# VinAIResearch/DiMSUM

Hardware: AMD Instinct MI355X
Metric: denoiser-fwd latents/sec (higher is better)
Workload: dtype f32; 1 GPU; DiM-L/2 denoiser forward, 256px (4x32x32 latents, 256 tokens), 256 latents per GPU, random-init weights (reference init, zero tensors re-drawn N(0, 0.02^2)); global_batch=256, parallelism=dp1 (replicas, independent latents), launch=eager, matmul_policy=f16s (see notes.matmul_policy)

## Files before the change

### dimsum_amd/_lib.py

```python
import ctypes as C
import os

_HERE = os.path.dirname(os.path.abspath(__file__))
LIB_PATH = os.environ.get("DIMSUM_HIP_LIB") or os.path.join(_HERE, "lib", "libdimsum_hip.so")

F32, F16, BF16 = 0, 1, 2
i32, i64, vp, f32 = C.c_int32, C.c_int64, C.c_void_p, C.c_float


u32 = C.c_uint32


class _Sized(C.Structure):

    def __init__(self, *args, **kw):
        super().__init__(*args, **kw)
        self.struct_size = C.sizeof(type(self))


class SsmExt(_Sized):
    _fields_ = [("struct_size", u32), ("kernel_variant", i32), ("ckpt_ptr", vp), ("timing_start_event", vp), ("timing_stop_event", vp),
                ("out_z_lo_offset", i64), ("dt_w_ptr", vp), ("dt_x_ptr", vp), ("dt_w_row_stride", i64), ("dt_x_row_stride", i64),
                ("dt_rank", i32), ("out_z_f16", i32), ("out_z_scale_ptr", vp), ("out_z_scale_ld", i64)]


class SsmParams(_Sized):
    _fields_ = ([("struct_size", u32)]
                + [(n, i32) for n in ("batch", "dim", "seqlen", "dstate", "n_groups", "n_chunks", "delta_softplus", "dtype", "reserved")]
                + [(n, i64) for n in ("A_d_stride", "A_dstate_stride", "B_batch_stride", "B_group_stride",
                                      "B_dstate_stride", "C_batch_stride", "C_group_stride", "C_dstate_stride",
                                      "u_batch_stride", "u_d_stride", "delta_batch_stride", "delta_d_stride",
                                      "z_batch_stride", "z_d_stride", "out_batch_stride", "out_d_stride",
                                      "out_z_batch_stride", "out_z_d_stride")]
                + [(n, vp) for n in ("A_ptr", "B_ptr", "C_ptr", "D_ptr", "u_ptr", "delta_ptr", "delta_bias_ptr",
                                     "z_ptr", "out_ptr", "x_ptr", "out_z_ptr")]
                + [("ext", C.POINTER(SsmExt))])


def attach_ext(P, ext_type):
    E = ext_type()
    P.ext = C.pointer(E)
    return E


class SsmBwdParams(_Sized):
    _fields_ = ([("struct_size", u32), ("reserved", u32), ("fwd", SsmParams)]
                + [(n, i64) for n in ("dout_batch_stride", "dout_d_stride", "dA_d_stride", "dA_dstate_stride",
                                      "dB_batch_stride", "dB_group_stride", "dB_dstate_stride", "dC_batch_stride",
                                      "dC_group_stride", "dC_dstate_stride", "du_batch_stride", "du_d_stride",
                                      "dz_batch_stride", "dz_d_stride", "ddelta_batch_stride", "ddelta_d_stride")]
                + [(n, vp) for n in ("dout_ptr", "dA_ptr", "dB_ptr", "dC_ptr", "dD_ptr", "du_ptr", "dz_ptr",
                                     "ddelta_ptr", "ddelta_bias_ptr", "workspace_ptr")]
                + [("workspace_bytes", i64)])


class SsmBidirParams(_Sized):
    _fields_ = [("struct_size", u32), ("reserved", u32), ("fwd", SsmParams), ("A_b_ptr", vp), ("A_b_d_stride", i64), ("A_b_dstate_stride", i64),
                ("out_b_ptr", vp), ("out_b_batch_stride", i64), ("out_b_d_stride", i64), ("ckpt_b_ptr", vp)]


class SsmBidirBwdParams(_Sized):
    _fields_ = [("struct_size", u32), ("reserved", u32), ("bwd", SsmBwdParams), ("A_b_ptr", vp), ("A_b_d_stride", i64), ("A_b_dstate_stride", i64),
                ("out_b_ptr", vp), ("out_b_batch_stride", i64), ("out_b_d_stride", i64), ("ckpt_b_ptr", vp),
                ("dA_b_ptr", vp), ("dA_b_d_stride", i64), ("dA_b_dstate_stride", i64)]


class OptimParams(_Sized):
    _fields_ = ([("struct_size", u32), ("n_tensors", i32), ("n_chunks", i32), ("n_partials", i32)]
                + [(n, vp) for n in ("p_ptrs", "g_ptrs", "m_ptrs", "v_ptrs", "ema_ptrs", "step_ptrs", "numel", "chunk_table", "partials", "total_norm")]
                + [(n, C.c_double) for n in ("lr", "beta1", "beta2", "eps", "weight_decay", "max_norm", "ema_decay")]
                + [("reserved", i64 * 4)])


OPTIM_CHUNK, OPTIM_MAX_PARTIALS = 4096, 2048


class ConvParams(_Sized):
    _fields_ = ([("struct_size", u32)] + [(n, i32) for n in ("batch", "dim", "seqlen", "width", "silu_activation", "dtype", "reserved")]
                + [(n, i64) for n in ("x_batch_stride", "x_c_stride", "weight_c_stride", "weight_width_stride",
                                      "out_batch_stride", "out_c_stride")]
                + [(n, vp) for n in ("x_ptr", "weight_ptr", "bias_ptr", "out_ptr")])


class ConvBwdParams(_Sized):
    _fields_ = ([("struct_size", u32), ("reserved", u32), ("fwd", ConvParams)]
                + [(n, i64) for n in ("dout_batch_stride", "dout_c_stride", "dx_batch_stride", "dx_c_stride",
                                      "dweight_c_stride", "dweight_width_stride")]
                + [(n, vp) for n in ("dout_ptr", "dx_ptr", "dweight_ptr", "dbias_ptr")])


class NormParams(_Sized):
    _fields_ = ([("struct_size", u32)] + [(n, i32) for n in ("rows", "cols", "is_rms_norm", "x_dtype", "residual_dtype", "out_dtype")]
                + [("eps", f32)]
                + [(n, i64) for n in ("x_row_stride", "residual_row_stride", "y_row_stride", "residual_out_row_stride")]
                + [(n, vp) for n in ("x_ptr", "residual_ptr", "weight_ptr", "bias_ptr", "y_ptr", "residual_out_ptr",
                                     "mean_ptr", "rstd_ptr", "xbias_ptr", "mod_scale_ptr", "mod_shift_ptr")]
                + [("mod_row_stride", i64), ("rows_per_batch", i32), ("y_split3", i32), ("y_inv_scale_ptr", vp)])


class NormBwdParams(_Sized):
    _fields_ = ([("struct_size", u32)] + [(n, i32) for n in ("rows", "cols", "is_rms_norm")] + [("eps", f32), ("reserved", i32)]
                + [(n, i64) for n in ("r_row_stride", "dy_row_stride", "dres_row_stride", "dx_row_stride")]
                + [(n, vp) for n in ("r_ptr", "weight_ptr", "mean_ptr", "rstd_ptr", "dy_ptr", "dres_ptr", "dx_ptr",
                                     "dweight_ptr", "dbias_ptr")])


class TtParams(_Sized):
    _fields_ = ([("struct_size", u32)] + [(n, i32) for n in ("batch", "tokens", "channels", "grid", "kind", "y_split3")]
                + [(n, i64) for n in ("x_batch_stride", "x_token_stride", "res_batch_stride", "res_token_stride",
                                      "y_batch_stride", "y_token_stride", "mod_batch_stride", "w_batch_stride",
                                      "w_token_stride", "red_batch_stride")]
                + [(n, vp) for n in ("x_ptr", "in_index_ptr", "out_index_ptr", "gate_ptr", "scale_ptr", "shift_ptr",
                                     "residual_ptr", "y_ptr", "w_ptr", "wdot_ptr", "wsum_ptr", "tsum_ptr", "y_inv_scale_ptr")]
                + [("y_f16s_lds_offset", i32), ("reserved", i32)])


class XattnParams(_Sized):
    _fields_ = ([("struct_size", u32)] + [(n, i32) for n in ("batch", "seqlen", "heads", "head_dim")] + [("scale", f32), ("n_dirs", i32)]
                + [(n, i64) for n in ("qkv_batch_stride", "qkv_token_stride", "out_batch_stride", "out_token_stride")]
                + [(n, vp) for n in ("qkv1_ptr", "qkv2_ptr", "out_ptr", "lse_ptr", "bias1_ptr", "bias2_ptr")]
                + [("precision", i32), ("out_split3", i32)]
                + [(n, vp) for n in ("x1_inv_ptr", "x2_inv_ptr", "kv_bound_ptr", "out_inv_ptr")] + [("qkv_f16", i32), ("reserved2", i32)])


class XattnBwdParams(_Sized):
    _fields_ = ([("struct_size", u32), ("reserved", u32), ("fwd", XattnParams)] + [(n, i64) for n in ("dqkv_batch_stride", "dqkv_token_stride")]
                + [(n, vp) for n in ("dout_ptr", "dqkv1_ptr", "dqkv2_ptr", "delta_ptr")])


class GemmExt(_Sized):
    _fields_ = ([("struct_size", u32), ("rows_per_batch", i32), ("timing_start_event", vp), ("timing_stop_event", vp)]
                + [(n, i32) for n in ("tune_variant", "tune_group_m", "tune_reserved", "c_image_pieces")]
                + [(n, vp) for n in ("gate_bound_ptr", "h_inv_scale_ptr", "residual_ptr", "gate_ptr")]
                + [("residual_ld", i64), ("gate_ld", i64), ("x12_ptr", vp), ("x12_ld", i64), ("a_alias_rows", i64), ("b_alias_rows", i64),
                   ("a_alias_weight_order", i32), ("qkv_q_cols", i32), ("conv_weight_ptr", vp), ("conv_bias_ptr", vp),
                   ("conv_rows", i32), ("conv_width", i32), ("conv_seq", i32), ("conv_weight_ld", i32),
                   ("a_block_inv_ptr", vp), ("a_block_inv_ld", i64), ("tn_pair_a_cols", i64), ("tn_pair_b_cols", i64),
                   ("k_scale_ptr", vp), ("c_scale_ptr", vp), ("k_inv_a_ptr", vp), ("k_inv_b_ptr", vp)])


class GemmParams(_Sized):
    _fields_ = ([("struct_size", u32)] + [(n, i32) for n in ("m", "n", "k", "operand_dtype", "epilogue")] + [("out_scale", f32), ("reserved", i32)]
                + [(n, i64) for n in ("lda", "ldb", "ldc")]
                + [(n, vp) for n in ("a_ptr", "b_ptr", "bias_ptr", "c_ptr", "a_inv_scale_ptr", "b_inv_scale_ptr")]
                + [("ext", C.POINTER(GemmExt))])


class F16sJob(C.Structure):
    _fields_ = ([(n, vp) for n in ("src", "dst", "inv_scale_ptr", "l1max_ptr", "absmax_ptr")]
                + [(n, i64) for n in ("rows", "cols", "src_row_stride", "dst_row_stride")] + [("l1_factor", f32), ("reserved", i32)])


GEMM_EPI_F32, GEMM_EPI_GATED_GELU_SPLIT3, GEMM_EPI_GATED_GELU_F16, GEMM_EPI_F32_BIAS, GEMM_EPI_F32_GATE_RESIDUAL, GEMM_EPI_F16_QKV, GEMM_EPI_F32_CONV = 0, 1, 2, 3, 4, 5, 6

EXPORTS = (
    "dimsum_status_string", "dimsum_abi_version", "dimsum_target_arch",
    "dimsum_event_create", "dimsum_event_destroy", "dimsum_event_elapsed_ms",
    "dimsum_ssm_scan_fwd", "dimsum_ssm_scan_bwd", "dimsum_ssm_scan_bwd_workspace_bytes", "dimsum_ssm_scan_fwd_variant",
    "dimsum_ssm_scan_bidir_fwd", "dimsum_ssm_scan_bidir_bwd", "dimsum_ssm_scan_bidir_fwd_variant",
    "dimsum_optim_grad_sumsq", "dimsum_optim_adamw_ema_step", "dimsum_optim_write_ptrs",
    "dimsum_causal_conv1d_fwd", "dimsum_causal_conv1d_bwd",
    "dimsum_norm_fwd", "dimsum_norm_bwd", "dimsum_token_transform", "dimsum_xattn_fusion_fwd", "dimsum_xattn_fusion_bwd",
    "dimsum_gated_gelu_fwd", "dimsum_gated_gelu_bwd", "dimsum_gated_gelu_fwd_split3", "dimsum_gated_gelu_bwd_split3", "dimsum_gated_gelu_bwd_pair", "dimsum_gated_gelu_bwd_f16s", "dimsum_split3", "dimsum_split3_t",
    "dimsum_gemm_nt", "dimsum_gemm_nt_kernel_for", "dimsum_gemm_tn", "dimsum_gemm_nn", "dimsum_row_factors", "dimsum_rows_block_f16s", "dimsum_rows_f16s", "dimsum_rows_f16s_multi",
)

_P = C.POINTER
_SIGNATURES = (
    [("dimsum_status_string", C.c_char_p, [C.c_int]), ("dimsum_target_arch", C.c_char_p, None), ("dimsum_abi_version", C.c_int, None),
     ("dimsum_event_create", vp, []), ("dimsum_event_destroy", None, [vp]), ("dimsum_event_elapsed_ms", C.c_float, [vp, vp])]
    + [(name, C.c_int, [_P(ptype), vp]) for name, ptype in (
        ("dimsum_ssm_scan_fwd", SsmParams), ("dimsum_ssm_scan_bwd", SsmBwdParams), ("dimsum_ssm_scan_bidir_fwd", SsmBidirParams),
        ("dimsum_ssm_scan_bidir_bwd", SsmBidirBwdParams), ("dimsum_optim_grad_sumsq", OptimParams), ("dimsum_optim_adamw_ema_step", OptimParams),
        ("dimsum_causal_conv1d_fwd", ConvParams), ("dimsum_causal_conv1d_bwd", ConvBwdParams), ("dimsum_norm_fwd", NormParams),
        ("dimsum_norm_bwd", NormBwdParams), ("dimsum_token_transform", TtParams), ("dimsum_xattn_fusion_fwd", XattnParams),
        ("dimsum_xattn_fusion_bwd", XattnBwdParams), ("dimsum_gemm_nt", GemmParams))]
    + [(name, C.c_int, [vp] * nptr + [i64, i64, vp]) for name, nptr in (
        ("dimsum_gated_gelu_fwd", 3), ("dimsum_gated_gelu_bwd", 5), ("dimsum_gated_gelu_fwd_split3", 3), ("dimsum_gated_gelu_bwd_split3", 5),
        ("dimsum_gated_gelu_bwd_pair", 5), ("dimsum_gated_gelu_bwd_f16s", 6))]
    + [("dimsum_optim_write_ptrs", C.c_int, [vp, i64, _P(vp), i32, vp]),
       ("dimsum_gemm_nt_kernel_for", C.c_int, [_P(GemmParams)]),
       ("dimsum_gemm_tn", C.c_int, [_P(GemmParams), i32, i64, vp]),
       ("dimsum_gemm_nn", C.c_int, [_P(GemmParams), i32, i64, vp]),
       ("dimsum_rows_block_f16s", C.c_int, [vp, i64, i64, i64, vp, i64, vp, i64, vp]),
       ("dimsum_row_factors", C.c_int, [vp, vp, i64, vp, vp, vp]),
       ("dimsum_split3", C.c_int, [vp, i64, i64, i64, vp, i32, vp]),
       ("dimsum_split3_t", C.c_int, [vp, i64, i64, i64, vp, vp]),
       ("dimsum_rows_f16s", C.c_int, [vp, i64, i64, i64, vp, i64, vp, vp, vp]),
       ("dimsum_rows_f16s_multi", C.c_int, [_P(F16sJob), i32, vp]),
       ("dimsum_ssm_scan_bwd_workspace_bytes", i64, [i32] * 5),
       ("dimsum_ssm_scan_fwd_variant", C.c_int, [_P(SsmParams)]),
       ("dimsum_ssm_scan_bidir_fwd_variant", C.c_int, [_P(SsmBidirParams)])])

_lib = None


def load():
    global _lib
    if _lib is not None:
        return _lib
    if not os.path.exists(LIB_PATH):
        raise RuntimeError(f"dimsum_amd: {LIB_PATH} not found. Build it with `python -c 'import __graft_entry__ as g; "
                           f"g.build()'` or `make -C dimsum_amd/csrc`. There is no CPU fallback.")
    lib = C.CDLL(LIB_PATH)
    for name, restype, argtypes in _SIGNATURES:
        if hasattr(lib, name):
            fn = getattr(lib, name)
            fn.restype, fn.argtypes = restype, argtypes
    if lib.dimsum_abi_version() != 18:
        raise RuntimeError("dimsum_amd: libdimsum_hip.so ABI version mismatch; rebuild")
    _lib = lib
    return lib


GEMM_NT_KERNELS = {0: "gemm_nt_kernel<256 x 256 tiles>", 1: "gemm_nt_m128_kernel<128 x 256 tiles>", 2: "gemm_nt_persist_kernel"}
SCAN_FWD_KERNELS = {1: "ssm_scan_fwd_kernel", 2: "ssm_scan_fwd_split_kernel<2 lanes per channel>",
                    4: "ssm_scan_fwd_split_kernel<4 lanes per channel>",
                    16: "ssm_scan_fwd_lanes_kernel<one lane per state>"}


def check(status, what):
    if status != 0:
        raise RuntimeError(f"{what}: {load().dimsum_status_string(status).decode()} (status {status})")
```

### dimsum_amd/csrc/gemm_nt.hip

```cpp
#include "gemm_nt_kernel.hpp"

namespace dimsum {
namespace gemm_nt {

template <int kOp, int kEpi, int kVar = 0> int launch(const Args &a, hipStream_t s, hipEvent_t e0, hipEvent_t e1, int *probe) {
    if (probe) { *probe = 0; return DIMSUM_OK; }
    const dim3 grid((unsigned)(a.tiles_m * a.tiles_n)), block(512);
    if (e0 || e1) hipExtLaunchKernelGGL((gemm_nt_kernel<kOp, kEpi, kVar>), grid, block, 0, s, e0, e1, 0, a);
    else hipLaunchKernelGGL((gemm_nt_kernel<kOp, kEpi, kVar>), grid, block, 0, s, a);
    return launch_status();
}

template <int kOp, int kEpi, int kVar = 0> int launch_m128(const Args &a0, hipStream_t s, hipEvent_t e0, hipEvent_t e1, int *probe) {
    if (probe) { *probe = 1; return DIMSUM_OK; }
    Args a = a0;
    a.tiles_m = a.M / 128;
    a.group_m = a.tiles_m <= 32 ? a.tiles_m : 2 * a0.group_m;
    const dim3 grid((unsigned)(a.tiles_m * a.tiles_n)), block(256);
    if (e0 || e1) hipExtLaunchKernelGGL((gemm_nt_m128_kernel<kOp, kEpi, kVar>), grid, block, 0, s, e0, e1, 0, a);
    else hipLaunchKernelGGL((gemm_nt_m128_kernel<kOp, kEpi, kVar>), grid, block, 0, s, a);
    return launch_status();
}

inline int persist_grid() {
    int dev = 0, cus = 256;
    if (hipGetDevice(&dev) == hipSuccess) (void)hipDeviceGetAttribute(&cus, hipDeviceAttributeMultiprocessorCount, dev);
    return cus >= 8 ? cus / 8 * 8 : 8;
}
inline bool persist_ok(const Args &a, int tune_variant) {
    const int nk = a.K / kBK;
    return tune_variant != 513 && tune_variant != 512 && nk >= 4 && nk % 2 == 0 && a.tiles_m * a.tiles_n > persist_grid() && a.a_alias_tiles == 0 && a.b_alias_tiles == 0;
}
template <int kOp, int kEpi, int kVar = 0> int launch_persist(const Args &a, hipStream_t s, hipEvent_t e0, hipEvent_t e1, int *probe) {
    if (probe) { *probe = 2; return DIMSUM_OK; }
    const dim3 grid((unsigned)persist_grid()), block(512);
    if (e0 || e1) hipExtLaunchKernelGGL((gemm_nt_persist_kernel<kOp, kEpi, kVar>), grid, block, 0, s, e0, e1, 0, a);
    else hipLaunchKernelGGL((gemm_nt_persist_kernel<kOp, kEpi, kVar>), grid, block, 0, s, a);
    return launch_status();
}

template <int kEpi, int kVar = 0> int launch_f16(const Args &a, hipStream_t s, hipEvent_t e0, hipEvent_t e1, bool m128, int *probe) {
    return m128 ? launch_m128<kOpF16, kEpi, kVar>(a, s, e0, e1, probe) : launch<kOpF16, kEpi, kVar>(a, s, e0, e1, probe);
}

struct gemm_flat_t : dimsum_gemm_ext_t {
    int32_t m, n, k, operand_dtype, epilogue;
    float out_scale;
    int64_t lda, ldb, ldc;
    const void *a_ptr, *b_ptr, *bias_ptr;
    void *c_ptr;
    const void *a_inv_scale_ptr, *b_inv_scale_ptr;
};
static int gemm_flat_from(const dimsum_gemm_params_t *p, gemm_flat_t &f) {
    if (!p) return DIMSUM_ERR_NULL;
    if (p->struct_size != sizeof(dimsum_gemm_params_t)) return DIMSUM_ERR_ABI;
    const int rc = ext_from<dimsum_gemm_ext_t>(p->ext, f);
    if (rc != DIMSUM_OK) return rc;
    f.m = p->m; f.n = p->n; f.k = p->k; f.operand_dtype = p->operand_dtype; f.epilogue = p->epilogue; f.out_scale = p->out_scale;
    f.lda = p->lda; f.ldb = p->ldb; f.ldc = p->ldc;
    f.a_ptr = p->a_ptr; f.b_ptr = p->b_ptr; f.bias_ptr = p->bias_ptr; f.c_ptr = p->c_ptr;
    f.a_inv_scale_ptr = p->a_inv_scale_ptr; f.b_inv_scale_ptr = p->b_inv_scale_ptr;
    return DIMSUM_OK;
}

}
}

static int gemm_nt_run(const dimsum_gemm_params_t *pub, void *stream, int *probe) {
    using namespace dimsum;
    using namespace dimsum::gemm_nt;
    gemm_flat_t flat;
    {
        const int frc = gemm_flat_from(pub, flat);
        if (frc != DIMSUM_OK) return frc;
    }
    const gemm_flat_t *p = &flat;
    if (!p->a_ptr || !p->b_ptr || !p->c_ptr) return DIMSUM_ERR_NULL;
    if (p->operand_dtype != DIMSUM_F16 && p->operand_dtype != DIMSUM_BF16) return DIMSUM_ERR_DTYPE;
    if (p->m <= 0 || p->n <= 0 || p->k < 2 * kBK || p->m % kBM != 0 || p->k % kBK != 0 || p->n % 4 != 0) return DIMSUM_ERR_SHAPE;
    if (p->a_alias_rows != 0 && (p->a_alias_rows < 0 || p->a_alias_rows % kBK != 0 || p->k != 3 * p->a_alias_rows)) return DIMSUM_ERR_SHAPE;
    if (p->b_alias_rows != 0 && (p->b_alias_rows < 0 || p->b_alias_rows % kBK != 0 || p->k != 3 * p->b_alias_rows || (p->epilogue != DIMSUM_GEMM_EPI_F32 && p->epilogue != DIMSUM_GEMM_EPI_F32_CONV))) return DIMSUM_ERR_SHAPE;
    if (p->lda % 8 != 0 || p->ldb % 8 != 0 || p->lda < (p->a_alias_rows ? 2 * p->a_alias_rows : p->k) || p->ldb < (p->b_alias_rows ? 2 * p->b_alias_rows : p->k) ||
        !aligned_to<char>(p->a_ptr, 16) ||
        !aligned_to<char>(p->b_ptr, 16))
        return DIMSUM_ERR_STRIDE;
    if ((int64_t)256 * p->lda * 2 >= ((int64_t)1 << 31) || (int64_t)256 * p->ldb * 2 >= ((int64_t)1 << 31) || (int64_t)257 * p->ldc * 4 >= ((int64_t)1 << 31))
        return DIMSUM_ERR_STRIDE;
    Args a{};
    a.A = reinterpret_cast<const char *>(p->a_ptr);
    a.C = p->c_ptr;
    a.lda = p->lda; a.ldb = p->ldb; a.ldc = p->ldc;
    a.M = p->m; a.K = p->k;
    a.tiles_m = p->m / kBM;
    a.out_scale = p->out_scale;
    a.a_alias_tiles = (int)(p->a_alias_rows / kBK);
    a.a_alias_from = a.a_alias_tiles;
    if (p->a_alias_weight_order) {
        if (!p->a_alias_rows) return DIMSUM_ERR_SHAPE;
        a.a_alias_tiles *= 2;
        a.a_alias_from = a.a_alias_tiles;
    }
    a.b_alias_tiles = (int)(p->b_alias_rows / kBK);
    a.group_m = p->tune_group_m > 0 ? p->tune_group_m : (a.tiles_m <= 16 ? a.tiles_m : 4);
    a.stagger = p->tune_reserved > 0 ? p->tune_reserved : 0;
    if ((p->a_inv_scale_ptr == nullptr) != (p->b_inv_scale_ptr == nullptr)) return DIMSUM_ERR_NULL;
    a.sa = reinterpret_cast<const float *>(p->a_inv_scale_ptr);
    a.sb = reinterpret_cast<const float *>(p->b_inv_scale_ptr);
    if (a.sb && !aligned_to<char>(a.sb, 16)) return DIMSUM_ERR_STRIDE;
    hipStream_t s = reinterpret_cast<hipStream_t>(stream);
    hipEvent_t e0 = reinterpret_cast<hipEvent_t>(p->timing_start_event), e1 = reinterpret_cast<hipEvent_t>(p->timing_stop_event);
    const bool bf = p->operand_dtype == DIMSUM_BF16;
    const bool m128 = p->tune_variant == 512 || (p->tune_variant == 0 && !bf && p->k <= 576 && (p->epilogue == DIMSUM_GEMM_EPI_F32 || p->epilogue == DIMSUM_GEMM_EPI_F32_BIAS));
#ifndef DIMSUM_GEMM_TUNE
    if (p->tune_variant != 0 && p->tune_variant != 512 && p->tune_variant != 513 && p->tune_variant != 514) return DIMSUM_ERR_UNSUPPORTED;
#endif
    if (p->tune_variant == 512 && bf) return DIMSUM_ERR_UNSUPPORTED;
    if (p->epilogue == DIMSUM_GEMM_EPI_F32_GATE_RESIDUAL) {
        if (!p->residual_ptr) return DIMSUM_ERR_NULL;
        if (p->ldc % 4 != 0 || p->ldc < p->n || !aligned_to<char>(p->c_ptr, 16) || p->residual_ld % 4 != 0 || p->residual_ld < p->n ||
            !aligned_to<char>(p->residual_ptr, 16) || (p->bias_ptr && !aligned_to<char>(p->bias_ptr, 16)) ||
            (p->gate_ptr && (p->gate_ld % 4 != 0 || !aligned_to<char>(p->gate_ptr, 16))))
            return DIMSUM_ERR_STRIDE;
        if (p->gate_ptr && (p->rows_per_batch <= 0 || p->rows_per_batch % kBM != 0 || p->m % p->rows_per_batch != 0)) return DIMSUM_ERR_SHAPE;
        a.B0 = a.B1 = reinterpret_cast<const char *>(p->b_ptr);
        a.bias0 = reinterpret_cast<const float *>(p->bias_ptr);
        a.res = reinterpret_cast<const float *>(p->residual_ptr);
        a.gate = reinterpret_cast<const float *>(p->gate_ptr);
        a.ldr = p->residual_ld; a.ldg = p->gate_ld;
        a.rows_per_batch = p->gate_ptr ? p->rows_per_batch : p->m;
        a.N = p->n;
        a.tiles_n = (p->n + kBN - 1) / kBN;
        constexpr int kShipR = kVarFullLineStores | kVarNtStores;
        if (!bf && !m128 && p->tune_variant == 514 && p->n % kBN == 0 && persist_ok(a, p->tune_variant)) return launch_persist<kOpF16, kEpiF32GateRes, kShipR>(a, s, e0, e1, probe);
        return bf ? launch<kOpBf16, kEpiF32GateRes, kShipR>(a, s, e0, e1, probe) : launch_f16<kEpiF32GateRes, kShipR>(a, s, e0, e1, m128, probe);
    }
    if (p->epilogue == DIMSUM_GEMM_EPI_F16_QKV) {
        if (bf || !a.sa || !p->gate_bound_ptr) return DIMSUM_ERR_NULL;
        if (p->rows_per_batch <= 0 || p->rows_per_batch % kBM != 0 || p->m % p->rows_per_batch != 0 || p->qkv_q_cols <= 0 || p->qkv_q_cols % 16 != 0 ||
            p->qkv_q_cols > p->n || p->n % 8 != 0)
            return DIMSUM_ERR_SHAPE;
        if (p->ldc % 8 != 0 || p->ldc < p->n || !aligned_to<char>(p->c_ptr, 16) || (p->bias_ptr && !aligned_to<char>(p->bias_ptr, 16)) ||
            (int64_t)257 * p->ldc * 2 >= ((int64_t)1 << 31))
            return DIMSUM_ERR_STRIDE;
        a.B0 = a.B1 = reinterpret_cast<const char *>(p->b_ptr);
        a.bias0 = reinterpret_cast<const float *>(p->bias_ptr);
        a.gate_bound = reinterpret_cast<const float *>(p->gate_bound_ptr);
        a.rows_per_batch = p->rows_per_batch;
        a.q_cols = p->qkv_q_cols;
        a.N = p->n;
        a.tiles_n = (p->n + kBN - 1) / kBN;
        return launch_f16<kEpiF16Qkv>(a, s, e0, e1, p->tune_variant == 512 || (p->tune_variant == 0 && p->k <= 576), probe);
    }
    if (p->epilogue == DIMSUM_GEMM_EPI_F32_CONV) {
        if (!p->conv_weight_ptr) return DIMSUM_ERR_NULL;
        if (p->conv_rows <= 0 || p->conv_rows % kBM != 0 || p->conv_rows > p->m || p->conv_width < 2 || p->conv_width > 4 || p->conv_seq <= 0 || 256 % p->conv_seq != 0 ||
            p->conv_seq % 4 != 0 || p->n % p->conv_seq != 0 || p->conv_weight_ld < p->conv_width)
            return DIMSUM_ERR_SHAPE;
        if (p->ldc % 4 != 0 || p->ldc < p->n || !aligned_to<char>(p->c_ptr, 16)) return DIMSUM_ERR_STRIDE;
        a.B0 = a.B1 = reinterpret_cast<const char *>(p->b_ptr);
        a.conv_w = reinterpret_cast<const float *>(p->conv_weight_ptr);
        a.conv_b = reinterpret_cast<const float *>(p->conv_bias_ptr);
        a.conv_rows = p->conv_rows; a.conv_width = p->conv_width; a.conv_seq = p->conv_seq; a.conv_w_ld = p->conv_weight_ld;
        a.N = p->n;
        a.tiles_n = (p->n + kBN - 1) / kBN;
        constexpr int kShipC = kVarFullLineStores | kVarNtStores;
        return bf ? launch<kOpBf16, kEpiF32Conv, kShipC>(a, s, e0, e1, probe) : launch_f16<kEpiF32Conv, kShipC>(a, s, e0, e1, p->tune_variant == 512 || (p->tune_variant == 0 && p->k <= 576), probe);
    }
    if (p->epilogue == DIMSUM_GEMM_EPI_F32 || p->epilogue == DIMSUM_GEMM_EPI_F32_BIAS) {
        if (p->ldc % 4 != 0 || p->ldc < p->n || !aligned_to<char>(p->c_ptr, 16)) return DIMSUM_ERR_STRIDE;
        const bool bias = p->epilogue == DIMSUM_GEMM_EPI_F32_BIAS;
        if (bias && (!p->bias_ptr || !aligned_to<char>(p->bias_ptr, 16))) return DIMSUM_ERR_NULL;
        a.B0 = a.B1 = reinterpret_cast<const char *>(p->b_ptr);
        a.bias0 = reinterpret_cast<const float *>(p->bias_ptr);
        a.N = p->n;
        a.tiles_n = (p->n + kBN - 1) / kBN;
        constexpr int kShip = kVarFullLineStores | kVarNtStores;
        if (bias) return bf ? launch<kOpBf16, kEpiF32Bias, kShip>(a, s, e0, e1, probe) : launch_f16<kEpiF32Bias, kShip>(a, s, e0, e1, m128, probe);
#ifdef DIMSUM_GEMM_TUNE
        if (bf) switch (p->tune_variant) {
            case 0: case 512: case 513: break;
            case 100: return launch<kOpBf16, kEpiF32, 0>(a, s, e0, e1, probe);
            case 1: return launch<kOpBf16, kEpiF32, 1>(a, s, e0, e1, probe);
            case 2: return launch<kOpBf16, kEpiF32, 2>(a, s, e0, e1, probe);
            case 4: return launch<kOpBf16, kEpiF32, 4>(a, s, e0, e1, probe);
            case 8: return launch<kOpBf16, kEpiF32, 8>(a, s, e0, e1, probe);
            case 12: return launch<kOpBf16, kEpiF32, 12>(a, s, e0, e1, probe);
            case 16: return launch<kOpBf16, kEpiF32, 16>(a, s, e0, e1, probe);
            case 3: return launch<kOpBf16, kEpiF32, 3>(a, s, e0, e1, probe);
            case 40: return launch<kOpBf16, kEpiF32, 40>(a, s, e0, e1, probe);
            case 44: return launch<kOpBf16, kEpiF32, 44>(a, s, e0, e1, probe);
            case 72: return launch<kOpBf16, kEpiF32, 72>(a, s, e0, e1, probe);
            case 104: return launch<kOpBf16, kEpiF32, 104>(a, s, e0, e1, probe);
            default: return DIMSUM_ERR_UNSUPPORTED;
        }
#endif
        return bf ? launch<kOpBf16, kEpiF32, kShip>(a, s, e0, e1, probe) : launch_f16<kEpiF32, kShip>(a, s, e0, e1, m128, probe);
    }
    if (p->epilogue == DIMSUM_GEMM_EPI_GATED_GELU_SPLIT3 || p->epilogue == DIMSUM_GEMM_EPI_GATED_GELU_F16) {
        if (p->n % 16 != 0) return DIMSUM_ERR_SHAPE;
        const int F = p->n / 2;
        const bool img = p->epilogue == DIMSUM_GEMM_EPI_GATED_GELU_SPLIT3;
        if (p->c_image_pieces != 0 && p->c_image_pieces != 3 && !(img && p->c_image_pieces == 2)) return DIMSUM_ERR_UNSUPPORTED;
        a.c_pieces2 = p->c_image_pieces == 2;
        if (p->ldc % 8 != 0 || p->ldc < (img ? (a.c_pieces2 ? 2 : 3) : 1) * (int64_t)F || !aligned_to<char>(p->c_ptr, 16) || (int64_t)257 * p->ldc * 2 + 6 * (int64_t)F >= ((int64_t)1 << 31))
            return DIMSUM_ERR_STRIDE;
        if (p->bias_ptr && !aligned_to<char>(p->bias_ptr, 16)) return DIMSUM_ERR_STRIDE;
        a.B0 = reinterpret_cast<const char *>(p->b_ptr);
        a.B1 = a.B0 + (int64_t)F * p->ldb * 2;
        a.bias0 = reinterpret_cast<const float *>(p->bias_ptr);
        a.bias1 = a.bias0 ? a.bias0 + F : nullptr;
        a.N = F;
        a.tiles_n = (F + 127) / 128;
        if (p->gate_bound_ptr) {
            if (img || !a.sa || !p->h_inv_scale_ptr) return DIMSUM_ERR_NULL;
            a.gate_bound = reinterpret_cast<const float *>(p->gate_bound_ptr);
            a.inv_out = reinterpret_cast<float *>(p->h_inv_scale_ptr);
        }
        if (p->x12_ptr) {
            const bool f16_train = !img && !bf && a.sa && p->gate_bound_ptr;
            if (!f16_train && (!img || !bf || a.sa)) return DIMSUM_ERR_UNSUPPORTED;
            if (p->x12_ld % 4 != 0 || p->x12_ld < p->n || !aligned_to<char>(p->x12_ptr, 16) || (int64_t)257 * p->x12_ld * 4 + (int64_t)p->n * 4 >= ((int64_t)1 << 31))
                return DIMSUM_ERR_STRIDE;
            a.x12 = reinterpret_cast<float *>(p->x12_ptr);
            a.ldx = p->x12_ld;
            if (f16_train) return launch<kOpF16, kEpiGatedF16, kVarKeepX12>(a, s, e0, e1, probe);
            return launch<kOpBf16, kEpiGatedSplit3, kVarKeepX12>(a, s, e0, e1, probe);
        }
        if (img) return bf ? launch<kOpBf16, kEpiGatedSplit3>(a, s, e0, e1, probe) : launch<kOpF16, kEpiGatedSplit3>(a, s, e0, e1, probe);
        if (!bf && !m128 && F % 128 == 0 && persist_ok(a, p->tune_variant)) return launch_persist<kOpF16, kEpiGatedF16>(a, s, e0, e1, probe);
        return bf ? launch<kOpBf16, kEpiGatedF16>(a, s, e0, e1, probe) : launch_f16<kEpiGatedF16>(a, s, e0, e1, m128, probe);
    }
    return DIMSUM_ERR_UNSUPPORTED;
}

extern "C" int dimsum_gemm_nt(const dimsum_gemm_params_t *p, void *stream) { return gemm_nt_run(p, stream, nullptr); }

extern "C" int dimsum_gemm_nt_kernel_for(const dimsum_gemm_params_t *p) {
    int which = -1;
    const int rc = gemm_nt_run(p, nullptr, &which);
    return rc == DIMSUM_OK ? which : -rc;
}

extern "C" int dimsum_gemm_tn(const dimsum_gemm_params_t *pub, int32_t splits, int64_t c_split_stride, void *stream) {
    using namespace dimsum;
    using namespace dimsum::gemm_nt;
    gemm_flat_t flat;
    {
        const int frc = gemm_flat_from(pub, flat);
        if (frc != DIMSUM_OK) return frc;
    }
    const gemm_flat_t *p = &flat;
    if (!p->a_ptr || !p->b_ptr || !p->c_ptr) return DIMSUM_ERR_NULL;
    if (p->operand_dtype != DIMSUM_F16 && p->operand_dtype != DIMSUM_BF16) return DIMSUM_ERR_DTYPE;
    if (p->epilogue != DIMSUM_GEMM_EPI_F32 || p->bias_ptr) return DIMSUM_ERR_UNSUPPORTED;
    if (((p->a_inv_scale_ptr || p->a_block_inv_ptr) == 0) != (p->b_inv_scale_ptr == nullptr)) return DIMSUM_ERR_NULL;
    if ((p->a_inv_scale_ptr || p->a_block_inv_ptr) && (p->operand_dtype != DIMSUM_F16 || splits != 1 || p->tn_pair_a_cols != 0 || p->a_alias_rows != 0)) return DIMSUM_ERR_UNSUPPORTED;
    if (p->k_inv_b_ptr && !p->k_inv_a_ptr) return DIMSUM_ERR_NULL;
    if (p->k_scale_ptr || p->k_inv_a_ptr) {
        if (p->k_inv_a_ptr ? (p->k_scale_ptr || p->c_scale_ptr) : !p->c_scale_ptr) return DIMSUM_ERR_NULL;
        if (p->operand_dtype != DIMSUM_F16 || p->a_inv_scale_ptr || p->a_block_inv_ptr || p->tn_pair_a_cols != 0 || p->a_alias_rows != 0) return DIMSUM_ERR_UNSUPPORTED;
        if (splits < 1 || p->k / splits > 16384) return DIMSUM_ERR_SHAPE;
        if ((p->k_scale_ptr && (!aligned_to<char>(p->k_scale_ptr, 16) || !aligned_to<char>(p->c_scale_ptr, 4))) ||
            (p->k_inv_a_ptr && (!aligned_to<char>(p->k_inv_a_ptr, 16) || (p->k_inv_b_ptr && !aligned_to<char>(p->k_inv_b_ptr, 16)) || p->k / splits % 8 != 0)))
            return DIMSUM_ERR_STRIDE;
    }
    if (p->a_block_inv_ptr && (p->a_inv_scale_ptr || p->a_block_inv_ld < p->k / kBK || p->k > 64 * kBK)) return DIMSUM_ERR_SHAPE;
    if (p->b_inv_scale_ptr && !aligned_to<char>(p->b_inv_scale_ptr, 16)) return DIMSUM_ERR_STRIDE;
    const int row_splits = (p->tn_pair_a_cols != 0) ? splits / 3 : splits;
    const int64_t n_pad = (p->n + kBN - 1) / kBN * kBN;
    if (splits < 1 || row_splits < 1 || p->m <= 0 || p->n <= 0 || p->m % kBM != 0 || p->n % 4 != 0 || (p->n % kBN != 0 && (p->ldb < n_pad || p->tn_pair_a_cols != 0)) ||
        p->k % ((int64_t)row_splits * kBK) != 0 || p->k / row_splits < 2 * kBK)
        return DIMSUM_ERR_SHAPE;
    if (p->lda % 8 != 0 || p->ldb % 8 != 0 || p->lda < p->m || p->ldb < p->n || !aligned_to<char>(p->a_ptr, 16) || !aligned_to<char>(p->b_ptr, 16) ||
        p->ldc % 4 != 0 || p->ldc < p->n || !aligned_to<char>(p->c_ptr, 16) || (splits > 1 && (c_split_stride % 4 != 0 || c_split_stride < (int64_t)p->m * p->ldc)))
        return DIMSUM_ERR_STRIDE;
    if ((int64_t)64 * p->lda * 2 + 512 >= ((int64_t)1 << 31) || (int64_t)64 * p->ldb * 2 + 512 >= ((int64_t)1 << 31) || (int64_t)257 * p->ldc * 4 >= ((int64_t)1 << 31))
        return DIMSUM_ERR_STRIDE;
    Args a{};
    a.A = reinterpret_cast<const char *>(p->a_ptr);
    a.B0 = a.B1 = reinterpret_cast<const char *>(p->b_ptr);
    a.C = p->c_ptr;
    a.lda = p->lda; a.ldb = p->ldb; a.ldc = p->ldc;
    a.M = p->m; a.N = p->n; a.K = p->k / row_splits;
    a.tiles_m = p->m / kBM;
    a.tiles_n = (int)(n_pad / kBN);
// ... 97 lines not shown
```

### dimsum_amd/csrc/gemm_nt_kernel.hpp

```cpp
#pragma once
#include "common.hpp"

namespace dimsum {
namespace gemm_nt {

typedef float f4 __attribute__((ext_vector_type(4)));
typedef __bf16 bf16x8_t __attribute__((ext_vector_type(8)));
typedef _Float16 f16x8_t __attribute__((ext_vector_type(8)));
typedef unsigned u32x4 __attribute__((ext_vector_type(4)));
typedef unsigned u32x2 __attribute__((ext_vector_type(2)));
typedef __attribute__((address_space(3))) void lds_void_t;
typedef __attribute__((address_space(1))) const void glb_void_t;

constexpr int kBM = 256, kBN = 256, kBK = 64;
constexpr int kHalf = 16384;
constexpr int kParity = 4 * kHalf;
constexpr int kSlotA0 = 0, kSlotA1 = kHalf, kSlotB0 = 2 * kHalf, kSlotB1 = 3 * kHalf;

enum { kOpBf16 = 0, kOpF16 = 1 };
enum { kEpiF32 = 0, kEpiGatedSplit3 = 1, kEpiGatedF16 = 2, kEpiF32Bias = 3, kEpiF32GateRes = 4, kEpiF16Qkv = 5, kEpiF32Conv = 6 };

struct Args {
    const char *A, *B0, *B1;
    void *C;
    const float *bias0, *bias1;
    const float *sa, *sb;
    const float *gate_bound;
    float *inv_out;
    const float *res, *gate;
    int64_t ldr, ldg;
    int rows_per_batch;
    int64_t lda, ldb, ldc;
    int M, N, K;
    int tiles_m, tiles_n;
    float out_scale;
    int group_m;
    int stagger;
    float *x12;
    int64_t ldx;
    int splits;
    int64_t c_split_stride;
    int a_alias_tiles;
    int a_alias_from;
    int tn_pieces;
    int64_t a_pair_cols, b_pair_cols;
    int b_alias_tiles;
    const float *conv_w, *conv_b;
    int conv_rows, conv_width, conv_seq, conv_w_ld;
    const float *a_block_inv;
    int a_block_inv_ld;
    const _Float16 *k_fac;
    const float *c_scale;
    const float *k_inv_a, *k_inv_b;
    int q_cols;
    int c_pieces2;
};
enum { kVarLgkmAfterBarrier = 1, kVarNoEpilogue = 2, kVarNtStores = 4, kVarFullLineStores = 8, kVarNoSetprio = 16, kVarSc1Stores = 32, kVarSc0Stores = 64, kVarKeepX12 = 128, kVarTN = 256, kVarM128 = 512, kVarRebase = 1024, kVarPersist = 2048, kVarRowFac = 4096, kVarNN = 8192 };

__device__ __forceinline__ float dpp_row_ror8(float x) {
    const int v = __builtin_bit_cast(int, x);
    return __builtin_bit_cast(float, __builtin_amdgcn_update_dpp(v, v, 0x128, 0xf, 0xf, false));
}
template <int kAux> __device__ __forceinline__ void store_f4(__amdgpu_buffer_rsrc_t rsrc, unsigned voff, const f4 &v) {
    __builtin_amdgcn_raw_buffer_store_b128(__builtin_bit_cast(u32x4, v), rsrc, voff, 0, kAux);
}

template <int kOp> __device__ __forceinline__ f4 mma(const u32x4 &a, const u32x4 &b, f4 c) {
    if constexpr (kOp == kOpBf16) return __builtin_amdgcn_mfma_f32_16x16x32_bf16(__builtin_bit_cast(bf16x8_t, a), __builtin_bit_cast(bf16x8_t, b), c, 0, 0, 0);
    else return __builtin_amdgcn_mfma_f32_16x16x32_f16(__builtin_bit_cast(f16x8_t, a), __builtin_bit_cast(f16x8_t, b), c, 0, 0, 0);
}

__device__ __forceinline__ const char *uniform_ptr(const char *q) {
    const uint64_t v = reinterpret_cast<uint64_t>(q);
    const unsigned lo = __builtin_amdgcn_readfirstlane((unsigned)v), hi = __builtin_amdgcn_readfirstlane((unsigned)(v >> 32));
    return reinterpret_cast<const char *>(((uint64_t)hi << 32) | lo);
}

__device__ __forceinline__ unsigned pick_mask(bool c) {
    unsigned m = c ? 0xffffffffu : 0u;
    asm volatile("" : "+v"(m));
    return m;
}
__device__ __forceinline__ unsigned pick_mask_lanes(bool c) {
    unsigned m = c ? 0xffffffffu : 0u;
    asm volatile("" : "+v"(m));
    return m;
}
__device__ __forceinline__ float pick(unsigned m, float a, float b) {
    return __uint_as_float((__float_as_uint(a) & m) | (__float_as_uint(b) & ~m));
}
__device__ __forceinline__ f4 pick(unsigned m, const f4 &a, const f4 &b) {
    return f4{pick(m, a[0], b[0]), pick(m, a[1], b[1]), pick(m, a[2], b[2]), pick(m, a[3], b[3])};
}

#define DIMSUM_DS_READ_B128(dst, addr, off) asm volatile("ds_read_b128 %0, %1 offset:%2" : "=v"(dst) : "v"(addr), "i"(off))
#define DIMSUM_DS_READ_TR(dst, addr, off) asm volatile("ds_read_b64_tr_b16 %0, %1 offset:%2" : "=v"(dst) : "v"(addr), "i"(off))
#define DIMSUM_WAIT_VM(n) asm volatile("s_waitcnt vmcnt(" #n ")" ::: "memory")
#ifndef DIMSUM_PERSIST_GS
#define DIMSUM_PERSIST_GS 2
#endif
#ifndef DIMSUM_EPI_PACE
#define DIMSUM_EPI_PACE 0
#endif
#define DIMSUM_STR2(x) #x
#define DIMSUM_STR(x) DIMSUM_STR2(x)
#define DIMSUM_PACE_STORES() do { if constexpr (kM1 && DIMSUM_EPI_PACE >= 0) asm volatile("s_waitcnt vmcnt(" DIMSUM_STR(DIMSUM_EPI_PACE) ")" ::: "memory"); } while (0)
#define DIMSUM_WAIT_LGKM0() asm volatile("s_waitcnt lgkmcnt(0)" ::: "memory")

__device__ __forceinline__ float gelu_tanh_f(float x) {
    const float u = 0.7978845608028654f * (x + 0.044715f * x * x * x);
    return x * fast_rcp(1.0f + fast_exp2(-2.0f * kLog2e * u));
}

template <int kOp, int kEpi, int kVar>
__device__ __forceinline__ void gemm_body(const Args &p, char *lds) {
    const unsigned lds0 = (unsigned)(uintptr_t)(__attribute__((address_space(3))) char *)lds;
    const int lane = threadIdx.x & 63;
    const int w = __builtin_amdgcn_readfirstlane(threadIdx.x >> 6);
    constexpr bool kM1 = (kVar & kVarM128) != 0;
    constexpr int kTileM = kM1 ? 128 : kBM;
    constexpr int kMiRows = kM1 ? 64 : 128;
    const int wr = kM1 ? 0 : (w >> 2), wc = w & 3;

    constexpr bool kTN = (kVar & kVarTN) != 0;
    constexpr bool kNN = (kVar & kVarNN) != 0;
    constexpr bool kBT = kTN || kNN;
    static_assert(!kBT || kEpi == kEpiF32, "the TN / NN variants have the plain fp32 epilogue");
    static_assert(!(kBT && kM1) && !(kTN && kNN), "the TN / NN variants have 256 x 256 tiles only");
    constexpr bool kPersist = (kVar & kVarPersist) != 0;
    static_assert(!kPersist || (!kTN && !kM1 && (kEpi == kEpiF32 || kEpi == kEpiF32Bias || kEpi == kEpiF32GateRes || kEpi == kEpiGatedF16)), "persistent: the 256-row NT kernel");
    int tile_m, tile_n, split = 0;
    auto map_tile = [&](int bid, int &tile_m, int &tile_n) {
        const int nwg = kPersist ? p.tiles_m * p.tiles_n : (int)gridDim.x;
        const int q = nwg >> 3, r = nwg & 7, xcd = bid & 7;
        int t = (xcd < r ? xcd * (q + 1) : r * (q + 1) + (xcd - r) * q) + (bid >> 3);
        if constexpr (kBT) {
            const int tiles = p.tiles_m * p.tiles_n;
            split = t / tiles;
            t -= split * tiles;
        }
        const int GM = p.group_m;
        const int per_group = GM * p.tiles_n;
        const int g = t / per_group, within = t - g * per_group;
        const int first_m = g * GM;
        const int gsz = min(p.tiles_m - first_m, GM);
        tile_n = within / gsz;
        tile_m = first_m + (within - tile_n * gsz);
    };
    int bid = blockIdx.x;
    map_tile(bid, tile_m, tile_n);
    constexpr int kTileN = (kEpi == kEpiGatedSplit3 || kEpi == kEpiGatedF16) ? 128 : kBN;
    int m0 = tile_m * kTileM, n0 = tile_n * kTileN;

    const int st_row = w * 16 + (lane >> 2);
    const int st_kc = (lane & 3) ^ ((lane >> 5) << 1);
    const unsigned a_voff = (unsigned)((st_row * p.lda + st_kc * 8) * 2);
    struct Src { const char *a_base, *b_base[2]; unsigned b_voff[2]; };
    auto make_src = [&](int m0_, int n0_) {
        Src s_;
        if constexpr (kEpi == kEpiGatedSplit3 || kEpi == kEpiGatedF16) {
            s_.b_base[0] = p.B0 + (int64_t)n0_ * p.ldb * 2;
            s_.b_base[1] = p.B1 + (int64_t)n0_ * p.ldb * 2;
            const int row = min(st_row, p.N - 1 - n0_);
            s_.b_voff[0] = s_.b_voff[1] = (unsigned)((row * p.ldb + st_kc * 8) * 2);
        } else {
            s_.b_base[0] = s_.b_base[1] = p.B0 + (int64_t)n0_ * p.ldb * 2;
#pragma unroll
            for (int ni = 0; ni < 2; ++ni) {
                const int row = min(ni * 128 + st_row, p.N - 1 - n0_);
                s_.b_voff[ni] = (unsigned)((row * p.ldb + st_kc * 8) * 2);
            }
        }
        s_.a_base = p.A + (int64_t)m0_ * p.lda * 2;
        return s_;
    };
    Src cur = make_src(m0, n0);
    const char *(&b_base)[2] = cur.b_base;
    unsigned (&b_voff)[2] = cur.b_voff;
    const char *&a_base = cur.a_base;
    const int64_t a_half = (int64_t)kMiRows * p.lda * 2;
    unsigned b_voff2[2][2];
    if constexpr (kM1) {
#pragma unroll
        for (int ni = 0; ni < 2; ++ni)
#pragma unroll
            for (int h = 0; h < 2; ++h) {
                const int first = (kEpi == kEpiGatedSplit3 || kEpi == kEpiGatedF16) ? 0 : ni * 128;
                const int row = min(first + h * 64 + st_row, p.N - 1 - n0);
                b_voff2[ni][h] = (unsigned)((row * p.ldb + st_kc * 8) * 2);
            }
    }

    unsigned tn_voff_a[2], tn_voff_b[2];
    const char *tn_a = nullptr, *tn_b = nullptr;
    int64_t tn_a_tile = 0, tn_b_tile = 0;
    int tn_row_split = 0;
    if constexpr (kBT) {
#pragma unroll
        for (int pc = 0; pc < 2; ++pc) {
            const int row = w * 8 + pc * 4 + (lane >> 4), key = pc * 4 + (lane >> 4);
            const int chunk = ((((lane & 15) >> 1) ^ key) << 1) | (lane & 1);
            const int rl = row & 31, srow = kNN ? ((row & ~31) | (((rl & 15) >> 2) << 3) | ((rl >> 4) << 2) | (rl & 3)) : row;
            tn_voff_a[pc] = (unsigned)(srow * p.lda * 2 + chunk * 16);
            tn_voff_b[pc] = (unsigned)(srow * p.ldb * 2 + chunk * 16);
        }
        int row_split = split;
        int64_t a_col = 0, b_col = 0;
        if (p.tn_pieces) {
            const int spp = p.splits / 3, piece = split / spp;
            row_split = split - piece * spp;
// ... 264 lines not shown
            adv(spos, 2 * kU);
        };
#define DIMSUM_M1_SYNC()                                                                   \
    do {                                                                                   \
        DIMSUM_WAIT_LGKM0();                                                               \
        __builtin_amdgcn_s_barrier();                                                      \
        __builtin_amdgcn_sched_barrier(0);                                                 \
    } while (0)
#define DIMSUM_M1_PHASE(READ, SIZE, STAGE, VM, MI, NI, AF, BF)                              \
    do {                                                                                   \
        READ;                                                                              \
        adv(rpos, SIZE);                                                                   \
        STAGE;                                                                             \
        DIMSUM_WAIT_VM(VM);                                                                \
        DIMSUM_M1_SYNC();                                                                  \
        DIMSUM_QUADRANT(MI, NI, AF, BF);                                                   \
        __builtin_amdgcn_sched_barrier(0);                                                 \
    } while (0)
        st_a(0, 0); st_b(0, 0); st_b(1, 0); st_a(1, 0); st_a(0, 1); st_b(0, 1);
        DIMSUM_WAIT_VM(12);
        __builtin_amdgcn_s_barrier();
        __builtin_amdgcn_sched_barrier(0);
        DIMSUM_READ_A(a0, 0, rpos);
        adv(rpos, kU);
        DIMSUM_M1_SYNC();
        int kt = 0;
        for (; kt < nk - 2; ++kt) {
            DIMSUM_M1_PHASE(DIMSUM_READ_B(b0, 0, rpos), 2 * kU, st_b(1, kt + 1), 12, 0, 0, a0, b0);
            DIMSUM_M1_PHASE(DIMSUM_READ_B(b1, 0, rpos), 2 * kU, st_a(1, kt + 1), 12, 0, 1, a0, b1);
            DIMSUM_M1_PHASE(DIMSUM_READ_A(a1, 0, rpos), kU, st_a(0, kt + 2), 12, 1, 1, a1, b1);
            DIMSUM_M1_PHASE(DIMSUM_READ_A(a0, 0, rpos), kU, st_b(0, kt + 2), 12, 1, 0, a1, b0);
        }
        DIMSUM_M1_PHASE(DIMSUM_READ_B(b0, 0, rpos), 2 * kU, st_b(1, kt + 1), 12, 0, 0, a0, b0);
        DIMSUM_M1_PHASE(DIMSUM_READ_B(b1, 0, rpos), 2 * kU, st_a(1, kt + 1), 12, 0, 1, a0, b1);
        DIMSUM_M1_PHASE(DIMSUM_READ_A(a1, 0, rpos), kU, (void)0, 10, 1, 1, a1, b1);
        DIMSUM_M1_PHASE(DIMSUM_READ_A(a0, 0, rpos), kU, (void)0, 6, 1, 0, a1, b0);
        DIMSUM_M1_PHASE(DIMSUM_READ_B(b0, 0, rpos), 2 * kU, (void)0, 2, 0, 0, a0, b0);
        DIMSUM_M1_PHASE(DIMSUM_READ_B(b1, 0, rpos), 2 * kU, (void)0, 0, 0, 1, a0, b1);
        DIMSUM_M1_PHASE(DIMSUM_READ_A(a1, 0, rpos), kU, (void)0, 0, 1, 1, a1, b1);
        DIMSUM_QUADRANT(1, 0, a1, b0);
#undef DIMSUM_M1_PHASE
#undef DIMSUM_M1_SYNC
    } else {
    stage_a0(0); stage_b0(0); stage_b1(0); stage_a1(0);
    stage_a0(1); stage_b0(1); stage_b1(1); stage_a1(1);
    DIMSUM_WAIT_VM(12);
    __builtin_amdgcn_s_barrier();
    if (wr == 1) __builtin_amdgcn_s_barrier();
    __builtin_amdgcn_sched_barrier(0);
    DIMSUM_READ_A(a0, kSlotA0, 0);
    read_fac(0);
    DIMSUM_PHASE_SYNC();
    rebase(a0, 0, 0);
    DIMSUM_PHASE_END();

    }
#define DIMSUM_KTILE(KT, ST_A0, ST_B0, ST_B1, ST_A1, W12, W34)                                                                  \
    do {                                                                                                                        \
        const unsigned par = ((KT) & 1) * kParity, par_next = kParity - par;                                                    \
        DIMSUM_READ_B(b0, kSlotB0, par); ST_A0; if (W12) DIMSUM_WAIT_VM(12); DIMSUM_PHASE_SYNC();                               \
        DIMSUM_QUADRANT(0, 0, a0, b0); DIMSUM_PHASE_END();                                                                      \
        DIMSUM_READ_B(b1, kSlotB1, par); ST_B0; if (W12) DIMSUM_WAIT_VM(12); DIMSUM_PHASE_SYNC();                               \
        DIMSUM_QUADRANT(0, 1, a0, b1); DIMSUM_PHASE_END();                                                                      \
        DIMSUM_READ_A(a1, kSlotA1, par); read_fac(KT); ST_B1; if (W34) DIMSUM_WAIT_VM(12); DIMSUM_PHASE_SYNC();                 \
        rebase(a1, 1, KT); DIMSUM_QUADRANT(1, 1, a1, b1); DIMSUM_PHASE_END();                                                   \
        DIMSUM_READ_A(a0, kSlotA0, par_next); read_fac((KT) + 1);                                                               \
        ST_A1; if (W34) DIMSUM_WAIT_VM(12); DIMSUM_PHASE_SYNC();                                                                \
        DIMSUM_QUADRANT(1, 0, a1, b0);                                                                                          \
        rebase(a0, 0, (KT) + 1);                     \
        DIMSUM_PHASE_END();                                                                                                     \
    } while (0)
    bool resumed = false;
    for (;;) {
    bool has_next = false;
    int nbid = 0, ntile_m = 0, ntile_n = 0;
    Src nxt = cur;
    if constexpr (kPersist) {
        nbid = bid + (int)gridDim.x;
        has_next = nbid < p.tiles_m * p.tiles_n;
        if (has_next) {
            map_tile(nbid, ntile_m, ntile_n);
            nxt = make_src(ntile_m * kTileM, ntile_n * kTileN);
        }
    }
    if constexpr (kPersist) {
        for (int kt = 0; kt < nk; ++kt) {
            const bool own = kt + 2 < nk;
            const int skt = own ? kt + 2 : kt + 2 - nk;
            Src ss;
            ss.a_base = uniform_ptr(own ? cur.a_base : nxt.a_base);
            ss.b_base[0] = uniform_ptr(own ? cur.b_base[0] : nxt.b_base[0]);
            ss.b_base[1] = uniform_ptr(own ? cur.b_base[1] : nxt.b_base[1]);
            ss.b_voff[0] = cur.b_voff[0];
            ss.b_voff[1] = cur.b_voff[1];
            const bool w12 = !(resumed && kt < 2), w34 = !(resumed && kt < 1);
            DIMSUM_KTILE(kt, stage_of(ss, 0, skt), stage_of(ss, 1, skt), stage_of(ss, 2, skt), stage_of(ss, 3, skt), w12, w34);
        }
        if (wr == 0) __builtin_amdgcn_s_barrier();
    } else if constexpr (!kM1) {
    int kt = 0;
    for (; kt < nk - 2; ++kt) DIMSUM_KTILE(kt, stage_a0(kt + 2), stage_b0(kt + 2), stage_b1(kt + 2), stage_a1(kt + 2), true, true);
    {
        const unsigned par = (kt & 1) * kParity, par_next = kParity - par;
        DIMSUM_READ_B(b0, kSlotB0, par);
        DIMSUM_WAIT_VM(10);
        DIMSUM_PHASE_SYNC();
        DIMSUM_QUADRANT(0, 0, a0, b0);
        DIMSUM_PHASE_END();
        DIMSUM_READ_B(b1, kSlotB1, par);
        DIMSUM_WAIT_VM(8);
        DIMSUM_PHASE_SYNC();
        DIMSUM_QUADRANT(0, 1, a0, b1);
        DIMSUM_PHASE_END();
        DIMSUM_READ_A(a1, kSlotA1, par);
        read_fac(kt);
        DIMSUM_WAIT_VM(6);
        DIMSUM_PHASE_SYNC();
        rebase(a1, 1, kt);
        DIMSUM_QUADRANT(1, 1, a1, b1);
        DIMSUM_PHASE_END();
        DIMSUM_READ_A(a0, kSlotA0, par_next);
        read_fac(kt + 1);
        DIMSUM_WAIT_VM(4);
        DIMSUM_PHASE_SYNC();
        DIMSUM_QUADRANT(1, 0, a1, b0);
        rebase(a0, 0, kt + 1);
        DIMSUM_PHASE_END();
        DIMSUM_READ_B(b0, kSlotB0, par_next);
        DIMSUM_WAIT_VM(2);
        DIMSUM_PHASE_SYNC();
        DIMSUM_QUADRANT(0, 0, a0, b0);
        DIMSUM_PHASE_END();
        DIMSUM_READ_B(b1, kSlotB1, par_next);
        DIMSUM_WAIT_VM(0);
        DIMSUM_PHASE_SYNC();
        DIMSUM_QUADRANT(0, 1, a0, b1);
        DIMSUM_PHASE_END();
        DIMSUM_READ_A(a1, kSlotA1, par_next);
        read_fac(kt + 1);
        DIMSUM_PHASE_SYNC();
        rebase(a1, 1, kt + 1);
        DIMSUM_QUADRANT(1, 1, a1, b1);
        DIMSUM_PHASE_END();
        DIMSUM_QUADRANT(1, 0, a1, b0);
    }
    if (wr == 0) __builtin_amdgcn_s_barrier();
    }

    int lane_e = lane;
    if constexpr (kPersist) asm volatile("" : "+v"(lane_e));
    {
    const int lane = lane_e;
    const int ecol = wc * 32 + (lane >> 4) * 4;
    if constexpr (kVar & kVarNoEpilogue) {
#pragma unroll
        for (int mi = 0; mi < 2; ++mi)
#pragma unroll
            for (int ni = 0; ni < 2; ++ni)
#pragma unroll
                for (int i = 0; i < 4; ++i)
#pragma unroll
                    for (int j = 0; j < 2; ++j) asm volatile("" ::"v"(acc[mi][ni][i][j]));
    } else if constexpr (kEpi == kEpiF32 || kEpi == kEpiF32Bias || kEpi == kEpiF32GateRes || kEpi == kEpiF32Conv) {
        if constexpr (kEpi == kEpiF32Conv) {
            if (m0 < p.conv_rows) {
                constexpr int kNW = kM1 ? 4 : 8;
                constexpr int kHalfRows = kM1 ? 64 : 128;
                float *Ct = reinterpret_cast<float *>(p.C) + (int64_t)m0 * p.ldc + n0;
                const __amdgpu_buffer_rsrc_t crsrc = __builtin_amdgcn_make_buffer_rsrc(Ct, 0, 0x7fffffff, 0x00020000);
                const int W = p.conv_width;
                const bool has_s = p.sa != nullptr;
                const unsigned ms = pick_mask(has_s);
                const float *sap = has_s ? p.sa + m0 : reinterpret_cast<const float *>(p.A), *sbp = has_s ? p.sb : reinterpret_cast<const float *>(p.B0);
                float csa[2][4];
                f4 csb[2][2];
#pragma unroll
                for (int mi = 0; mi < 2; ++mi)
#pragma unroll
                    for (int i = 0; i < 4; ++i) {
                        csa[mi][i] = pick(ms, sap[mi * kMiRows + wr * 64 + i * 16 + (lane & 15)], 1.0f);
                    }
#pragma unroll
                for (int ni = 0; ni < 2; ++ni)
#pragma unroll
                    for (int j = 0; j < 2; ++j) {
                        const int col = n0 + ni * 128 + ecol + j * 16;
                        csb[ni][j] = pick(ms, *reinterpret_cast<const f4 *>(sbp + (col < p.N ? col : 0)), f4{1.f, 1.f, 1.f, 1.f});
                    }
                float ctap[2], cbia[2];
#pragma unroll
                for (int mi = 0; mi < 2; ++mi) {
                    const int row = m0 + mi * kMiRows + w * (kHalfRows / kNW) + (lane & 15);
                    ctap[mi] = pick(pick_mask_lanes((lane >> 4) < W), p.conv_w[(int64_t)row * p.conv_w_ld + ((lane >> 4) < W ? (lane >> 4) : 0)], 0.f);
                    cbia[mi] = pick(pick_mask(p.conv_b != nullptr), (p.conv_b ? p.conv_b : reinterpret_cast<const float *>(p.B0))[row], 0.f);
                }
#pragma unroll
                for (int mi = 0; mi < 2; ++mi) {
                    if (mi) __syncthreads();
#pragma unroll
                    for (int ni = 0; ni < 2; ++ni)
#pragma unroll
                        for (int j = 0; j < 2; ++j) {
                            const int tcol = ni * 128 + ecol + j * 16;
#pragma unroll
                            for (int i = 0; i < 4; ++i) {
                                const int rl = wr * 64 + i * 16 + (lane & 15);
                                const f4 x = acc[mi][ni][i][j] * (csb[ni][j] * csa[mi][i]);
                                *reinterpret_cast<f4 *>(lds + rl * 1024 + (((tcol >> 2) ^ (rl & 7)) << 4)) = x;
                            }
                        }
                    __syncthreads();
#pragma unroll 4
                    for (int it = 0; it < kHalfRows / kNW; ++it) {
                        const int rl = w * (kHalfRows / kNW) + it, row = m0 + mi * kMiRows + rl;
                        const f4 v = *reinterpret_cast<const f4 *>(lds + rl * 1024 + ((lane ^ (rl & 7)) << 4));
                        float w4[4];
#pragma unroll
                        for (int k = 0; k < 4; ++k)
                            w4[k] = (k >= 4 - W) ? __builtin_bit_cast(float, __builtin_amdgcn_readlane(__builtin_bit_cast(int, ctap[mi]), it + 16 * (k - (4 - W)))) : 0.f;
                        const float cbias = __builtin_bit_cast(float, __builtin_amdgcn_readlane(__builtin_bit_cast(int, cbia[mi]), it));
                        const bool start = ((4 * lane) % p.conv_seq) == 0;
                        float p1 = __shfl_up(v[3], 1, 64), p2 = __shfl_up(v[2], 1, 64), p3 = __shfl_up(v[1], 1, 64);
                        p1 = start ? 0.f : p1; p2 = start ? 0.f : p2; p3 = start ? 0.f : p3;
                        f4 y;
                        y[0] = fmaf(w4[0], p3, fmaf(w4[1], p2, fmaf(w4[2], p1, fmaf(w4[3], v[0], cbias))));
                        y[1] = fmaf(w4[0], p2, fmaf(w4[1], p1, fmaf(w4[2], v[0], fmaf(w4[3], v[1], cbias))));
                        y[2] = fmaf(w4[0], p1, fmaf(w4[1], v[0], fmaf(w4[2], v[1], fmaf(w4[3], v[2], cbias))));
                        y[3] = fmaf(w4[0], v[0], fmaf(w4[1], v[1], fmaf(w4[2], v[2], fmaf(w4[3], v[3], cbias))));
#pragma unroll
                        for (int e = 0; e < 4; ++e) y[e] = y[e] * fast_rcp(1.0f + fast_exp(-y[e]));
                        if (n0 + 4 * lane < p.N) store_f4<2>(crsrc, (unsigned)(((mi * kMiRows + rl) * p.ldc + 4 * lane) * 4), y);
                        DIMSUM_PACE_STORES();
                    }
                }
                return;
            }
        }
        constexpr int kAux = ((kVar & kVarNtStores) ? 2 : 0) | ((kVar & kVarSc1Stores) ? 16 : 0) | ((kVar & kVarSc0Stores) ? 1 : 0);
        float *Ct = reinterpret_cast<float *>(p.C) + (int64_t)m0 * p.ldc + n0 + (kBT ? (int64_t)split * p.c_split_stride : (int64_t)0);
        const __amdgpu_buffer_rsrc_t rsrc = __builtin_amdgcn_make_buffer_rsrc(Ct, 0, 0x7fffffff, 0x00020000);
        if constexpr (kVar & kVarFullLineStores) {
            const bool up = (lane & 8) != 0;
            const int frow = wr * 64 + (lane & 7);
            const int fcol = wc * 32 + (lane >> 4) * 4 + (up ? 16 : 0);
            const bool has_s = kRebase || p.sa != nullptr;
            const unsigned ms = pick_mask(has_s);
            const bool has_sb = has_s && !kRowFac;
            const unsigned msb = pick_mask(has_sb);
            const float *sap = p.sa ? p.sa + m0 : reinterpret_cast<const float *>(p.A), *sbp = has_sb ? p.sb : reinterpret_cast<const float *>(p.B0);
            float c_scale = 1.0f;
            if constexpr (kRowFac) c_scale = p.k_inv_a ? c_scale_own : *p.c_scale;
            bool live[2];
            f4 bv[2], sbv[2], gv[2];
            auto load_cols = [&](int ni) {
                const int col = ni * 128 + fcol;
                live[ni] = n0 + col < p.N;
                const int lc = live[ni] ? n0 + col : 0;
                bv[ni] = f4{0.f, 0.f, 0.f, 0.f}; sbv[ni] = gv[ni] = f4{1.f, 1.f, 1.f, 1.f};
                if constexpr (kEpi == kEpiF32Bias) bv[ni] = *reinterpret_cast<const f4 *>(p.bias0 + lc);
                if constexpr (kEpi == kEpiF32GateRes) {
                    bv[ni] = pick(pick_mask(p.bias0 != nullptr), *reinterpret_cast<const f4 *>((p.bias0 ? p.bias0 : reinterpret_cast<const float *>(p.B0)) + lc), bv[ni]);
                    gv[ni] = pick(pick_mask(p.gate != nullptr),
                                  *reinterpret_cast<const f4 *>((p.gate ? p.gate + (int64_t)(m0 / p.rows_per_batch) * p.ldg : reinterpret_cast<const float *>(p.B0)) + lc), gv[ni]);
                }
                sbv[ni] = pick(msb, *reinterpret_cast<const f4 *>(sbp + lc), sbv[ni]);
            };
            load_cols(0);
            live[1] = n0 + 128 + fcol < p.N;
            float rs[2][4][2];
            if constexpr (!kPersist || kRebase || kEpi != kEpiF32GateRes)
#pragma unroll
            for (int mi = 0; mi < 2; ++mi)
#pragma unroll
                for (int i = 0; i < 4; ++i) {
                    const int lrow = frow + mi * kMiRows + i * 16;
                    if constexpr (kRebase) rs[mi][i][0] = rs[mi][i][1] = top[mi * 2 + (i >> 1)];
                    else if constexpr (kRowFac) {
                        rs[mi][i][0] = c_scale * pick(ms, sap[lrow], 1.0f); rs[mi][i][1] = c_scale * pick(ms, sap[lrow + 8], 1.0f);
                    }
                    else {
                        rs[mi][i][0] = pick(ms, sap[lrow], 1.0f); rs[mi][i][1] = pick(ms, sap[lrow + 8], 1.0f);
                    }
                }
            constexpr int kGS = kPersist ? DIMSUM_PERSIST_GS : 4, kNG = 16 / kGS;
            f4 rr[2][kGS][2];
            float rg[2][kGS][2];
            auto load_res = [&](int g) {
                if constexpr (kEpi == kEpiF32GateRes) {
                    const int t0 = g * kGS, ni = t0 >> 3, mi = (t0 >> 2) & 1;
                    if constexpr (kPersist) {
#pragma unroll
                        for (int k = 0; k < kGS; ++k) {
                            const int lrow = frow + mi * kMiRows + ((t0 + k) & 3) * 16;
                            rg[g & 1][k][0] = pick(ms, sap[lrow], 1.0f); rg[g & 1][k][1] = pick(ms, sap[lrow + 8], 1.0f);
                        }
                    }
                    const float *rp = p.res + (int64_t)(m0 + frow + mi * kMiRows) * p.ldr + (live[ni] ? n0 + ni * 128 + fcol : 0);
#pragma unroll
                    for (int k = 0; k < kGS; ++k) {
                        const int i = (t0 + k) & 3;
                        rr[g & 1][k][0] = *reinterpret_cast<const f4 *>(rp + (int64_t)(i * 16) * p.ldr);
                        rr[g & 1][k][1] = *reinterpret_cast<const f4 *>(rp + (int64_t)(i * 16 + 8) * p.ldr);
                    }
                }
            };
            load_res(0);
#pragma unroll
            for (int g = 0; g < kNG; ++g) {
                if (g + 1 < kNG) load_res(g + 1);
                if (g * kGS == 4) load_cols(1);
#pragma unroll
                for (int k = 0; k < kGS; ++k) {
                    const int t = g * kGS + k, ni = t >> 3, mi = (t >> 2) & 1, i = t & 3;
                    const int col = ni * 128 + fcol;
                    const f4 x0 = acc[mi][ni][i][0], x1 = acc[mi][ni][i][1];
                    f4 s0, s1;
#pragma unroll
                    for (int e = 0; e < 4; ++e) {
                        const float r0 = dpp_row_ror8(x0[e]), r1 = dpp_row_ror8(x1[e]);
                        s0[e] = up ? r1 : x0[e];
                        s1[e] = up ? x1[e] : r0;
                    }
                    const int lrow = frow + mi * kMiRows + i * 16;
                    const unsigned voff = (unsigned)((lrow * p.ldc + col) * 4);
                    constexpr bool kRowsInGroup = kPersist && kEpi == kEpiF32GateRes;
                    s0 = s0 * (sbv[ni] * (kRowsInGroup ? rg[g & 1][k][0] : rs[mi][i][0]));
                    s1 = s1 * (sbv[ni] * (kRowsInGroup ? rg[g & 1][k][1] : rs[mi][i][1]));
                    if constexpr (kEpi == kEpiF32GateRes) {
                        s0 = rr[g & 1][k][0] + gv[ni] * (s0 + bv[ni]);
                        s1 = rr[g & 1][k][1] + gv[ni] * (s1 + bv[ni]);
                    } else {
                        s0 = s0 + bv[ni];
                        s1 = s1 + bv[ni];
                    }
                    if (live[ni]) {
                        store_f4<kAux>(rsrc, voff, s0);
                        store_f4<kAux>(rsrc, voff + (unsigned)(8 * p.ldc * 4), s1);
                    }
                    if constexpr (kEpi != kEpiF32GateRes) DIMSUM_PACE_STORES();
                }
            }
        } else {
            const int frow = wr * 64 + (lane & 15);
#pragma unroll
            for (int ni = 0; ni < 2; ++ni)
#pragma unroll
                for (int j = 0; j < 2; ++j) {
                    const int col = ni * 128 + ecol + j * 16;
                    if (n0 + col < p.N) {
                        f4 bv = f4{0.f, 0.f, 0.f, 0.f};
                        if constexpr (kEpi == kEpiF32Bias) bv = *reinterpret_cast<const f4 *>(p.bias0 + n0 + col);
#pragma unroll
                        for (int mi = 0; mi < 2; ++mi)
#pragma unroll
                            for (int i = 0; i < 4; ++i)
                                store_f4<kAux>(rsrc, (unsigned)(((frow + mi * kMiRows + i * 16) * p.ldc + col) * 4), acc[mi][ni][i][j] + bv);
                    }
                }
        }
    } else if constexpr (kEpi == kEpiF16Qkv) {
        constexpr int kNW = kM1 ? 4 : 8;
        float *red = reinterpret_cast<float *>(lds);
        const float wl1 = p.gate_bound[0], bmax = p.gate_bound[1];
        float row_sa[2][4], row_qs[2][4];
        f4 cbv[2][2], csb[2][2];
#pragma unroll
        for (int mi = 0; mi < 2; ++mi)
#pragma unroll
            for (int i = 0; i < 4; ++i) row_sa[mi][i] = p.sa[m0 + mi * kMiRows + wr * 64 + i * 16 + (lane & 15)];
        {
            const unsigned mbias = pick_mask(p.bias0 != nullptr);
            const float *b0p = p.bias0 ? p.bias0 : p.sb;
#pragma unroll
            for (int ni = 0; ni < 2; ++ni)
#pragma unroll
                for (int j = 0; j < 2; ++j) {
                    const int col = n0 + ni * 128 + ecol + j * 16, lc = col < p.N ? col : 0;
                    cbv[ni][j] = pick(mbias, *reinterpret_cast<const f4 *>(b0p + lc), f4{0.f, 0.f, 0.f, 0.f});
                    csb[ni][j] = *reinterpret_cast<const f4 *>(p.sb + lc);
                }
        }
        {
            const float *sab = p.sa + (int64_t)(m0 / p.rows_per_batch) * p.rows_per_batch;
            float mloc = 0.f;
            for (int t = threadIdx.x; t < p.rows_per_batch; t += kNW * 64) mloc = fmaxf(mloc, sab[t]);
            mloc = wave_allmax(mloc);
            if (lane == 0) red[w] = mloc;
        }
        __syncthreads();
        float mb = red[0];
#pragma unroll
        for (int i = 1; i < kNW; ++i) mb = fmaxf(mb, red[i]);
        __syncthreads();
        float kv_scale, kv_inv;
        f16s_scales(2.0f * (32768.0f * mb * wl1 + bmax), kv_scale, kv_inv);
#pragma unroll
        for (int mi = 0; mi < 2; ++mi)
#pragma unroll
            for (int i = 0; i < 4; ++i) {
                float qinv;
                f16s_scales(2.0f * (32768.0f * row_sa[mi][i] * wl1 + bmax), row_qs[mi][i], qinv);
            }
#pragma unroll
        for (int ni = 0; ni < 2; ++ni)
#pragma unroll
            for (int j = 0; j < 2; ++j) {
                const int tcol = ni * 128 + ecol + j * 16, col = n0 + tcol;
                const f4 bv = cbv[ni][j], sbv = csb[ni][j];
                const bool is_q = col < p.q_cols;
                const int unit = tcol >> 2;
#pragma unroll
                for (int mi = 0; mi < 2; ++mi)
#pragma unroll
                    for (int i = 0; i < 4; ++i) {
                        const int r = mi * kMiRows + wr * 64 + i * 16 + (lane & 15);
                        const f4 x = acc[mi][ni][i][j] * (sbv * row_sa[mi][i]) + bv;
                        const float sc = is_q ? row_qs[mi][i] : kv_scale;
                        const __half2 a = __floats2half2_rn(x[0] * sc, x[1] * sc), b = __floats2half2_rn(x[2] * sc, x[3] * sc);
                        *reinterpret_cast<uint2 *>(lds + r * 512 + ((unit ^ (lane & 15)) << 3)) = make_uint2(__builtin_bit_cast(unsigned, a), __builtin_bit_cast(unsigned, b));
                    }
            }
        __syncthreads();
        char *Ct = reinterpret_cast<char *>(p.C) + ((int64_t)m0 * p.ldc + n0) * 2;
        const __amdgpu_buffer_rsrc_t rsrc = __builtin_amdgcn_make_buffer_rsrc(Ct, 0, 0x7fffffff, 0x00020000);
        const int piece = lane & 31;
        const bool live = n0 + piece * 8 < p.N;
#pragma unroll
        for (int it = 0; it < 16; ++it) {
            const int r = w * 32 + it * 2 + (lane >> 5);
            const char *src = lds + r * 512 + ((piece ^ ((r & 15) >> 1)) << 4);
            u32x4 v = *reinterpret_cast<const u32x4 *>(src);
            v = (r & 1) ? u32x4{v[2], v[3], v[0], v[1]} : v;
            if (live) __builtin_amdgcn_raw_buffer_store_b128(v, rsrc, (unsigned)((r * p.ldc + piece * 8) * 2), 0, 2);
        }
    } else {
        constexpr bool kImg = kEpi == kEpiGatedSplit3;
        const bool has_s = p.sa != nullptr, has_b = p.bias0 != nullptr;
        const unsigned ms = pick_mask(has_s), mb = pick_mask(has_b);
        const float *sap = has_s ? p.sa + m0 : reinterpret_cast<const float *>(p.A);
        const float *sbp = has_s ? p.sb : reinterpret_cast<const float *>(p.B0), *b0p = has_b ? p.bias0 : reinterpret_cast<const float *>(p.B0), *b1p = has_b ? p.bias1 : b0p;
        const int sb2_off = has_s ? p.N : 0;
        float row_sa[2][4], row_hs[2][4];
        f4 cbv1[2], cbv2[2], csb1[2], csb2[2];
#pragma unroll
        for (int mi = 0; mi < 2; ++mi)
#pragma unroll
            for (int i = 0; i < 4; ++i) row_sa[mi][i] = pick(ms, sap[mi * kMiRows + wr * 64 + i * 16 + (lane & 15)], 1.0f);
#pragma unroll
        for (int j = 0; j < 2; ++j) {
            const int col = n0 + ecol + j * 16, lc = col < p.N ? col : 0;
            const f4 zero = f4{0.f, 0.f, 0.f, 0.f}, one = f4{1.f, 1.f, 1.f, 1.f};
            cbv1[j] = pick(mb, *reinterpret_cast<const f4 *>(b0p + lc), zero);
            cbv2[j] = pick(mb, *reinterpret_cast<const f4 *>(b1p + lc), zero);
            csb1[j] = pick(ms, *reinterpret_cast<const f4 *>(sbp + lc), one);
            csb2[j] = pick(ms, *reinterpret_cast<const f4 *>(sbp + sb2_off + lc), one);
        }
        const bool bound = !kImg && has_s && p.gate_bound != nullptr;
        const float gb0 = bound ? p.gate_bound[0] : 0.f, gb1 = bound ? p.gate_bound[1] : 0.f;
#pragma unroll
        for (int mi = 0; mi < 2; ++mi)
#pragma unroll
            for (int i = 0; i < 4; ++i) {
                const int r = mi * kMiRows + wr * 64 + i * 16 + (lane & 15);
                row_hs[mi][i] = p.out_scale;
                if constexpr (!kImg) {
                    if (bound) {
                        const float xb = 32768.0f * row_sa[mi][i] * gb0 + gb1;
                        float inv;
                        f16s_scales(4.0f * xb * xb, row_hs[mi][i], inv);
                        if (tile_n == 0 && wc == 0 && lane < 16) p.inv_out[m0 + r] = inv;
                    }
                }
            }
        if constexpr ((kVar & kVarKeepX12) != 0) {
            float *Xt = p.x12 + (int64_t)m0 * p.ldx + n0;
            const __amdgpu_buffer_rsrc_t xrsrc = __builtin_amdgcn_make_buffer_rsrc(Xt, 0, 0x7fffffff, 0x00020000);
            const bool up = (lane & 8) != 0;
            const int frow = wr * 64 + (lane & 7);
            const int fcol = wc * 32 + (lane >> 4) * 4 + (up ? 16 : 0);
            const bool xlive = n0 + fcol < p.N;
#pragma unroll
            for (int ni = 0; ni < 2; ++ni)
#pragma unroll
                for (int mi = 0; mi < 2; ++mi)
#pragma unroll
                    for (int i = 0; i < 4; ++i) {
                        const f4 x0 = acc[mi][ni][i][0] * ((ni ? csb2[0] : csb1[0]) * row_sa[mi][i]), x1 = acc[mi][ni][i][1] * ((ni ? csb2[1] : csb1[1]) * row_sa[mi][i]);
                        f4 s0, s1;
// ... 171 lines not shown
```

### dimsum_amd/gemm.py

```python
import contextlib

import threading

import os

import torch
import torch.nn.functional as F

_policy = "default"


class _Local(threading.local):
    frozen = None


_tls = _Local()


@contextlib.contextmanager
def frozen_weights():
    outer = _tls.frozen
    if outer is None:
        _tls.frozen = {}
    try:
# ... 293 lines not shown
def qkv_f16s(x, weight, bias, rows_per_batch, bound2):
    from . import native
    w16 = weight_f16s(weight)
    N = weight.shape[0]
    if not (os.environ.get("DIMSUM_QKV_F16", "1") != "0" and own_gemm_enabled() and native.gemm_nt_supported(x.data, w16.data) and rows_per_batch % 256 == 0
            and x.data.shape[0] % rows_per_batch == 0 and N % 3 == 0 and (N // 3) % 16 == 0):
        return None
    b = None if bias is None else bias.detach().float().contiguous()
    return native.gemm_nt(x.data, w16.data, bias=b, epilogue="f16_qkv", scales=(x.inv, w16.inv), gate_bound=bound2, rows_per_batch=rows_per_batch,
                          q_cols=N // 3)


def f16s_plan(model):
    from .attention_fusion import CrossAttentionFusion
    from .mlp import GatedMLP
    plan = []
    for m in model.modules():
        if hasattr(m, "in_proj") and hasattr(m, "x_proj") and hasattr(m, "dt_proj"):
            plan.append((m.in_proj.weight, "plain", None, None))
            if getattr(m, "out_proj", None) is not None and getattr(m.out_proj, "bias", None) is None:
                plan.append((m.out_proj.weight, "plain_t", None, None))
        elif isinstance(m, CrossAttentionFusion):
            plan += [(m.qkv1.weight, "kv", m.qkv1.bias, m.qkv2), (m.proj.weight, "plain", None, None)]
        elif isinstance(m, GatedMLP):
            plan += [(m.w12.weight, "gated", m.w12.bias, None), (m.w3.weight, "plain", None, None)]
        elif type(m).__name__ == "Attention" and hasattr(m, "qkv") and hasattr(m, "proj"):
            plan += [(m.qkv.weight, "kv", m.qkv.bias, None), (m.proj.weight, "plain", None, None)]
    return plan


@contextlib.contextmanager
def forward_scope(model, rows):
    import os
    from . import native
    first = next(model.parameters(), None)
    training = torch.is_grad_enabled()
    if (_policy != "f16s" or _tls.frozen is not None or not torch.backends.cuda.matmul.allow_tf32 or first is None
            or (training and (os.environ.get("DIMSUM_F16S_TRAIN", "1") == "0" or os.environ.get("DIMSUM_SPLIT3_TRAIN", "1") == "0"
                              or os.environ.get("DIMSUM_FORWARD_SCOPE_TRAIN", "1") == "0" or first.dtype != torch.float32 or torch.is_autocast_enabled("cuda")))
            or not first.is_cuda or torch.cuda.is_current_stream_capturing() or not own_gemm_enabled() or os.environ.get("DIMSUM_SPLIT3", "1") == "0"
            or rows < int(os.environ.get("DIMSUM_SPLIT3_MIN_ROWS", "8192")) or os.environ.get("DIMSUM_FORWARD_SCOPE", "1") == "0"):
        yield
        return
    ident = tuple(id(p_) for p_ in model.parameters())
    cached = model.__dict__.get("_f16s_plan")
    if cached is None or cached[0] != ident:
        cached = model.__dict__["_f16s_plan"] = (ident, f16s_plan(model))
    plan = cached[1]

    def src_ok(t):
        if t is None:
            return True
        t2 = t if t.dim() == 2 else t.reshape(1, -1)
        return (t.is_cuda and t.dtype == torch.float32 and t2.stride(1) == 1 and t2.shape[1] % 4 == 0 and (t2.shape[0] == 1 or t2.stride(0) % 4 == 0)
                and t.data_ptr() % 16 == 0)
    jobs, slot = [], 0
    tbufs = {}
    layout = []
    for w, kind, bias, partner in plan:
        ok = src_ok(w) and src_ok(bias) and (partner is None or (src_ok(partner.weight) and src_ok(partner.bias)))
        if not ok:
            layout.append(None)
            continue
        layout.append((len(jobs), slot))
        if kind == "plain":
            jobs.append((w.detach(), True, slot, None, 1.0))
            slot += 1
        elif kind == "plain_t" and (training or os.environ.get("DIMSUM_OUT_PROJ_F16", "1") == "0"):
            layout[-1] = None
        elif kind == "plain_t":
            buf = tbufs.setdefault(tuple(w.shape), [])
            buf.append(len(jobs))
            jobs.append((w.detach(), True, slot, None, 1.0, None))
            slot += 1
        elif kind == "gated":
            jobs.append((w.detach(), True, slot, None, _K10))
            if bias is not None:
                jobs.append((bias.detach().float(), False, None, slot + 1, 1.0))
            slot += 2
        else:
            ws = [(w, bias)] + ([(partner.weight, partner.bias)] if partner is not None else [])
            for i, (wi, bi) in enumerate(ws):
                jobs.append((wi.detach(), True, slot + 2 * i, None, _K10))
                if bi is not None:
                    jobs.append((bi.detach().float(), False, None, slot + 2 * i + 1, 1.0))
            slot += 4
    tdata = {}
    for shape, idx in tbufs.items():
        data = torch.empty((len(idx),) + shape, device=first.device, dtype=torch.float16)
        inv = torch.empty((len(idx), shape[0]), device=first.device, dtype=torch.float32)
        for n, j in enumerate(idx):
            jobs[j] = jobs[j][:5] + ((data[n], inv[n]),)
            tdata[j] = (shape, n)
        tbufs[shape] = (data, inv)
    images, scal = native.rows_f16s_multi(jobs, n_slots=slot)
    tbufs = {shape: (_pad_cols_256(data.transpose(1, 2)), inv) for shape, (data, inv) in tbufs.items()}
    cache = {}
    key = lambda kind, w: (kind, w.data_ptr(), tuple(w.shape), tuple(w.stride()), w.dtype)
    for (w, kind, bias, partner), lay in zip(plan, layout):
        if lay is None:
            continue
        j, sl = lay
        if kind == "plain":
            cache[key("w16s", w)] = ((images[j], scal[sl:sl + 1]), w)
        elif kind == "plain_t":
            shape, n = tdata[j]
            cache[key("w16t", w)] = ((tbufs[shape][0][n], tbufs[shape][1][n]), w)
        elif kind == "gated":
            cache[key("w16s", w)] = ((images[j], lambda i=sl: scal[i:i + 1] / _K10), w)
            cache[key("w16s_bound", w)] = (scal[sl:sl + 2], w)
        else:
            cache[key("w16s", w)] = ((images[j], lambda i=sl: scal[i:i + 1] / _K10), w)
            if partner is not None:
                j2 = j + (2 if bias is not None else 1)
                cache[key("w16s", partner.weight)] = ((images[j2], lambda i=sl + 2: scal[i:i + 1] / _K10), partner.weight)
                cache[key("kvbound", w)] = (scal[sl:sl + 4], w)
            else:
                cache[key("kvbound", w)] = (torch.cat([scal[sl:sl + 2], scal[sl:sl + 2]]), w)
    if not training and os.environ.get("DIMSUM_FORWARD_MEMO", "1") != "0":
        alogs = [a for m in model.modules() for a in (getattr(m, "A_log", None), getattr(m, "A_b_log", None)) if isinstance(a, torch.nn.Parameter) and a.is_cuda]
        if alogs:
            vals = torch._foreach_neg(torch._foreach_exp([a.detach().float() for a in alogs]))
            for a, v in zip(alogs, vals):
                cache[key("negexpA", a)] = (v, a)
    _tls.frozen = cache
    try:
        yield
    finally:
        _tls.frozen = None


def neg_exp(a_log):
    frozen = _tls.frozen
    if frozen is not None and not torch.is_grad_enabled() and not torch.cuda.is_current_stream_capturing():
        hit = frozen.get(("negexpA", a_log.data_ptr(), tuple(a_log.shape), tuple(a_log.stride()), a_log.dtype))
        if hit is not None:
            return hit[0]
    return -torch.exp(a_log.float())


def own_gemm_enabled():
    import os
    return os.environ.get("DIMSUM_GEMM_NT", "1") != "0"


def _nt(a, b, **kw):
    from . import native
    if own_gemm_enabled() and native.gemm_nt_supported(a, b):
        return native.gemm_nt(a, b, **kw)
    y = torch.mm(a, b.t(), out_dtype=torch.float32)
    return y if kw.get("bias") is None else y + kw["bias"]


def _tail(y, bias, residual, gate, rows_per_batch):
    if bias is not None:
        y = y + bias
    if residual is None:
        return y
    if gate is not None:
        y = (y.view(-1, rows_per_batch, y.shape[-1]) * gate.unsqueeze(1)).view(y.shape)
    return residual + y


def _nt_f16s(a, b, bias=None, residual=None, gate=None, rows_per_batch=None):
    from . import native
    if own_gemm_enabled() and native.gemm_nt_supported(a.data, b.data) and (gate is None or rows_per_batch % 256 == 0):
        return native.gemm_nt(a.data, b.data, bias=bias, scales=(a.inv, b.inv), residual=residual, gate=gate, rows_per_batch=rows_per_batch)
    return _tail(torch.mm(a.data, b.data.t(), out_dtype=torch.float32) * a.inv[:, None] * b.inv[None, :], bias, residual, gate, rows_per_batch)


def linear_split3(x3, weight, bias=None, residual=None, gate=None, rows_per_batch=None):
    from . import native
    if isinstance(x3, native.F16Image):
        return _nt_f16s(x3, weight_f16s(weight), bias, residual, gate, rows_per_batch)
    w3i = weight_image(weight)
    if isinstance(x3, native.PairImage) and not (own_gemm_enabled() and native.gemm_nt_supported(x3, w3i) and (gate is None or rows_per_batch % 256 == 0)):
        x3 = x3.image3()
    if residual is None and bias is None:
        return _nt(x3, w3i)
    if own_gemm_enabled() and native.gemm_nt_supported(x3, w3i) and (gate is None or rows_per_batch % 256 == 0):
        return native.gemm_nt(x3, w3i, bias=bias, residual=residual, gate=gate, rows_per_batch=rows_per_batch)
    return _tail(torch.mm(x3, w3i.t(), out_dtype=torch.float32), bias, residual, gate, rows_per_batch)


def matmul_wx_split3(weight, x3, conv=None):
    from . import native
    if conv is not None:
        cw, cb, seq = conv
        a = weight_f16s(weight) if isinstance(x3, native.F16Image) else weight_image(weight)
        ad, bd = (a.data, x3.data) if isinstance(x3, native.F16Image) else (a, x3)
        ok = (os.environ.get("DIMSUM_INPROJ_CONV", "1") != "0" and own_gemm_enabled() and native.gemm_nt_supported(ad, bd)
              and cw.dtype == torch.float32 and cw.dim() == 2 and cw.stride(1) == 1 and cw.shape[0] % 256 == 0 and 2 <= cw.shape[1] <= 4
              and seq % 4 == 0 and 256 % seq == 0 and x3.shape[0] % seq == 0)
        if ok:
            cbf = None if cb is None else cb.detach().float().contiguous()
            if isinstance(x3, native.F16Image):
                return native.gemm_nt(ad, bd, scales=(a.inv, x3.inv), conv=(cw.detach(), cbf, seq)), True
            return native.gemm_nt(a, x3, conv=(cw.detach(), cbf, seq)), True
        return matmul_wx_split3(weight, x3), False
    if isinstance(x3, native.F16Image):
        return _nt_f16s(weight_f16s(weight), x3)
    w3i = weight_image(weight)
    if isinstance(x3, native.PairImage) and not (own_gemm_enabled() and native.gemm_nt_supported(w3i, x3)):
        x3 = x3.image3()
    return _nt(w3i, x3)


def gated_mlp_hidden_split3(x3, w12, b12):
    from . import native
    if isinstance(x3, native.F16Image):
        w16 = weight_f16s(w12)
        if own_gemm_enabled() and native.gemm_nt_supported(x3.data, w16.data, gated=True):
            return native.gemm_nt(x3.data, w16.data, bias=b12, epilogue="gated_f16", scales=(x3.inv, w16.inv), gate_bound=gated_bound(w12, b12))
        x12 = _nt_f16s(x3, w16)
        return native.rows_f16s(native.gated_gelu_fwd(x12, b12))
    w3i = weight_image(w12)
    if own_gemm_enabled() and native.gemm_nt_supported(x3, w3i, gated=True):
        pair = (w12.shape[0] // 2) % 64 == 0 and os.environ.get("DIMSUM_PAIR_IMAGES", "1") != "0"
        return native.gemm_nt(x3, w3i, bias=b12, epilogue="gated_split3", pair_out=pair)
    if isinstance(x3, native.PairImage):
        x3 = x3.image3()
    return native.gated_gelu_fwd(torch.mm(x3, w3i.t(), out_dtype=torch.float32), b12, split3=True)


def train_pairs_enabled(M, *widths):
    return (own_gemm_enabled() and os.environ.get("DIMSUM_PAIR_IMAGES", "1") != "0" and M % 256 == 0 and M >= 2048
            and all(w % 256 == 0 for w in widths))


def gated_mlp_hidden_split3_train(x3, w12, b12):
    from . import native
    w3i = weight_image(w12)
    if own_gemm_enabled() and native.gemm_nt_supported(x3, w3i, gated=True):
        return native.gemm_nt(x3, w3i, bias=b12, epilogue="gated_split3", keep_x12=True, pair_out=isinstance(x3, native.PairImage))
    if isinstance(x3, native.PairImage):
        x3 = x3.image3()
    x12 = _nt(x3, w3i)
    return native.gated_gelu_fwd(x12, b12, split3=True), x12


def split3_train_enabled(x, weight):
    import os
    if not (_policy in ("default", "f16s") and torch.backends.cuda.matmul.allow_tf32 and os.environ.get("DIMSUM_SPLIT3", "1") != "0"
            and os.environ.get("DIMSUM_SPLIT3_TRAIN", "1") != "0" and x.is_cuda and x.dtype == torch.float32
            and weight.dtype == torch.float32 and x.shape[-1] % 4 == 0 and torch.is_grad_enabled()
            and not torch.is_autocast_enabled("cuda")):
        return False
    if x.numel() // x.shape[-1] < int(os.environ.get("DIMSUM_SPLIT3_MIN_ROWS", "8192")):
        return False
    if _policy == "f16s" and os.environ.get("DIMSUM_F16S_TRAIN", "1") != "0" and own_gemm_enabled():
        return "f16s"
    return True


def attn_bwd_f16_enabled(qkv):
    import os
    return bool(_policy == "f16s" and torch.backends.cuda.matmul.allow_tf32 and os.environ.get("DIMSUM_F16S_TRAIN", "1") != "0"
                and os.environ.get("DIMSUM_SPLIT3_TRAIN", "1") != "0" and os.environ.get("DIMSUM_SPLIT3", "1") != "0"
                and qkv.is_cuda and qkv.dtype == torch.float32 and not torch.is_autocast_enabled("cuda"))


def weight_f16s_train(weight, want_l1=False):
    from . import native
    if _tls.frozen is not None and not torch.cuda.is_current_stream_capturing():
        return weight_f16s(weight, want_l1=want_l1)
    return native.rows_f16s(weight.detach(), want_l1=want_l1)


def train_scope_active():
    return _tls.frozen is not None and not torch.cuda.is_current_stream_capturing()


def weight_t_f16s_train(weight):
    from . import native
    return native.rows_f16s(weight.detach().t().contiguous())


def nt_f16s_any(a, b):
    from . import native
    if own_gemm_enabled() and native.gemm_nt_supported(a.data, b.data):
        return native.gemm_nt(a.data, b.data, scales=(a.inv.reshape(-1), b.inv))
    return torch.mm(a.data, b.data.t(), out_dtype=torch.float32) * a.inv.reshape(-1)[:, None] * b.inv[None, :]


def dx_f16s(dy16, w16):
    from . import native
    a = dy16.data.reshape(-1, dy16.data.shape[-1])
    if own_gemm_enabled() and native.gemm_nn_supported(a, w16.data) and w16.data.shape[0] <= 16384:
        return native.gemm_nn(a, dy16.inv.reshape(-1).contiguous(), w16.data, w16.inv)
    return torch.mm(a.float() * dy16.inv.reshape(-1)[:, None], w16.data.float() * w16.inv[:, None])


def dw_f16s(dy16, x16):
    from . import native
    a, b = dy16.data.reshape(-1, dy16.data.shape[-1]), x16.data.reshape(-1, x16.data.shape[-1])
    ai, bi = dy16.inv.reshape(-1), x16.inv.reshape(-1)
    if own_gemm_enabled() and native.gemm_tn_supported(a, b):
        return native.gemm_tn(a, b, row_invs=(ai.contiguous(), bi.contiguous()))
    return mm_tn(a.float() * ai[:, None], b.float() * bi[:, None])


class _LinearF16sFn(torch.autograd.Function):

    @staticmethod
    def forward(ctx, x, weight):
        from . import native
        K = x.shape[-1]
        x16 = native.rows_f16s(x.reshape(-1, K))
        w16 = weight_f16s_train(weight)
        ctx.save_for_backward(x16.data, x16.inv, w16.data, w16.inv)
        ctx.x_shape = x.shape
        return nt_f16s_any(x16, w16).view(*x.shape[:-1], weight.shape[0])

    @staticmethod
    def backward(ctx, dy):
        from . import native
        xd, xi, wd, wi = ctx.saved_tensors
        N = wd.shape[0]
        M = xd.shape[0]
        dy16 = native.rows_f16s(dy.reshape(M, N).contiguous())
        dx = dw = None
        if ctx.needs_input_grad[0]:
            dx = dx_f16s(dy16, native.F16Image(wd, wi)).view(ctx.x_shape)
        if ctx.needs_input_grad[1]:
            dw = dw_f16s(dy16, native.F16Image(xd, xi))
        return dx, dw
```

### dimsum_amd/mlp.py

```python
import torch
import torch.nn as nn
import torch.nn.functional as F

from . import gemm, native


class _GatedGeluFn(torch.autograd.Function):
    @staticmethod
    def forward(ctx, x12, bias):
        x12 = x12.contiguous()
        ctx.save_for_backward(x12, bias)
        return native.gated_gelu_fwd(x12, bias)

    @staticmethod
    def backward(ctx, dh):
        x12, bias = ctx.saved_tensors
        dx12, dbias = native.gated_gelu_bwd(x12, bias, dh, need_dbias=bias is not None and ctx.needs_input_grad[1])
        return dx12, dbias


def gated_gelu(x12, bias=None):
    return _GatedGeluFn.apply(x12, bias)


class _ModGatedMlpImagesFn(torch.autograd.Function):

    @staticmethod
    def forward(ctx, normed, shift, scale, w12, b12, w3):
        B, L, H = normed.shape
        M = B * L
        normed = normed if normed.stride(-1) == 1 else normed.contiguous()
        pairs = gemm.train_pairs_enabled(M, H, w12.shape[0] // 2, w3.shape[0])
        h3 = native.token_transform(normed, "none", True, scale=scale, shift=shift, split3="pair" if pairs else True)
        b12f = None if b12 is None else b12.float()
        g3, x12 = gemm.gated_mlp_hidden_split3_train(h3.reshape(M, -1), w12, b12f)
        m = gemm.linear_split3(g3, w3)
        ctx.pairs = pairs and isinstance(g3, native.PairImage)
        ctx.save_for_backward(normed, scale, h3.data if pairs else h3, x12, g3.data if ctx.pairs else g3, w12, b12f, w3)
        if pairs and not ctx.pairs:
            raise RuntimeError("mlp: the pair images need the hand-written GEMM for every product of the MLP")
        return m.view(B, L, w3.shape[0])

    @staticmethod
    def backward(ctx, dm):
        normed, scale, h3, x12, g3, w12, b12f, w3 = ctx.saved_tensors
        B, L, H = normed.shape
        M, F2 = x12.shape
        Fh = F2 // 2
        Ho = w3.shape[0]
        if ctx.pairs:
            P = native.PairImage
            dm_w = native.split3_rows(dm.reshape(M, Ho).contiguous(), left="pair")
            dg = native.gemm_nt(dm_w, native.split3_rows(w3.detach().t().contiguous(), left=True), weight_order=True)
            dw3 = gemm.mm_tn(dm_w, P(g3)) if ctx.needs_input_grad[5] else None
            dx12_w, db12 = native.gated_gelu_bwd(x12, b12f, dg, need_dbias=b12f is not None and ctx.needs_input_grad[4], split3="pair")
            dh = native.gemm_nt(dx12_w, native.split3_rows(w12.detach().t().contiguous(), left=True), weight_order=True)
            dw12 = gemm.mm_tn(dx12_w, P(h3.view(M, 2 * H))) if ctx.needs_input_grad[3] else None
        else:
            dm_w = native.split3_rows(dm.reshape(M, Ho).contiguous(), left=False)
            dg = gemm._nt(dm_w, native.split3_rows(w3.detach().t().contiguous(), left=True))
            dw3 = gemm.mm_tn(dm_w.view(3 * M, Ho), g3.view(3 * M, Fh), out_dtype=torch.float32) if ctx.needs_input_grad[5] else None
            dx12_w, db12 = native.gated_gelu_bwd(x12, b12f, dg, need_dbias=b12f is not None and ctx.needs_input_grad[4], split3=True)
            dh = gemm._nt(dx12_w, native.split3_rows(w12.detach().t().contiguous(), left=True))
            dw12 = gemm.mm_tn(dx12_w.view(3 * M, F2), h3.view(3 * M, H), out_dtype=torch.float32) if ctx.needs_input_grad[3] else None
        dh = dh.view(B, L, H)
        dnormed = dshift = dscale = None
        if ctx.needs_input_grad[0] and (ctx.needs_input_grad[1] or ctx.needs_input_grad[2]):
            dnormed, dscale, _, dshift = native.token_transform(dh, "none", True, scale=scale, w=normed, want_y=True, want_tsum=True)
        elif ctx.needs_input_grad[0]:
            dnormed = native.token_transform(dh, "none", False, gate=1.0 + scale)
        elif ctx.needs_input_grad[1] or ctx.needs_input_grad[2]:
            _, dscale, dshift = native.token_transform(normed, "none", True, w=dh, want_y=False, want_wsum=True)
        if db12 is not None and b12f is not None:
            db12 = db12.to(b12f.dtype)
        return dnormed, dshift, dscale, dw12, db12, dw3


class _ModGatedMlpF16sFn(torch.autograd.Function):

    @staticmethod
    def forward(ctx, normed, shift, scale, w12, b12, w3):
        B, L, H = normed.shape
        M = B * L
        normed = normed if normed.stride(-1) == 1 else normed.contiguous()
        h16 = native.token_transform(normed, "none", True, scale=scale, shift=shift, split3="f16s")
        b12f = None if b12 is None else b12.float()
        if gemm.train_scope_active():
            w12_16, bound = gemm.weight_f16s_train(w12), gemm.gated_bound(w12, b12)
        else:
            w12_16, l1 = gemm.weight_f16s_train(w12, want_l1=True)
            bound = torch.cat([l1 * gemm._K10, gemm._absmax(b12f, w12)]).contiguous()
        g16, x12 = native.gemm_nt(h16.data.view(M, H), w12_16.data, bias=b12f, epilogue="gated_f16", scales=(h16.inv.view(M), w12_16.inv), gate_bound=bound, keep_x12=True)
        w3_16 = gemm.weight_f16s_train(w3)
        m = gemm.nt_f16s_any(g16, w3_16)
        ctx.save_for_backward(normed, scale, h16.data, h16.inv, x12, g16.data, g16.inv, w12_16.data, w12_16.inv, b12f, w3_16.data, w3_16.inv)
        return m.view(B, L, w3.shape[0])

    @staticmethod
    def backward(ctx, dm):
        normed, scale, hd, hi, x12, gd, gi, w12d, w12i, b12f, w3d, w3i = ctx.saved_tensors
        B, L, H = normed.shape
        M = B * L
        Ho = w3d.shape[0]
        F16 = native.F16Image
        dm16 = native.rows_f16s(dm.reshape(M, Ho).contiguous())
        dg = gemm.dx_f16s(dm16, F16(w3d, w3i))
        dw3 = gemm.dw_f16s(dm16, F16(gd, gi)) if ctx.needs_input_grad[5] else None
        dx12_16, db12 = native.gated_gelu_bwd(x12, b12f, dg, need_dbias=b12f is not None and ctx.needs_input_grad[4], split3="f16s")
        dh = gemm.dx_f16s(dx12_16, F16(w12d, w12i)).view(B, L, H)
        dw12 = gemm.dw_f16s(dx12_16, F16(hd, hi)) if ctx.needs_input_grad[3] else None
        dnormed = dshift = dscale = None
        if ctx.needs_input_grad[0] and (ctx.needs_input_grad[1] or ctx.needs_input_grad[2]):
            dnormed, dscale, _, dshift = native.token_transform(dh, "none", True, scale=scale, w=normed, want_y=True, want_tsum=True)
        elif ctx.needs_input_grad[0]:
            dnormed = native.token_transform(dh, "none", False, gate=1.0 + scale)
        elif ctx.needs_input_grad[1] or ctx.needs_input_grad[2]:
            _, dscale, dshift = native.token_transform(normed, "none", True, w=dh, want_y=False, want_wsum=True)
        if db12 is not None and b12f is not None:
            db12 = db12.to(b12f.dtype)
        return dnormed, dshift, dscale, dw12, db12, dw3


def f16s_mlp_train_ok(mlp, normed):
    H, F2 = mlp.w12.weight.shape[1], mlp.w12.weight.shape[0]
    M = normed.numel() // normed.shape[-1]
    return M % 256 == 0 and H % 64 == 0 and H >= 128 and H <= 2048 and (F2 // 2) % 128 == 0 and F2 // 2 <= 5120 and mlp.w3.weight.shape[0] % 4 == 0


def mod_gated_mlp_images(mlp, normed, shift, scale):
    if gemm.split3_train_enabled(normed, mlp.w12.weight) == "f16s" and f16s_mlp_train_ok(mlp, normed):
        return _ModGatedMlpF16sFn.apply(normed, shift, scale, mlp.w12.weight, mlp.w12.bias, mlp.w3.weight), mlp.w3.bias
    return _ModGatedMlpImagesFn.apply(normed, shift, scale, mlp.w12.weight, mlp.w12.bias, mlp.w3.weight), mlp.w3.bias


class GatedMLP(nn.Module):
    def __init__(self, in_features, hidden_features=None, out_features=None, act_layer=F.gelu, drop=0.0, bias=True):
        super().__init__()
        out_features = out_features or in_features
        hidden_features = hidden_features or in_features
        self.w12 = nn.Linear(in_features, 2 * hidden_features, bias=bias)
        self.w3 = nn.Linear(hidden_features, out_features, bias=bias)
        self.act_layer = act_layer()
        self._fused = isinstance(self.act_layer, nn.GELU) and self.act_layer.approximate == "tanh"

    def forward_deferred(self, x, x3=None, residual=None, gate=None):
        if x3 is not None:
            b12 = self.w12.bias
            h3 = gemm.gated_mlp_hidden_split3(x3, self.w12.weight, None if b12 is None else b12.float())
            if residual is not None:
                H = self.w3.weight.shape[0]
                b3 = None if self.w3.bias is None else self.w3.bias.float()
                y = gemm.linear_split3(h3, self.w3.weight, bias=b3, residual=residual.reshape(-1, H), gate=gate, rows_per_batch=residual.shape[-2])
                return y.view(residual.shape), None
            return gemm.linear_split3(h3, self.w3.weight).view(*x.shape[:-1], self.w3.weight.shape[0]), self.w3.bias
        if self._fused and x.dtype == torch.float32:
            b12 = self.w12.bias
            h = gated_gelu(gemm.linear(x, self.w12.weight), None if b12 is None else b12.float())
        else:
            x1, x2 = self.w12(x).chunk(2, dim=-1)
            h = self.act_layer(x1) * x2
        return gemm.linear(h, self.w3.weight), self.w3.bias

    def forward(self, x):
        y, b = self.forward_deferred(x)
        return y if b is None else y + b
```

### dimsum_amd/models_dim.py

```python
import math
import os
from functools import partial

import numpy as np
import torch
import torch.nn as nn
import torch.nn.functional as F

from . import scanning_orders as so
from . import gemm
from .attention_fusion import CrossAttentionFusion
from .dct_layer import init_dct_kernel, init_idct_kernel
from .mlp import GatedMLP
from .modules.mamba_simple import CondMamba, Mamba
from .ops import token_ops
from .ops.layernorm import RMSNorm, layer_norm_fn, rms_norm_fn
from .wavelet_layer import DWT_2D, IDWT_2D


def modulate(x, shift, scale):
    return x * (1 + scale.unsqueeze(1)) + shift.unsqueeze(1)


def get_1d_sincos_pos_embed_from_grid(embed_dim, pos):
# ... 108 lines not shown

def _ln_modulate(norm, x, shift, scale, split3=False):
    if torch.is_grad_enabled() or not x.is_cuda or x.dtype != torch.float32 or norm.weight is not None:
        return None
    from . import native
    B, L, H = x.shape
    ones = norm.__dict__.get("_dimsum_ones")
    if ones is None or ones.device != x.device:
        ones = norm.__dict__["_dimsum_ones"] = torch.ones(H, device=x.device, dtype=torch.float32)
    y = native.layer_norm_fwd(x.reshape(B * L, H), ones, None, norm.eps, is_rms_norm=False, mod_scale=scale, mod_shift=shift, rows_per_batch=L,
                              **({"split3": split3} if split3 else {}))[0]
    return y if split3 else y.view(B, L, H)


class FinalLayer(nn.Module):
    def __init__(self, hidden_size, patch_size, out_channels):
        super().__init__()
        self.norm_final = nn.LayerNorm(hidden_size, elementwise_affine=False, eps=1e-6)
        self.linear = nn.Linear(hidden_size, patch_size * patch_size * out_channels, bias=True)
        self.adaLN_modulation = nn.Sequential(nn.SiLU(), nn.Linear(hidden_size, 2 * hidden_size, bias=True))

    def forward(self, x, c):
        shift, scale = _modulation(self.adaLN_modulation, c).chunk(2, dim=1)
        h = _ln_modulate(self.norm_final, x, shift, scale)
        return self.linear(modulate(self.norm_final(x), shift, scale) if h is None else h)


class Attention(nn.Module):

    def __init__(self, dim, num_heads=8, qkv_bias=False, **_):
        super().__init__()
        self.num_heads, self.head_dim = num_heads, dim // num_heads
        self.qkv = nn.Linear(dim, dim * 3, bias=qkv_bias)
        self.proj = nn.Linear(dim, dim)

    def forward_deferred(self, x, x3=None, residual=None, gate=None):
        from . import native
        from .attention_fusion import _XattnCoreFn
        B, N, C = x.shape
        if x3 is not None:
            qb = None if self.qkv.bias is None else self.qkv.bias.float().contiguous()
            in_gemm = qb is not None and native.xattn_supported(x, self.head_dim)
            f16 = isinstance(x3, native.F16Image) and C % 8 == 0 and native.xattn_supported(x, self.head_dim)
            qkv = None
            if f16:
                kvb = gemm.attn_kv_bound(self.qkv.weight, self.qkv.bias)
                qkv = gemm.qkv_f16s(x3.reshape(B * N, -1), self.qkv.weight, self.qkv.bias, N, kvb[0:2])
                if qkv is not None:
                    qkv, in_gemm = qkv.view(B, N, 3 * C), True
            if qkv is None:
                qkv = gemm.linear_split3(x3, self.qkv.weight, **({"bias": qb} if in_gemm else {})).view(B, N, 3 * C)
            if native.xattn_supported(x, self.head_dim):
                if in_gemm:
                    qb = None
                if f16:
                    o3 = native.xattn_fusion_fwd(qkv, None, self.num_heads, bias1=qb, split3="f16s", f16s=(x3.inv.reshape(B, N), None, kvb))
                else:
                    o3 = native.xattn_fusion_fwd(qkv, None, self.num_heads, bias1=qb, split_bf16=True, split3="pair" if isinstance(x3, native.PairImage) else True)
                if residual is not None:
                    pb = None if self.proj.bias is None else self.proj.bias.float()
                    y = gemm.linear_split3(o3.reshape(B * N, -1), self.proj.weight, bias=pb, residual=residual.reshape(B * N, C), gate=gate, rows_per_batch=N)
                    return y.view(B, N, C), None
                return gemm.linear_split3(o3.reshape(B * N, -1), self.proj.weight).view(B, N, C), self.proj.bias
        else:
            qkv = gemm.linear(x, self.qkv.weight)
        if native.xattn_supported(qkv, self.head_dim):
            o = _XattnCoreFn.apply(qkv, None, self.qkv.bias, None, self.num_heads)
        else:
            from .utils import note_torch_path
            note_torch_path(f"Attention (shared DiTBlock) core for head_dim {self.head_dim} / {qkv.dtype}", required_opt_in=True)
            if self.qkv.bias is not None:
                qkv = qkv + self.qkv.bias
            q, k, v = qkv.reshape(B, N, 3, self.num_heads, self.head_dim).permute(2, 0, 3, 1, 4).unbind(0)
            o = torch.nn.functional.scaled_dot_product_attention(q, k, v).transpose(1, 2).reshape(B, N, C)
        return gemm.linear(o, self.proj.weight), self.proj.bias

    def forward(self, x):
        y, b = self.forward_deferred(x)
        return y if b is None else y + b


class Mlp(nn.Module):
    def __init__(self, in_features, hidden_features=None, out_features=None, act_layer=nn.GELU, drop=0.0):
        super().__init__()
        self.fc1 = nn.Linear(in_features, hidden_features or in_features)
        self.act = act_layer()
        self.fc2 = nn.Linear(hidden_features or in_features, out_features or in_features)

    def forward(self, x):
        return self.fc2(self.act(self.fc1(x)))


def drop_path(x, drop_prob=0.0, training=False, scale_by_keep=True):
    if drop_prob == 0.0 or not training:
        return x
    keep = 1 - drop_prob
    mask = x.new_empty((x.shape[0],) + (1,) * (x.ndim - 1)).bernoulli_(keep)
    if keep > 0.0 and scale_by_keep:
        mask.div_(keep)
    return x * mask


class DropPath(nn.Module):
    def __init__(self, drop_prob=0.0, scale_by_keep=True):
        super().__init__()
        self.drop_prob, self.scale_by_keep = drop_prob, scale_by_keep

    def forward(self, x):
        return drop_path(x, self.drop_prob, self.training, self.scale_by_keep)


_approx_gelu = lambda: nn.GELU(approximate="tanh")


def _make_mlp(dim, use_gated_mlp=True):
    cls = GatedMLP if use_gated_mlp else Mlp
    return cls(in_features=dim, hidden_features=int(dim * 4), act_layer=_approx_gelu, drop=0)


def _modulation(seq, c):
    hit = getattr(gemm._tls, "cond", None)
    if hit is not None and hit[0] is c and len(seq) == 2 and isinstance(seq[0], nn.SiLU):
        return seq[1](hit[1])
    return seq(c)


def _mlp_tail(mlp, x, normed, shift, scale, gate):
    if getattr(mlp, "_fused", False) and gemm.split3_train_enabled(normed, mlp.w12.weight):
        from .mlp import mod_gated_mlp_images
        m, mb = mod_gated_mlp_images(mlp, normed, shift, scale)
        return token_ops.gate_residual(x, m, gate, mb)
    h = token_ops.pre_mixer(normed, "none", None, shift, scale)
    if hasattr(mlp, "forward_deferred"):
        m, mb = mlp.forward_deferred(h)
        return token_ops.gate_residual(x, m, gate, mb)
    return token_ops.gate_residual(x, mlp(h), gate, None)


def _mix_through_images(mixer, hidden_states, kind, table, shift, scale, c, fork=False):
    if getattr(mixer, "takes_image", lambda: False)() and gemm.split3_enabled(hidden_states, mixer.in_proj.weight, left=False):
        m = mixer(None, c, x3=token_ops.pre_mixer(hidden_states, kind, table, shift, scale,
                                                  split3=gemm.split3_enabled(hidden_states, mixer.in_proj.weight, left=False)))
        return (m, hidden_states) if fork else m
    if fork and hidden_states.is_cuda and torch.is_grad_enabled() and hidden_states.requires_grad:
        t, hidden_states = token_ops.pre_mixer_fork(hidden_states, kind, table, shift, scale)
        return mixer(t, c), hidden_states
    m = mixer(token_ops.pre_mixer(hidden_states, kind, table, shift, scale), c)
    return (m, hidden_states) if fork else m


class _BlockBase(nn.Module):

    def _prenorm(self, hidden_states, residual):
        if not self.fused_add_norm:
            residual = hidden_states if residual is None else residual + self.drop_path(hidden_states)
            hidden_states = (self.norm(residual) if isinstance(self.norm, nn.Identity)
                             else self.norm(residual.to(dtype=self.norm.weight.dtype)))
            if self.residual_in_fp32:
                residual = residual.to(torch.float32)
            return hidden_states, residual
        fn = rms_norm_fn if isinstance(self.norm, RMSNorm) else layer_norm_fn
        x = hidden_states if residual is None else self.drop_path(hidden_states)
        return fn(x, self.norm.weight, self.norm.bias, residual=residual, prenorm=True,
                  residual_in_fp32=self.residual_in_fp32, eps=self.norm.eps)

    def _table(self, L, device, build):
        cache = self.__dict__.setdefault("_tables", {})
        key = (L, str(device))
        if key not in cache:
            fwd = build(math.isqrt(L))
            mixer = getattr(self, "mixer", None)
            if mixer is not None and getattr(mixer, "_is_zigzag", lambda: False)() and getattr(mixer, "zigzag_paths", None) is not None \
                    and os.environ.get("DIMSUM_FOLD_ZIGZAG", "1") != "0":
                perm = mixer.zigzag_paths[mixer.layer_idx].detach().cpu().numpy().astype(np.int64)
                assert perm.shape[0] == L, "zigzag path length != sequence length"
                fwd = perm if fwd is None else so.compose(fwd, perm)
                mixer._zigzag_folded = True
            if fwd is None:
                cache[key] = None
            else:
                inv = so.reverse_permut_np(fwd)
                cache[key] = {"fwd": so.as_index(fwd, device), "inv": so.as_index(inv, device),
                              "inv32": torch.as_tensor(inv.astype(np.int32), device=device)}
        return cache[key]

    def allocate_inference_cache(self, *a, **k):
        raise NotImplementedError("autoregressive decode caches are outside the denoiser hot path")


class DiMBlockRaw(_BlockBase):

    def __init__(self, dim, mixer_cls, norm_cls=nn.LayerNorm, fused_add_norm=False, residual_in_fp32=False, drop_path=0.0,
                 reverse=False, transpose=False, scanning_continuity=False, c_dim=None):
        super().__init__()
        self.residual_in_fp32, self.fused_add_norm = residual_in_fp32, fused_add_norm
        self.reverse, self.transpose, self.scanning_continuity = reverse, transpose, scanning_continuity
        c_dim = dim if c_dim is None else c_dim
        self.mixer = mixer_cls(dim)
        self.norm = norm_cls(dim)
        self.drop_path = DropPath(drop_path) if drop_path > 0.0 else nn.Identity()
        self.adaLN_modulation = nn.Sequential(nn.SiLU(), nn.Linear(c_dim, 3 * dim, bias=True))

    def _order(self, H):
        if not (self.reverse or self.transpose or self.scanning_continuity):
            return None
        return so.block_order_table(H, self.reverse, self.transpose, self.scanning_continuity)

    def forward(self, hidden_states, residual=None, c=None, inference_params=None, out_split3=False):
        hidden_states, residual = self._prenorm(hidden_states, residual)
        table = self._table(hidden_states.shape[1], hidden_states.device, self._order)
        shift, scale, gate = _modulation(self.adaLN_modulation, c).chunk(3, dim=1)
        m, hidden_states = _mix_through_images(self.mixer, hidden_states, "none", table, shift, scale, c, fork=True)
        return token_ops.post_mixer(hidden_states, m, gate, "none", table, **({"split3": out_split3} if out_split3 else {})), residual


class _FreqBlock(_BlockBase):
    kind = "none"

    def _init_common(self, dim, mixer_cls, norm_cls, fused_add_norm, residual_in_fp32, drop_path, reverse, transpose,
                     scanning_continuity, no_ffn, c_dim):
        self.residual_in_fp32, self.fused_add_norm = residual_in_fp32, fused_add_norm
        self.reverse, self.transpose, self.scanning_continuity, self.no_ffn = reverse, transpose, scanning_continuity, no_ffn
        self._c_dim = dim if c_dim is None else c_dim

    def _finish_common(self, dim, norm_cls, drop_path):
        self.drop_path = DropPath(drop_path) if drop_path > 0.0 else nn.Identity()
        self.adaLN_modulation = nn.Sequential(nn.SiLU(), nn.Linear(self._c_dim, 6 * dim if not self.no_ffn else 3 * dim, bias=True))
        if not self.no_ffn:
            self.norm_2 = norm_cls(dim)
            self.mlp = _make_mlp(dim)

    def forward(self, hidden_states, residual=None, c=None, inference_params=None, out_split3=False):
        hidden_states, residual = self._prenorm(hidden_states, residual)
        table = self._table(hidden_states.shape[1], hidden_states.device, self._order)
        mods = _modulation(self.adaLN_modulation, c).chunk(3 if self.no_ffn else 6, dim=1)
        shift, scale, gate = mods[:3]
        if self.no_ffn:
            m, hidden_states = _mix_through_images(self.mixer, hidden_states, self.kind, table, shift, scale, c, fork=True)
            return token_ops.post_mixer(hidden_states, m, gate, self.kind, table, **({"split3": out_split3} if out_split3 else {})), residual
        assert not out_split3
        t = token_ops.pre_mixer(hidden_states, self.kind, table, torch.zeros_like(shift), torch.zeros_like(scale))
        t = t + gate.unsqueeze(1) * self.mixer(modulate(t, shift, scale), c)
        t = t + mods[5].unsqueeze(1) * self.mlp(modulate(self.norm_2(t), mods[3], mods[4]))
        zero = torch.zeros_like(hidden_states)
        return token_ops.post_mixer(zero, t, torch.ones_like(gate), self.kind, table), residual


class WaveDiMBlock(_FreqBlock):
    kind = "haar"

    def __init__(self, dim, mixer_cls, norm_cls=nn.LayerNorm, fused_add_norm=False, residual_in_fp32=False, drop_path=0.0,
                 reverse=False, transpose=False, scanning_continuity=False, skip=False, no_ffn=False, c_dim=None,
                 window_scan=True, num_wavelet_lv=2):
        super().__init__()
        assert num_wavelet_lv == 2, "only the two-level transform of the published configs is implemented"
        self._init_common(dim, mixer_cls, norm_cls, fused_add_norm, residual_in_fp32, drop_path, reverse, transpose,
                          scanning_continuity, no_ffn, c_dim)
        self.window_scan, self.num_wavelet_lv = window_scan, num_wavelet_lv
        self.mixer = mixer_cls(dim)
        self.norm = norm_cls(dim)
        self.dwt, self.idwt = DWT_2D(wave="haar"), IDWT_2D(wave="haar")
        self._finish_common(dim, norm_cls, drop_path)

    def _order(self, H):
        if self.window_scan:
            tab = so.local_scan_table(H, H // 4, column_first=bool(self.transpose))
        else:
            tab = so.block_order_table(H, False, self.transpose, False)
        return so.compose(tab, so.block_order_table(H, self.reverse, False, self.scanning_continuity))


class DCTBlock(_FreqBlock):
    kind = "dct"

    def __init__(self, dim, mixer_cls, fused_add_norm=False, residual_in_fp32=False, drop_path=0.0, norm_cls=nn.LayerNorm,
                 dct_size=2, reverse=False, transpose=False, scanning_continuity=False, no_ffn=False, c_dim=None):
        super().__init__()
        assert dct_size == 4, "only the 4x4 DCT of DiMBlockCombinedFourier is implemented"
        self._init_common(dim, mixer_cls, norm_cls, fused_add_norm, residual_in_fp32, drop_path, reverse, transpose,
                          scanning_continuity, no_ffn, c_dim)
        self.dim, self.dct_size, self.reserve_kernel = dim, dct_size, dct_size
        self.norm = norm_cls(dim)
        self.mixer = mixer_cls(dim)
        self._finish_common(dim, norm_cls, drop_path)
        self.dct_conv = init_dct_kernel(dim, dct_size, dct_size)
        self.idct_conv = nn.Sequential(init_idct_kernel(dim, dct_size, dct_size), nn.PixelShuffle(dct_size))

    def _order(self, H):
        if not (self.reverse or self.transpose or self.scanning_continuity):
            return None
        return so.block_order_table(H, self.reverse, self.transpose, self.scanning_continuity)


class _ForkHalves(torch.autograd.Function):

    @staticmethod
    def forward(ctx, h):
        C = h.shape[-1] // 2
        return h[..., :C], h[..., C:], h.view_as(h)

    @staticmethod
    def backward(ctx, d1, d2, dres):
        if dres is None:
            return torch.cat((d1, d2), dim=-1)
        C = dres.shape[-1] // 2
        out = torch.empty(dres.shape, device=dres.device, dtype=dres.dtype)
        for d, sl in ((d1, slice(0, C)), (d2, slice(C, 2 * C))):
            if d is None:
                out[..., sl] = dres[..., sl]
            else:
                torch.add(d, dres[..., sl], out=out[..., sl])
        return out


class _CombinedBase(_BlockBase):
    def _init_tail(self, dim, norm_cls, drop_path, use_gated_mlp, swap_k_kw):
        self.proj = CrossAttentionFusion(dim, num_heads=8, qkv_bias=True, **swap_k_kw)
        self.drop_path = DropPath(drop_path) if drop_path > 0.0 else nn.Identity()
        self.norm_2 = norm_cls(dim)
        self.adaLN_modulation = nn.Sequential(nn.SiLU(), nn.Linear(dim, 3 * dim, bias=True))
        self.mlp = _make_mlp(dim, use_gated_mlp)

    def forward(self, hidden_states, residual=None, c=None, inference_params=None):
        hidden_states, residual = self._prenorm(hidden_states, residual)
        if hidden_states.is_cuda and torch.is_grad_enabled() and hidden_states.requires_grad:
            x1, x2, hidden_states = _ForkHalves.apply(hidden_states)
        else:
            x1, x2 = hidden_states.chunk(2, dim=2)
        img = self.proj.takes_images(hidden_states) and gemm.split3_enabled(x1, self.proj.qkv1.weight)
        kw = {"out_split3": img} if img else {}
        if ((not torch.is_grad_enabled()) and hidden_states.is_cuda and branch_streams_enabled()
                and not torch.cuda.is_current_stream_capturing()):
            cur = torch.cuda.current_stream(hidden_states.device)
            side = self.__dict__.get("_side_stream")
            if side is None or side.device != hidden_states.device:
                side = self.__dict__["_side_stream"] = torch.cuda.Stream(device=hidden_states.device)
            side.wait_stream(cur)
            with torch.cuda.stream(side):
                x2, _ = self.freq_mamba(x2, None, c, inference_params, **kw)
            x1, _ = self.spatial_mamba(x1, None, c, inference_params, **kw)
            cur.wait_stream(side)
            x2.record_stream(cur)
        else:
            x1, _ = self.spatial_mamba(x1, None, c, inference_params, **kw)
            x2, _ = self.freq_mamba(x2, None, c, inference_params, **kw)
        fast_tail = (not torch.is_grad_enabled() and isinstance(self.norm_2, RMSNorm) and hasattr(self.mlp, "forward_deferred")
                     and hidden_states.dtype == torch.float32)
        in_epilogue = bool(img) and fast_tail and hidden_states.is_contiguous()
        fused, pb = self.proj.forward_deferred(x1, x2, **({"images": True} if img else {}), **({"residual": hidden_states} if in_epilogue else {}))
        shift, scale, gate = _modulation(self.adaLN_modulation, c).chunk(3, dim=1)
        if fast_tail:
            from . import native
            B, L, H = hidden_states.shape
            s3 = getattr(self.mlp, "_fused", False) and gemm.split3_enabled(hidden_states, self.mlp.w12.weight, producer="norm")
            y, _, _, hnew = native.layer_norm_fwd(fused.reshape(B * L, H), self.norm_2.weight, self.norm_2.bias, self.norm_2.eps,
                                                  residual=None if in_epilogue else hidden_states.reshape(B * L, H), is_rms_norm=True, x_bias=pb,
                                                  mod_scale=scale, mod_shift=shift, rows_per_batch=L, **({"split3": s3} if s3 else {}))
            if s3 and hnew.is_contiguous():
                return self.mlp.forward_deferred(hidden_states, x3=y, residual=hnew.view(B, L, H), gate=gate)[0], residual
            m, mb = self.mlp.forward_deferred(hidden_states, x3=y) if s3 else self.mlp.forward_deferred(y.view(B, L, H))
            return token_ops.gate_residual(hnew.view(B, L, H), m, gate, mb), residual
        hidden_states = token_ops.gate_residual(hidden_states, fused, None, pb)
        if isinstance(self.norm_2, RMSNorm) and hidden_states.is_cuda and torch.is_grad_enabled():
            normed, hidden_states = self.norm_2(hidden_states, prenorm=True)
            return _mlp_tail(self.mlp, hidden_states, normed, shift, scale, gate), residual
        return _mlp_tail(self.mlp, hidden_states, self.norm_2(hidden_states), shift, scale, gate), residual


class DiMBlockCombined(_CombinedBase):

    def __init__(self, dim, mixer_cls, norm_cls=nn.LayerNorm, fused_add_norm=False, residual_in_fp32=False, drop_path=0.0,
                 reverse=False, transpose=False, scanning_continuity=False, use_gated_mlp=True):
        super().__init__()
        self.residual_in_fp32, self.fused_add_norm = residual_in_fp32, fused_add_norm
        self.reverse, self.transpose, self.scanning_continuity = reverse, transpose, scanning_continuity
        self.norm = norm_cls(dim)
        kw = dict(norm_cls=nn.Identity, drop_path=0.0, fused_add_norm=False, residual_in_fp32=residual_in_fp32,
                  scanning_continuity=scanning_continuity, c_dim=dim)
        self.spatial_mamba = DiMBlockRaw(dim // 2, mixer_cls, reverse=reverse, transpose=transpose, **kw)
        self.freq_mamba = WaveDiMBlock(dim // 2, mixer_cls, reverse=False, transpose=reverse, no_ffn=True, num_wavelet_lv=2, **kw)
        self._init_tail(dim, norm_cls, drop_path, use_gated_mlp, dict(swap_k=False))


class DiMBlockCombinedFourier(_CombinedBase):

    def __init__(self, dim, mixer_cls, mixer_cls_2, norm_cls=nn.LayerNorm, fused_add_norm=False, residual_in_fp32=False,
                 drop_path=0.0, reverse=False, transpose=False, scanning_continuity=False, use_gated_mlp=True):
        super().__init__()
        self.residual_in_fp32, self.fused_add_norm = residual_in_fp32, fused_add_norm
        self.reverse, self.transpose, self.scanning_continuity = reverse, transpose, scanning_continuity
        self.norm = norm_cls(dim)
        kw = dict(norm_cls=nn.Identity, drop_path=0.0, fused_add_norm=False, residual_in_fp32=residual_in_fp32,
                  scanning_continuity=scanning_continuity, c_dim=dim)
        self.spatial_mamba = DiMBlockRaw(dim // 2, mixer_cls, reverse=reverse, transpose=transpose, **kw)
        self.freq_mamba = DCTBlock(dim // 2, mixer_cls_2, reverse=False, transpose=False, no_ffn=True, dct_size=4, **kw)
        self._init_tail(dim, norm_cls, drop_path, use_gated_mlp, {})


class DiTBlock(nn.Module):

    def __init__(self, hidden_size, num_heads, mlp_ratio=4.0, use_gated_mlp=True, **block_kwargs):
        super().__init__()
        self.norm1 = nn.LayerNorm(hidden_size, elementwise_affine=False, eps=1e-6)
        self.attn = Attention(hidden_size, num_heads=num_heads, qkv_bias=True, **block_kwargs)
        self.norm2 = nn.LayerNorm(hidden_size, elementwise_affine=False, eps=1e-6)
        cls = GatedMLP if use_gated_mlp else Mlp
        self.mlp = cls(in_features=hidden_size, hidden_features=int(hidden_size * mlp_ratio), act_layer=_approx_gelu, drop=0)
        self.adaLN_modulation = nn.Sequential(nn.SiLU(), nn.Linear(hidden_size, 6 * hidden_size, bias=True))

    def forward(self, x, c=None, **kwargs):
        sa, ca, ga, sm, cm, gm = _modulation(self.adaLN_modulation, c).chunk(6, dim=1)
        s3 = gemm.split3_enabled(x, self.attn.qkv.weight, producer="norm")
        h = _ln_modulate(self.norm1, x, sa, ca, split3=s3)
        from . import native
        if h is not None and s3 and x.is_contiguous() and native.xattn_supported(x, self.attn.head_dim):
            x = self.attn.forward_deferred(x, x3=h, residual=x, gate=ga)[0]
        else:
            if h is not None and s3:
                a, ab = self.attn.forward_deferred(x, x3=h)
            else:
                a, ab = self.attn.forward_deferred(token_ops.pre_mixer(self.norm1(x), "none", None, sa, ca) if h is None else h)
            x = token_ops.gate_residual(x, a, ga, ab)
        s3 = getattr(self.mlp, "_fused", False) and s3
        h = _ln_modulate(self.norm2, x, sm, cm, split3=s3)
        if h is None:
            return _mlp_tail(self.mlp, x, self.norm2(x), sm, cm, gm)
        if hasattr(self.mlp, "forward_deferred"):
            if s3 and x.is_contiguous():
                return self.mlp.forward_deferred(x, x3=h, residual=x, gate=gm)[0]
            m, mb = self.mlp.forward_deferred(x, x3=h) if s3 else self.mlp.forward_deferred(h)
            return token_ops.gate_residual(x, m, gm, mb)
        return token_ops.gate_residual(x, self.mlp(h), gm, None)


def _init_weights(module, n_layer, initializer_range=0.02, rescale_prenorm_residual=True, n_residuals_per_layer=1):
    if isinstance(module, nn.Linear):
        if module.bias is not None and not getattr(module.bias, "_no_reinit", False):
            nn.init.zeros_(module.bias)
    elif isinstance(module, nn.Embedding):
        nn.init.normal_(module.weight, std=initializer_range)
    if rescale_prenorm_residual:
        for name, p in module.named_parameters():
            if name in ("out_proj.weight", "fc2.weight"):
                nn.init.kaiming_uniform_(p, a=math.sqrt(5))
                with torch.no_grad():
                    p /= math.sqrt(n_residuals_per_layer * n_layer)


def create_block(d_model, ssm_cfg=None, norm_epsilon=1e-5, drop_path=0.0, rms_norm=False, residual_in_fp32=True,
                 fused_add_norm=False, layer_idx=None, device=None, dtype=None, scan_type="none", add_bias_linear=False,
                 gated_linear_unit=True, routing_mode="sinkhorn", num_moe_experts=8, mamba_moe_layers=None, is_moe=False,
                 block_type="linear", reverse=False, transpose=False, cond_mamba=False, scanning_continuity=False,
                 skip=False, use_gated_mlp=True, block_kwargs={}, block_kwargs2={}):
    if is_moe:
        raise NotImplementedError("MoE blocks are outside the denoiser hot path (never enabled by a published config)")
    ssm_cfg = ssm_cfg or {}
    fk = {"device": device, "dtype": dtype}
    norm_cls = partial(nn.LayerNorm if not rms_norm else RMSNorm, eps=norm_epsilon, **fk)
    if cond_mamba:
        kw = dict(layer_idx=layer_idx, scan_type=scan_type, d_cond=d_model, **ssm_cfg, **fk)
        kw.update(block_kwargs)
        mixer_cls = partial(CondMamba, **kw)
    else:
        mixer_cls = partial(Mamba, layer_idx=layer_idx, scan_type=scan_type, **ssm_cfg, **fk)
    common = dict(norm_cls=norm_cls, drop_path=drop_path, fused_add_norm=fused_add_norm, residual_in_fp32=residual_in_fp32,
                  scanning_continuity=scanning_continuity)
    if block_type == "raw":
        block = DiMBlockRaw(d_model, mixer_cls, reverse=reverse, transpose=transpose, **common)
    elif block_type == "wave":
        block = WaveDiMBlock(d_model, mixer_cls, reverse=reverse, transpose=transpose, skip=skip, window_scan=False, **common)
    elif block_type == "combined":
        block = DiMBlockCombined(d_model, mixer_cls, reverse=reverse, transpose=transpose, use_gated_mlp=use_gated_mlp, **common)
    elif block_type == "combined_fourier":
        mixer_cls_2 = partial(CondMamba, layer_idx=layer_idx, d_cond=d_model, **ssm_cfg, **block_kwargs2, **fk)
        block = DiMBlockCombinedFourier(d_model, mixer_cls, mixer_cls_2, reverse=reverse, transpose=transpose,
                                        use_gated_mlp=use_gated_mlp, **common)
    else:
        raise NotImplementedError(f"block_type={block_type!r} is outside the denoiser hot path "
                                  "(published configs use 'combined'; also available: raw, wave, combined_fourier)")
    block.layer_idx = layer_idx
    return block


class DiM(nn.Module):
    def __init__(self, img_resolution=32, patch_size=2, in_channels=4, hidden_size=1024, depth=16, label_dropout=0.1,
                 num_classes=1000, learn_sigma=False, ssm_cfg=None, rms_norm=False, residual_in_fp32=True,
                 fused_add_norm=False, scan_type="none", initializer_cfg=None, num_moe_experts=8, mamba_moe_layers=None,
                 add_bias_linear=False, gated_linear_unit=True, routing_mode="top1", is_moe=False, pe_type="ape",
                 block_type="linear", cond_mamba=False, scanning_continuity=False, enable_fourier_layers=False,
                 learnable_pe=False, skip=False, drop_path=0.0, use_final_norm=False, use_attn_every_k_layers=-1,
                 use_gated_mlp=True, use_independent_attn=False):
        super().__init__()
        if pe_type != "ape":
            raise NotImplementedError("only the absolute positional embedding of the published configs is implemented")
        if enable_fourier_layers:
            raise NotImplementedError("enable_fourier_layers is broken in the reference (models_dim.py:1702) and unused")
        self.depth = int(depth * 3) if block_type == "raw" else depth
        self.learn_sigma, self.in_channels = learn_sigma, in_channels
        self.out_channels = in_channels * 2 if learn_sigma else in_channels
        self.patch_size, self.num_classes, self.initializer_cfg = patch_size, num_classes, initializer_cfg
        self.enable_fourier_layers, self.fused_add_norm, self.residual_in_fp32 = False, fused_add_norm, residual_in_fp32
        self.use_attn_every_k_layers, self.use_independent_attn = use_attn_every_k_layers, use_independent_attn
        self.pe_type, self.block_type = pe_type, block_type
        if use_independent_attn:
            n_tb = self.depth // use_attn_every_k_layers - 1
            self.depth = self.depth - self.depth // use_attn_every_k_layers

        self.x_embedder = PatchEmbed(img_resolution, patch_size, in_channels, hidden_size)
        self.t_embedder = TimestepEmbedder(hidden_size)
        self.y_embedder = LabelEmbedder(num_classes, hidden_size, label_dropout)
        num_patches = self.x_embedder.num_patches
        self.pos_embed = nn.Parameter(torch.zeros(1, num_patches, hidden_size), requires_grad=learnable_pe)
        dpr = [x.item() for x in torch.linspace(0, drop_path, self.depth, device="cpu")]
        inter_dpr = [0.0] + dpr
        self.drop_path = DropPath(drop_path) if drop_path > 0.0 else nn.Identity()
        grid = int(math.sqrt(num_patches))

        def gen_paths(N, st):
            kind, n = st.split("_")[0], int(st.split("_")[1])
            zz = so.SCAN_ZOO[kind](N)[:n]
            rev = [so.reverse_permut_np(p) for p in zz]
            return dict(zigzag_paths=torch.cat([torch.from_numpy(p)[None] for p in zz] * self.depth, dim=0),
                        zigzag_paths_reverse=torch.cat([torch.from_numpy(p)[None] for p in rev] * self.depth, dim=0),
                        scan_type=st)

        block_kwargs = gen_paths(grid, scan_type) if scan_type.startswith(("zigma", "sweep", "jpeg")) else {}
        block_kwargs2 = gen_paths(grid, "jpeg_2")
        self.blocks = nn.ModuleList([
            create_block(hidden_size, ssm_cfg=ssm_cfg, norm_epsilon=1e-5, rms_norm=rms_norm, residual_in_fp32=residual_in_fp32,
                         fused_add_norm=fused_add_norm, layer_idx=i, scan_type=scan_type, drop_path=inter_dpr[i],
                         num_moe_experts=num_moe_experts, mamba_moe_layers=mamba_moe_layers, add_bias_linear=add_bias_linear,
                         gated_linear_unit=gated_linear_unit, routing_mode=routing_mode, is_moe=is_moe, block_type=block_type,
                         reverse=(scan_type == "none") and (i % 2 > 0), transpose=(scan_type == "none") and (i % 4 >= 2),
                         cond_mamba=cond_mamba, scanning_continuity=scanning_continuity, use_gated_mlp=use_gated_mlp,
                         block_kwargs=block_kwargs, block_kwargs2=block_kwargs2)
            for i in range(self.depth)])
        if use_attn_every_k_layers > 0:
            if use_independent_attn:
                self.attn_block = nn.ModuleList([DiTBlock(hidden_size, 16, use_gated_mlp=use_gated_mlp) for _ in range(n_tb)])
            else:
                self.attn_block = DiTBlock(hidden_size, 16, use_gated_mlp=use_gated_mlp)
        self.norm_f = (nn.LayerNorm if not rms_norm else RMSNorm)(hidden_size, eps=1e-5) if use_final_norm else None
        self.final_layer = FinalLayer(hidden_size, patch_size, self.out_channels)
        self.initialize_weights()

    def initialize_weights(self):
        pe = get_2d_sincos_pos_embed(self.pos_embed.shape[-1], int(self.x_embedder.num_patches ** 0.5))
        self.pos_embed.data.copy_(torch.from_numpy(pe).float().unsqueeze(0))
        w = self.x_embedder.proj.weight.data
        nn.init.xavier_uniform_(w.view([w.shape[0], -1]))
        nn.init.constant_(self.x_embedder.proj.bias, 0)
        nn.init.normal_(self.y_embedder.embedding_table.weight, std=0.02)
        nn.init.normal_(self.t_embedder.mlp[0].weight, std=0.02)
        nn.init.normal_(self.t_embedder.mlp[2].weight, std=0.02)
        for block in self.blocks:
            nn.init.constant_(block.adaLN_modulation[-1].weight, 0)
            nn.init.constant_(block.adaLN_modulation[-1].bias, 0)
        nn.init.constant_(self.final_layer.adaLN_modulation[-1].weight, 0)
        nn.init.constant_(self.final_layer.adaLN_modulation[-1].bias, 0)
        nn.init.constant_(self.final_layer.linear.weight, 0)
        nn.init.constant_(self.final_layer.linear.bias, 0)
        self.apply(partial(_init_weights, n_layer=self.depth, **(self.initializer_cfg or {})))

    def unpatchify(self, x):
        c, p = self.out_channels, self.x_embedder.patch_size[0]
        h = w = int(x.shape[1] ** 0.5)
        assert h * w == x.shape[1]
        x = x.reshape(x.shape[0], h, w, p, p, c)
        return torch.einsum("nhwpqc->nchpwq", x).reshape(x.shape[0], c, h * p, h * p)

    def forward(self, x, t, y=None, inference_params=None, **kwargs):
        if t is None:
            t = torch.randint(0, 1000, (x.shape[0],), device=x.device)
        if y is None:
            y = torch.ones(x.size(0), dtype=torch.long, device=x.device) * (self.y_embedder.get_in_channels() - 1)
        with gemm.forward_scope(self, x.shape[0] * self.x_embedder.num_patches):
            return self._forward(x, t, y, inference_params)

    def _forward(self, x, t, y, inference_params):
        c = self.t_embedder(t) + self.y_embedder(y, self.training)
        gemm._tls.cond = (c, F.silu(c)) if os.environ.get("DIMSUM_FORWARD_MEMO", "1") != "0" else None
        try:
            return self._forward_blocks(x, c, inference_params)
        finally:
            gemm._tls.cond = None

    def _forward_blocks(self, x, c, inference_params):
        x = self.x_embedder(x) + self.pos_embed
        residual = None
        for idx, block in enumerate(self.blocks):
            x, residual = block(x, residual, c, inference_params=inference_params)
            if self.use_attn_every_k_layers > 0 and (idx + 1) % self.use_attn_every_k_layers == 0:
                if self.use_independent_attn:
                    x = self.attn_block[(idx + 1) // self.use_attn_every_k_layers - 1](x, c)
                else:
                    x = self.attn_block(x, c)
        if self.norm_f is not None:
            if not self.fused_add_norm:
                residual = x if residual is None else residual + self.drop_path(x)
                x = self.norm_f(residual.to(dtype=self.norm_f.weight.dtype))
            else:
                fn = rms_norm_fn if isinstance(self.norm_f, RMSNorm) else layer_norm_fn
                x = fn(self.drop_path(x), self.norm_f.weight, self.norm_f.bias, eps=self.norm_f.eps, residual=residual,
                       prenorm=False, residual_in_fp32=self.residual_in_fp32)
        return self.unpatchify(self.final_layer(x, c))

    def forward_with_cfg(self, x, t, y=None, inference_params=None, cfg_scale=1.0, **kwargs):
        half = x[: len(x) // 2]
        out = self.forward(torch.cat([half, half], dim=0), t, y, inference_params)
        eps, rest = out[:, : self.in_channels], out[:, self.in_channels:]
        cond, uncond = torch.split(eps, len(eps) // 2, dim=0)
        g = uncond + cfg_scale * (cond - uncond)
        return torch.cat([torch.cat([g, g], dim=0), rest], dim=1)

    def forward_with_adacfg(self, x, t, y=None, inference_params=None, cfg_scale=3.8, scale_pow=4.0, **kwargs):
        if cfg_scale is None:
            return self.forward(x, t, y, inference_params)
        half = x[: len(x) // 2]
        out = self.forward(torch.cat([half, half], dim=0), t, y, inference_params)
        eps, rest = out[:, : self.in_channels], out[:, self.in_channels:]
        cond, uncond = torch.split(eps, len(eps) // 2, dim=0)
        step = (1 - torch.cos(((1 - t) ** scale_pow) * math.pi)) / 2
        s = ((cfg_scale - 1) * step + 1)[: len(x) // 2].view(-1, 1, 1, 1)
        g = uncond + s * (cond - uncond)
        return torch.cat([torch.cat([g, g], dim=0), rest], dim=1)


def _zoo(depth, hidden_size, patch_size):
    def make(**kwargs):
        return DiM(depth=depth, hidden_size=hidden_size, patch_size=patch_size, initializer_cfg=None, ssm_cfg=None, **kwargs)
    return make


DiM_XL_2, DiM_L_2, DiM_L_2_v1 = _zoo(24, 1152, 2), _zoo(16, 1024, 2), _zoo(20, 1024, 2)
DiM_B_2, DiM_L_4, DiM_L_4_v1 = _zoo(12, 768, 2), _zoo(16, 1024, 4), _zoo(20, 1024, 4)
DiM_S_2 = _zoo(12, 384, 2)

DiM_models = {"DiM-XL/2": DiM_XL_2, "DiM-L/2": DiM_L_2, "DiM-L/2-v1": DiM_L_2_v1, "DiM-B/2": DiM_B_2,
              "DiM-L/4": DiM_L_4, "DiM-L/4-v1": DiM_L_4_v1, "DiM-S/2": DiM_S_2}
```

### dimsum_amd/native.py

```python
import contextlib

import os

import torch

from . import _lib

_DT = {torch.float32: _lib.F32, torch.float16: _lib.F16, torch.bfloat16: _lib.BF16}


class _ZeroArena:
    CHUNK = 1 << 22

    def __init__(self):
        import threading
        self._lock, self._cur = threading.Lock(), {}

    def take(self, n, device):
        n = int(n)
        if n <= 0 or n > self.CHUNK // 4 or torch.cuda.is_current_stream_capturing() or os.environ.get("DIMSUM_ZERO_ARENA", "1") == "0":
            return torch.zeros(max(n, 0), device=device, dtype=torch.float32)
        pad = (n + 63) // 64 * 64
        key = (str(device), torch.cuda.current_stream(device).cuda_stream)
        with self._lock:
# ... 751 lines not shown
            splits *= 2
    _check(M % (splits * 64) == 0 and M // splits >= 128, "gemm_tn_pairs: splits must cut M into ranges of whole 64-row tiles")
    out = torch.empty((3 * splits, P, Q), device=ad.device, dtype=torch.float32)
    G = _lib.GemmParams()
    G.m, G.n, G.k = P, Q, M
    G.operand_dtype, G.epilogue, G.out_scale = _DT[ad.dtype], _lib.GEMM_EPI_F32, 1.0
    G.lda, G.ldb, G.ldc = ad.stride(0), bd.stride(0), Q
    G.a_ptr, G.b_ptr, G.c_ptr = _ptr(ad), _ptr(bd), _ptr(out)
    X = _lib.attach_ext(G, _lib.GemmExt)
    X.tn_pair_a_cols, X.tn_pair_b_cols = P, Q
    with torch.cuda.device(ad.device):
        _lib.check(_lib.load().dimsum_gemm_tn(G, 3 * splits, P * Q, _stream(ad)), "gemm_tn_pairs")
    return out.sum(0)


def row_factors(a_inv, b_inv=None):
    _gpu(a_inv, b_inv)
    a_inv = a_inv.reshape(-1)
    _check(a_inv.dtype == torch.float32 and a_inv.is_contiguous() and (b_inv is None or (b_inv.dtype == torch.float32 and b_inv.numel() == a_inv.numel())),
           "row_factors: (R,) float32 inverse scales")
    if b_inv is not None:
        b_inv = b_inv.reshape(-1).contiguous()
    fac = torch.empty(a_inv.numel(), device=a_inv.device, dtype=torch.float16)
    top = torch.empty(1, device=a_inv.device, dtype=torch.float32)
    with torch.cuda.device(a_inv.device):
        _lib.check(_lib.load().dimsum_row_factors(_ptr(a_inv), _ptr(b_inv), a_inv.numel(), _ptr(fac), _ptr(top), _stream(a_inv)), "row_factors")
    return fac, top


def gemm_tn(a, b, splits=None, events=None, alias_rows=0, scales=None, row_scales=None, row_invs=None):
    _gpu(a, b)
    blocks = None
    if row_invs is not None:
        ia, ib = row_invs
        _gpu(ia, ib)
        _check(row_scales is None and scales is None and not alias_rows and a.dtype == torch.float16 and ia.dtype == torch.float32 and ia.numel() == a.shape[0]
               and ia.is_contiguous() and (ib is None or (ib.dtype == torch.float32 and ib.numel() == a.shape[0] and ib.is_contiguous())),
               "gemm_tn: row_invs = (a_inv (R,), b_inv (R,) or None) float32 with float16 operands")
        if os.environ.get("DIMSUM_ROW_FACTORS_KERNEL", "0") == "1":
            row_scales, row_invs = row_factors(ia, ib), None
    if row_scales is not None:
        kf, cs = row_scales
        _gpu(kf, cs)
        _check(scales is None and not alias_rows and a.dtype == torch.float16 and kf.dtype == torch.float16 and kf.numel() == a.shape[0] and kf.is_contiguous()
               and cs.dtype == torch.float32 and cs.numel() == 1, "gemm_tn: row_scales = (k_fac (R,) float16, c_scale (1,) float32) with float16 operands")
    if scales is not None:
        _gpu(*scales)
        sa, sb = scales
        _check(a.dtype == torch.float16 and not alias_rows and sa.dtype == torch.float32 and sb.dtype == torch.float32 and sb.numel() == b.shape[1] and sb.is_contiguous(),
               "gemm_tn: scales = (a_inv, b_inv (Q,)) float32 with float16 operands")
        if sa.dim() == 2:
            _check(sa.shape[0] == a.shape[1] // 32 and sa.shape[1] >= a.shape[0] // 64 and sa.stride(1) == 1 and a.shape[0] <= 4096 and a.shape[1] % 32 == 0,
                   "gemm_tn: a block table must be (P / 32, R / 64) float32, R <= 4096")
            blocks = sa
        else:
            _check(sa.numel() == a.shape[1] and sa.is_contiguous(), "gemm_tn: a_inv must be (P,)")
        splits = 1
    if alias_rows:
        _check(a.dim() == 2 and a.shape[0] == 2 * alias_rows and b.shape[0] == 3 * alias_rows and alias_rows % 64 == 0 and gemm_tn_supported(a[:alias_rows], b[:alias_rows]),
               "gemm_tn: alias_rows = D takes a (2 D, P) plane pair and a (3 D, Q) row stack, D % 64 == 0")
        R, P = 3 * alias_rows, a.shape[1]
        splits = 1
    else:
        _check(gemm_tn_supported(a, b), "gemm_tn: unsupported operands (R % 64, P % 256, Q % 256, 16-bit rows, 16-byte aligned)")
        R, P = a.shape
    Q = b.shape[1]
    if splits is None:
        rowfac = row_scales is not None or row_invs is not None
        splits = gemm_tn_splits(R, P, Q, second_round=not rowfac)
        while rowfac and R // splits > 16384 and R % (2 * splits * 64) == 0:
            splits *= 2
    if row_scales is not None or row_invs is not None:
        _check(R // splits <= 16384, "gemm_tn: row factors need ranges of at most 16384 reduction rows")
    _check(splits >= 1 and R % (splits * 64) == 0 and R // splits >= 128, "gemm_tn: splits must cut R into ranges of whole 64-row tiles (>= 2)")
    out = torch.empty((splits, P, Q), device=a.device, dtype=torch.float32)
    G = _lib.GemmParams()
    G.m, G.n, G.k = P, Q, R
    G.operand_dtype = _DT[a.dtype]
    G.epilogue = _lib.GEMM_EPI_F32
    G.out_scale = 1.0
    G.lda, G.ldb, G.ldc = a.stride(0), b.stride(0), Q
    G.a_ptr, G.b_ptr, G.c_ptr = _ptr(a), _ptr(b), _ptr(out)
    X = _lib.attach_ext(G, _lib.GemmExt)
    X.a_alias_rows = alias_rows
    if scales is not None:
        G.b_inv_scale_ptr = _ptr(scales[1])
        if blocks is not None:
            X.a_block_inv_ptr, X.a_block_inv_ld = _ptr(blocks), blocks.stride(0)
        else:
            G.a_inv_scale_ptr = _ptr(scales[0])
    if row_scales is not None:
        X.k_scale_ptr, X.c_scale_ptr = _ptr(row_scales[0]), _ptr(row_scales[1])
    if row_invs is not None:
        X.k_inv_a_ptr, X.k_inv_b_ptr = _ptr(row_invs[0]), _ptr(row_invs[1])
    if events is not None:
        X.timing_start_event, X.timing_stop_event = events
    with torch.cuda.device(a.device):
        _lib.check(_lib.load().dimsum_gemm_tn(G, splits, P * Q, _stream(a)), "gemm_tn")
    return out[0] if splits == 1 else out.sum(0)


_gemm_kernel_log = None


@contextlib.contextmanager
def gemm_kernel_log():
    global _gemm_kernel_log
    old, _gemm_kernel_log = _gemm_kernel_log, []
    try:
        yield _gemm_kernel_log
    finally:
        _gemm_kernel_log = old


def gemm_nn_supported(a, b):
    if not (a.is_cuda and a.dim() == 2 and b.dim() == 2 and a.dtype == torch.float16 and b.dtype == torch.float16):
        return False
    P, R = a.shape
    Q = b.shape[1]
    return (b.shape[0] == R and R % 64 == 0 and R >= 128 and P % 256 == 0 and Q % 256 == 0 and a.stride(1) == 1 and b.stride(1) == 1
            and a.stride(0) % 8 == 0 and b.stride(0) % 8 == 0 and a.data_ptr() % 16 == 0 and b.data_ptr() % 16 == 0
            and 256 * a.stride(0) * 2 < 2 ** 31 and 64 * b.stride(0) * 2 + 512 < 2 ** 31)


def gemm_nn(a, a_inv, b, b_inv, splits=None):
    _gpu(a, a_inv, b, b_inv)
    _check(gemm_nn_supported(a, b) and a_inv.dtype == torch.float32 and a_inv.numel() == a.shape[0] and a_inv.is_contiguous()
           and b_inv.dtype == torch.float32 and b_inv.numel() == b.shape[0], "gemm_nn: unsupported operands")
    P, R = a.shape
    Q = b.shape[1]
    if splits is None:
        splits = gemm_tn_splits(R, P, Q, second_round=False)
        while R // splits > 16384 and R % (2 * splits * 64) == 0:
            splits *= 2
    _check(splits >= 1 and R % (splits * 64) == 0 and 128 <= R // splits <= 16384, "gemm_nn: splits must cut R into ranges of 2 .. 256 whole 64-row tiles")
    in_kernel = os.environ.get("DIMSUM_ROW_FACTORS_KERNEL", "0") != "1" and b_inv.is_contiguous()
    fac, top = (None, None) if in_kernel else row_factors(b_inv)
    out = torch.empty((splits, P, Q), device=a.device, dtype=torch.float32)
    G = _lib.GemmParams()
    G.m, G.n, G.k = P, Q, R
    G.operand_dtype, G.epilogue, G.out_scale = _DT[a.dtype], _lib.GEMM_EPI_F32, 1.0
    G.lda, G.ldb, G.ldc = a.stride(0), b.stride(0), Q
    G.a_ptr, G.b_ptr, G.c_ptr, G.a_inv_scale_ptr = _ptr(a), _ptr(b), _ptr(out), _ptr(a_inv)
    X = _lib.attach_ext(G, _lib.GemmExt)
    if in_kernel:
        X.k_inv_a_ptr = _ptr(b_inv)
    else:
        X.k_scale_ptr, X.c_scale_ptr = _ptr(fac), _ptr(top)
    with torch.cuda.device(a.device):
        _lib.check(_lib.load().dimsum_gemm_nn(G, splits, P * Q, _stream(a)), "gemm_nn")
    return out[0] if splits == 1 else out.sum(0)


def gemm_nt(a, b, bias=None, epilogue="f32", out=None, out_scale=1.0, events=None, tune=None, scales=None, gate_bound=None, residual=None,
            gate=None, rows_per_batch=None, keep_x12=False, pair_out=False, weight_order=False, q_cols=None, conv=None):
    pair_in = isinstance(a, PairImage)
    pair_b = isinstance(b, PairImage)
    if pair_in:
        a = a.data
    if pair_b:
        b = b.data
    _gpu(a, b, bias)
    gated = epilogue in ("gated_split3", "gated_f16")
    _check(not (pair_in and pair_b) and not (pair_b and (gated or residual is not None or bias is not None)), "gemm_nt: a right-hand pair goes with the plain fp32 epilogue")
    _check(gemm_nt_supported(a, b, gated, pair=pair_in, pair_b=pair_b), "gemm_nt: unsupported operands (M % 256, K % 64, K >= 128, 16-bit K-contiguous rows, 16-byte aligned)")
    M, K = a.shape[0], (a.shape[1] if pair_b else b.shape[1])
    N = b.shape[0]
    P = _lib.GemmParams()
    X = _lib.attach_ext(P, _lib.GemmExt)
    P.m, P.n, P.k = M, N, K
    if pair_in:
        X.a_alias_rows = K // 3
        X.a_alias_weight_order = int(bool(weight_order))
    if pair_b:
        X.b_alias_rows = K // 3
    P.operand_dtype = _DT[a.dtype]
    P.out_scale = float(out_scale)
    P.lda, P.ldb = a.stride(0), b.stride(0)
    if bias is not None:
        _check(bias.dtype == torch.float32 and bias.is_contiguous() and bias.numel() == N, "gemm_nt: bias must be (N,) float32")
    if epilogue == "f32":
        P.epilogue = _lib.GEMM_EPI_F32 if bias is None else _lib.GEMM_EPI_F32_BIAS
        if out is None:
            out = torch.empty((M, N), device=a.device, dtype=torch.float32)
        _check(out.dtype == torch.float32 and out.shape == (M, N) and out.stride(1) == 1, "gemm_nt: out must be (M, N) float32 rows")
        if conv is not None:
            cw, cb, seq = conv
            _gpu(cw, cb)
            _check(bias is None and residual is None and cw.dtype == torch.float32 and cw.dim() == 2 and cw.stride(1) == 1 and cw.shape[0] % 256 == 0
                   and cw.shape[0] <= M and 2 <= cw.shape[1] <= 4 and 256 % seq == 0 and seq % 4 == 0 and N % seq == 0
                   and (cb is None or (cb.dtype == torch.float32 and cb.is_contiguous() and cb.numel() == cw.shape[0])),
                   "gemm_nt: conv = (weight (rows % 256 == 0, width 2..4) f32, bias or None, seq with 256 % seq == 0)")
            P.epilogue = _lib.GEMM_EPI_F32_CONV
            X.conv_weight_ptr, X.conv_bias_ptr = _ptr(cw), _ptr(cb)
            X.conv_rows, X.conv_width, X.conv_seq, X.conv_weight_ld = cw.shape[0], cw.shape[1], seq, cw.stride(0)
        if residual is not None:
            _gpu(residual, gate)
            _check(residual.dtype == torch.float32 and residual.shape == (M, N) and residual.stride(1) == 1, "gemm_nt: residual must be (M, N) float32 rows")
            P.epilogue = _lib.GEMM_EPI_F32_GATE_RESIDUAL
            X.residual_ptr, X.residual_ld = _ptr(residual), residual.stride(0)
            if gate is not None:
                _check(rows_per_batch and rows_per_batch % 256 == 0 and M % rows_per_batch == 0 and gate.dtype == torch.float32
                       and gate.shape == (M // rows_per_batch, N) and gate.stride(1) == 1, "gemm_nt: gate must be (M / rows_per_batch, N) float32, rows_per_batch % 256 == 0")
                X.gate_ptr, X.gate_ld, X.rows_per_batch = _ptr(gate), gate.stride(0), rows_per_batch
    elif epilogue == "gated_split3":
        P.epilogue = _lib.GEMM_EPI_GATED_GELU_SPLIT3
        pieces = 2 if pair_out else 3
        X.c_image_pieces = pieces
        if out is None:
            out = torch.empty((M, pieces * (N // 2)), device=a.device, dtype=torch.bfloat16)
        _check(out.dtype == torch.bfloat16 and out.shape == (M, pieces * (N // 2)) and out.stride(1) == 1, "gemm_nt: out must be (M, 3F) / (M, 2F) bfloat16 rows")
    elif epilogue == "f16_qkv":
        P.epilogue = _lib.GEMM_EPI_F16_QKV
        _check(scales is not None and gate_bound is not None and rows_per_batch and rows_per_batch % 256 == 0 and M % rows_per_batch == 0
               and q_cols and q_cols % 16 == 0 and N % 8 == 0, "gemm_nt: f16_qkv needs scales, gate_bound = {wl1, bmax}, rows_per_batch % 256 == 0, q_cols % 16 == 0")
        X.rows_per_batch, X.qkv_q_cols = rows_per_batch, q_cols
        if out is None:
            out = torch.empty((M, N), device=a.device, dtype=torch.float16)
        _check(out.dtype == torch.float16 and out.shape == (M, N) and out.stride(1) == 1, "gemm_nt: out must be (M, N) float16 rows")
    elif epilogue == "gated_f16":
        P.epilogue = _lib.GEMM_EPI_GATED_GELU_F16
        if out is None:
            out = torch.empty((M, N // 2), device=a.device, dtype=torch.float16)
        _check(out.dtype == torch.float16 and out.shape == (M, N // 2) and out.stride(1) == 1, "gemm_nt: out must be (M, F) float16 rows")
    else:
        raise ValueError(f"gemm_nt: unknown epilogue {epilogue!r}")
    P.ldc = out.stride(0)
    h_inv = None
    if scales is not None:
        sa, sb = scales
        _gpu(sa, sb)
        _check(sa.dtype == torch.float32 and sb.dtype == torch.float32 and sa.is_contiguous() and sb.is_contiguous() and sa.numel() == M
               and sb.numel() == N, "gemm_nt: scales must be contiguous float32 (M,) and (N,)")
        P.a_inv_scale_ptr, P.b_inv_scale_ptr = _ptr(sa), _ptr(sb)
        if gate_bound is not None:
            _gpu(gate_bound)
            _check(epilogue in ("gated_f16", "f16_qkv") and gate_bound.dtype == torch.float32 and gate_bound.numel() == 2 and gate_bound.is_contiguous(),
                   "gemm_nt: gate_bound is a 2-element float32 tensor for the gated_f16 / f16_qkv epilogues")
            X.gate_bound_ptr = _ptr(gate_bound)
            if epilogue == "gated_f16":
                h_inv = torch.empty((M,), device=a.device, dtype=torch.float32)
                X.h_inv_scale_ptr = _ptr(h_inv)
    P.a_ptr, P.b_ptr, P.bias_ptr, P.c_ptr = _ptr(a), _ptr(b), _ptr(bias), _ptr(out)
    x12 = None
    if keep_x12:
        _check((epilogue == "gated_split3" and a.dtype == torch.bfloat16 and scales is None) or (epilogue == "gated_f16" and a.dtype == torch.float16 and h_inv is not None),
               "gemm_nt: keep_x12 goes with the gated_split3 epilogue over bf16 images or the gated_f16 epilogue over scaled-fp16 operands with gate_bound")
        x12 = torch.empty((M, N), device=a.device, dtype=torch.float32)
        X.x12_ptr, X.x12_ld = _ptr(x12), N
    if events is not None:
        X.timing_start_event, X.timing_stop_event = events
    if tune is not None:
        X.tune_variant, X.tune_group_m = tune[:2]
        X.tune_reserved = tune[2] if len(tune) > 2 else 0
    elif epilogue == "gated_f16" and os.environ.get("DIMSUM_GEMM_PERSIST", "1") == "0":
        X.tune_variant = 513
    with torch.cuda.device(a.device):
        if _gemm_kernel_log is not None:
            _gemm_kernel_log.append((epilogue if conv is None else "f32_conv", int(_lib.load().dimsum_gemm_nt_kernel_for(P))))
        _lib.check(_lib.load().dimsum_gemm_nt(P, _stream(a)), "gemm_nt")
    if x12 is not None:
        if h_inv is not None:
            return F16Image(out, h_inv), x12
        return (PairImage(out) if pair_out else out), x12
    if pair_out:
        return PairImage(out)
    return out if h_inv is None else F16Image(out, h_inv)


def gated_gelu_bwd(x12, bias, dh, need_dbias=True, split3=False):
    _gpu(x12, bias, dh)
    dh = dh.contiguous()
    H = x12.shape[-1] // 2
    if split3 == "f16s":
        _check(x12.is_contiguous() and x12.dtype == torch.float32 and dh.dtype == torch.float32 and H % 4 == 0 and H <= 5120, "gated_gelu_bwd: the f16s image needs contiguous float32 rows, H % 4 == 0, H <= 5120")
        rows = x12.numel() // (2 * H)
        img = torch.empty(x12.shape, device=x12.device, dtype=torch.float16)
        inv = torch.empty(x12.shape[:-1], device=x12.device, dtype=torch.float32)
        dbias = _zeros(2 * H, x12.device) if (bias is not None and need_dbias) else None
        with torch.cuda.device(x12.device):
            _lib.check(_lib.load().dimsum_gated_gelu_bwd_f16s(_ptr(x12), _ptr(bias), _ptr(dh), _ptr(img), _ptr(inv), _ptr(dbias), rows, H, _stream(x12)), "gated_gelu_bwd")
        return F16Image(img, inv), dbias
    pair = split3 == "pair"
    dx12 = torch.empty(x12.shape[:-1] + ((4 if pair else 6) * H,), device=x12.device, dtype=torch.bfloat16) if split3 else torch.empty_like(x12)
    dbias = _zeros(2 * H, x12.device) if (bias is not None and need_dbias) else None
    rows = x12.numel() // (2 * H)
    with torch.cuda.device(x12.device):
        lib = _lib.load()
        fn = lib.dimsum_gated_gelu_bwd_pair if pair else (lib.dimsum_gated_gelu_bwd_split3 if split3 else lib.dimsum_gated_gelu_bwd)
        _lib.check(fn(_ptr(x12), _ptr(bias), _ptr(dh), _ptr(dx12), _ptr(dbias), rows, H, _stream(x12)), "gated_gelu_bwd")
    return (PairImage(dx12) if pair else dx12), dbias


def xattn_supported(qkv, head_dim):
    return qkv.is_cuda and qkv.dtype == torch.float32 and qkv.stride(-1) == 1 and head_dim in (24, 32, 48, 64, 72)


def xattn_fusion_fwd(qkv1, qkv2, heads, need_lse=False, bias1=None, bias2=None, split_bf16=None, split3=False, f16s=None):
    self_attn = qkv2 is None
    if split_bf16 is None:
        split_bf16 = bool(torch.backends.cuda.matmul.allow_tf32)
    _gpu(qkv1, qkv2, bias1, bias2)
    _check(self_attn or (bias1 is None) == (bias2 is None), "xattn_fusion: pass both biases or none")
    for bb in (bias1, bias2):
        if bb is not None:
            _check(bb.dtype == torch.float32 and bb.numel() == qkv1.shape[2] and bb.is_contiguous(), "xattn_fusion: bad bias")
    B, L, W = qkv1.shape
    hd = W // (3 * heads)
    qkv_f16 = qkv1.dtype == torch.float16
    _check((qkv1.dtype == torch.float32 or (qkv_f16 and f16s is not None and bias1 is None and bias2 is None)) and qkv1.stride(2) == 1, "xattn_fusion: bad qkv")
    if not self_attn:
        _check(qkv1.shape == qkv2.shape and qkv2.dtype == qkv1.dtype and qkv1.stride() == qkv2.stride(), "xattn_fusion: qkv1/qkv2 must share shape, dtype and strides")
    nd = 1 if self_attn else 2
    out_inv = None
    if f16s is not None:
        x1_inv, x2_inv, kv_bound = f16s
        _gpu(x1_inv, x2_inv, kv_bound)
        _check(x1_inv.dtype == torch.float32 and x1_inv.numel() == B * L and x1_inv.is_contiguous()
               and (self_attn or (x2_inv is not None and x2_inv.dtype == torch.float32 and x2_inv.numel() == B * L and x2_inv.is_contiguous()))
               and kv_bound.dtype == torch.float32 and kv_bound.numel() == 4 and kv_bound.is_contiguous(), "xattn_fusion: bad f16s arguments")
        _check(split3 in (False, "f16s"), "xattn_fusion: the fp16 kernel writes fp32 or the scaled-fp16 image")
    if split3 == "f16s":
        _check(f16s is not None and (heads * hd) % 8 == 0, "xattn_fusion: the scaled-fp16 image needs the fp16 kernel")
        out = torch.empty((B, L, nd * heads * hd), device=qkv1.device, dtype=torch.float16)
        out_inv = torch.empty((B, L), device=qkv1.device, dtype=torch.float32)
    elif split3:
        _check(split_bf16, "xattn_fusion: the operand image output exists for the split-bf16 kernel only")
        out = torch.empty((B, L, (2 if split3 == "pair" else 3) * nd * heads * hd), device=qkv1.device, dtype=torch.bfloat16)
    else:
        out = torch.empty((B, L, nd * heads * hd), device=qkv1.device, dtype=torch.float32)
    lse = torch.empty((B, nd, heads, L), device=qkv1.device, dtype=torch.float32) if need_lse else None
    if B > 0:
        P = _lib.XattnParams()
        P.batch, P.seqlen, P.heads, P.head_dim, P.scale, P.n_dirs = B, L, heads, hd, hd ** -0.5, nd
        P.qkv_batch_stride, P.qkv_token_stride = qkv1.stride(0), qkv1.stride(1)
        P.out_batch_stride, P.out_token_stride = out.stride(0), out.stride(1)
        P.qkv1_ptr, P.qkv2_ptr, P.out_ptr, P.lse_ptr = _ptr(qkv1), _ptr(qkv2), _ptr(out), _ptr(lse)
        P.bias1_ptr, P.bias2_ptr = _ptr(bias1), _ptr(bias2)
        P.precision = 1 if split_bf16 else 0
        P.out_split3 = _SPLIT_MODE.get(split3, int(bool(split3)))
        if f16s is not None:
            P.precision = 2
            P.qkv_f16 = int(qkv_f16)
            P.x1_inv_ptr, P.x2_inv_ptr, P.kv_bound_ptr, P.out_inv_ptr = _ptr(x1_inv), _ptr(x2_inv), _ptr(kv_bound), _ptr(out_inv)
        with torch.cuda.device(qkv1.device):
            _lib.check(_lib.load().dimsum_xattn_fusion_fwd(P, _stream(qkv1)), "xattn_fusion_fwd")
    if out_inv is not None:
        out = F16Image(out, out_inv)
    elif split3 == "pair":
        out = PairImage(out)
    return (out, lse) if need_lse else out


def xattn_fusion_bwd(qkv1, qkv2, out, lse, dout, heads, bias1=None, bias2=None, split_bf16=None, f16=False):
    self_attn = qkv2 is None
    _gpu(qkv1, qkv2, out, lse, dout, bias1, bias2)
    B, L, W = qkv1.shape
    hd = W // (3 * heads)
    nd = 1 if self_attn else 2
    _check(qkv1.dtype == torch.float32 and qkv1.stride(2) == 1, "xattn_fusion_bwd: bad qkv")
    if not self_attn:
        _check(qkv1.shape == qkv2.shape and qkv1.stride() == qkv2.stride(), "xattn_fusion_bwd: bad qkv2")
    _check(tuple(out.shape) == (B, L, nd * heads * hd) and out.stride(2) == 1 and tuple(lse.shape) == (B, nd, heads, L) and lse.is_contiguous(), "xattn_fusion_bwd: bad out / lse")
    if dout.stride() != out.stride():
        dout, out = dout.contiguous(), out.contiguous()
    _check(self_attn or (bias1 is None) == (bias2 is None), "xattn_fusion_bwd: pass both biases or none")
    dqkv1 = torch.empty((B, L, W), device=qkv1.device, dtype=torch.float32)
    dqkv2 = None if self_attn else torch.empty((B, L, W), device=qkv1.device, dtype=torch.float32)
    delta = torch.empty((2 if f16 else 1, B, nd, heads, L), device=qkv1.device, dtype=torch.float32)
    if B > 0:
        Q = _lib.XattnBwdParams()
        P = Q.fwd
        P.batch, P.seqlen, P.heads, P.head_dim, P.scale, P.n_dirs = B, L, heads, hd, hd ** -0.5, nd
        P.qkv_batch_stride, P.qkv_token_stride = qkv1.stride(0), qkv1.stride(1)
        P.out_batch_stride, P.out_token_stride = out.stride(0), out.stride(1)
        P.qkv1_ptr, P.qkv2_ptr, P.out_ptr, P.lse_ptr = _ptr(qkv1), _ptr(qkv2), _ptr(out), _ptr(lse)
        P.bias1_ptr, P.bias2_ptr = _ptr(bias1), _ptr(bias2)
        if split_bf16 is None:
            split_bf16 = bool(torch.backends.cuda.matmul.allow_tf32)
        P.precision = 2 if f16 else (1 if split_bf16 else 0)
        Q.dqkv_batch_stride, Q.dqkv_token_stride = dqkv1.stride(0), dqkv1.stride(1)
        Q.dout_ptr, Q.dqkv1_ptr, Q.dqkv2_ptr, Q.delta_ptr = _ptr(dout), _ptr(dqkv1), _ptr(dqkv2), _ptr(delta)
        with torch.cuda.device(qkv1.device):
            _lib.check(_lib.load().dimsum_xattn_fusion_bwd(Q, _stream(qkv1)), "xattn_fusion_bwd")
    return dqkv1, dqkv2


def optim_tables(numels, device):
    _check(len(numels) > 0 and all(int(n) > 0 for n in numels), "optim_tables: a non-empty list of non-empty tensors is required")
    n = torch.tensor([int(v) for v in numels], dtype=torch.int64)
    per = (n + _lib.OPTIM_CHUNK - 1) // _lib.OPTIM_CHUNK
    _check(int(per.sum()) < 2 ** 31 and int(per.max()) < 2 ** 31, "optim_tables: too many chunks for int32 indices")
    tensor = torch.repeat_interleave(torch.arange(len(numels), dtype=torch.int64), per)
    first = torch.cumsum(per, 0) - per
    chunk = torch.arange(int(per.sum()), dtype=torch.int64) - first[tensor]
    return n.to(device), torch.stack([tensor, chunk], 1).to(torch.int32).contiguous().to(device)


def optim_write_ptrs(table, first, ptrs):
    _gpu(table)
    _check(table.dtype == torch.int64 and table.is_contiguous() and 0 <= first and first + len(ptrs) <= table.numel(),
           "optim_write_ptrs: the table is a contiguous int64 tensor that holds [first, first + len(ptrs))")
    if not ptrs:
        return
    lib = _lib.load()
    arr = (_lib.vp * len(ptrs))(*ptrs)
    with torch.cuda.device(table.device):
        _lib.check(lib.dimsum_optim_write_ptrs(table.data_ptr(), first, arr, len(ptrs), _stream(table)), "dimsum_optim_write_ptrs")


def optim_grad_sumsq(P, device):
    with torch.cuda.device(device):
        _lib.check(_lib.load().dimsum_optim_grad_sumsq(P, torch.cuda.current_stream(device).cuda_stream), "dimsum_optim_grad_sumsq")
# ... 6 lines not shown
```

### include/dimsum_hip.h

```cpp
#ifndef DIMSUM_HIP_H
#define DIMSUM_HIP_H

#include <stdint.h>

#ifdef __cplusplus
extern "C" {
#endif

#define DIMSUM_ABI_VERSION 18

typedef enum {
    DIMSUM_OK = 0,
    DIMSUM_ERR_NULL = 1,
    DIMSUM_ERR_DTYPE = 2,
    DIMSUM_ERR_SHAPE = 3,
    DIMSUM_ERR_STRIDE = 4,
    DIMSUM_ERR_UNSUPPORTED = 5,
    DIMSUM_ERR_LAUNCH = 6,
    DIMSUM_ERR_ABI = 7
} dimsum_status_t;

typedef enum { DIMSUM_F32 = 0, DIMSUM_F16 = 1, DIMSUM_BF16 = 2 } dimsum_dtype_t;

const char *dimsum_status_string(int status);
// ... 153 lines not shown
    int32_t x_dtype, residual_dtype, out_dtype;
    float eps;
    int64_t x_row_stride, residual_row_stride, y_row_stride, residual_out_row_stride;
    const void *x_ptr, *residual_ptr, *weight_ptr, *bias_ptr;
    void *y_ptr, *residual_out_ptr, *mean_ptr, *rstd_ptr;
    const void *xbias_ptr;
    const void *mod_scale_ptr, *mod_shift_ptr;
    int64_t mod_row_stride;
    int32_t rows_per_batch;
    int32_t y_split3;
    void *y_inv_scale_ptr;
} dimsum_norm_params_t;

typedef struct {
    uint32_t struct_size;
    int32_t rows, cols;
    int32_t is_rms_norm;
    float eps;
    int32_t reserved;
    int64_t r_row_stride, dy_row_stride, dres_row_stride, dx_row_stride;
    const void *r_ptr;
    const void *weight_ptr, *mean_ptr, *rstd_ptr;
    const void *dy_ptr;
    const void *dres_ptr;
    void *dx_ptr;
    void *dweight_ptr, *dbias_ptr;
} dimsum_norm_bwd_params_t;

int dimsum_norm_fwd(const dimsum_norm_params_t *p, void *stream);
int dimsum_norm_bwd(const dimsum_norm_bwd_params_t *p, void *stream);

int dimsum_split3(const void *src, int64_t rows, int64_t cols, int64_t src_row_stride, void *dst, int32_t left, void *stream);
int dimsum_split3_t(const void *src, int64_t rows, int64_t cols, int64_t src_row_stride, void *dst, void *stream);

int dimsum_rows_f16s(const void *src, int64_t rows, int64_t cols, int64_t src_row_stride, void *dst, int64_t dst_row_stride,
                     void *inv_scale, void *l1max, void *stream);

int dimsum_rows_block_f16s(const void *src, int64_t rows, int64_t cols, int64_t src_row_stride, void *dst, int64_t dst_row_stride, void *table,
                           int64_t table_ld, void *stream);

typedef struct {
    const void *src;
    void *dst;
    void *inv_scale_ptr;
    void *l1max_ptr;
    void *absmax_ptr;
    int64_t rows, cols, src_row_stride, dst_row_stride;
    float l1_factor;
    int32_t reserved;
} dimsum_f16s_job_t;
int dimsum_rows_f16s_multi(const dimsum_f16s_job_t *jobs, int32_t n_jobs, void *stream);

typedef enum {
    DIMSUM_TT_NONE = 0, DIMSUM_TT_HAAR_FWD = 1, DIMSUM_TT_HAAR_INV = 2, DIMSUM_TT_DCT_FWD = 3, DIMSUM_TT_DCT_INV = 4
} dimsum_tt_kind_t;

typedef struct {
    uint32_t struct_size;
    int32_t batch, tokens, channels, grid;
    int32_t kind;
    int32_t y_split3;
    int64_t x_batch_stride, x_token_stride;
    int64_t res_batch_stride, res_token_stride;
    int64_t y_batch_stride, y_token_stride;
    int64_t mod_batch_stride;
    int64_t w_batch_stride, w_token_stride;
    int64_t red_batch_stride;
    const void *x_ptr;
    const int32_t *in_index_ptr, *out_index_ptr;
    const void *gate_ptr, *scale_ptr, *shift_ptr, *residual_ptr;
    void *y_ptr;
    const void *w_ptr;
    void *wdot_ptr, *wsum_ptr;
    void *tsum_ptr;
    void *y_inv_scale_ptr;
    int32_t y_f16s_lds_offset;
    int32_t reserved;
} dimsum_tt_params_t;

int dimsum_token_transform(const dimsum_tt_params_t *p, void *stream);

typedef struct {
    uint32_t struct_size;
    int32_t batch, seqlen, heads, head_dim;
    float scale;
    int32_t n_dirs;
    int64_t qkv_batch_stride, qkv_token_stride;
    int64_t out_batch_stride, out_token_stride;
    const void *qkv1_ptr, *qkv2_ptr;
    void *out_ptr, *lse_ptr;
    const void *bias1_ptr, *bias2_ptr;
    int32_t precision;
    int32_t out_split3;
    const void *x1_inv_ptr, *x2_inv_ptr, *kv_bound_ptr;
    void *out_inv_ptr;
    int32_t qkv_f16;
    int32_t reserved2;
} dimsum_xattn_params_t;

int dimsum_xattn_fusion_fwd(const dimsum_xattn_params_t *p, void *stream);

typedef struct {
    uint32_t struct_size;
    uint32_t reserved;
    dimsum_xattn_params_t fwd;
    int64_t dqkv_batch_stride, dqkv_token_stride;
    const void *dout_ptr;
    void *dqkv1_ptr, *dqkv2_ptr, *delta_ptr;
} dimsum_xattn_bwd_params_t;

int dimsum_xattn_fusion_bwd(const dimsum_xattn_bwd_params_t *p, void *stream);

int dimsum_gated_gelu_fwd(const void *x12, const void *bias, void *h, int64_t rows, int64_t hidden, void *stream);
int dimsum_gated_gelu_fwd_split3(const void *x12, const void *bias, void *h3, int64_t rows, int64_t hidden, void *stream);
int dimsum_gated_gelu_bwd(const void *x12, const void *bias, const void *dh, void *dx12, void *dbias, int64_t rows,
                          int64_t hidden, void *stream);
int dimsum_gated_gelu_bwd_split3(const void *x12, const void *bias, const void *dh, void *dx12_image, void *dbias, int64_t rows,
                                 int64_t hidden, void *stream);
int dimsum_gated_gelu_bwd_pair(const void *x12, const void *bias, const void *dh, void *dx12_pair, void *dbias, int64_t rows, int64_t hidden, void *stream);
int dimsum_gated_gelu_bwd_f16s(const void *x12, const void *bias, const void *dh, void *dx12_image, void *inv_scale, void *dbias, int64_t rows,
                               int64_t hidden, void *stream);

typedef enum {
    DIMSUM_GEMM_EPI_F32 = 0, DIMSUM_GEMM_EPI_GATED_GELU_SPLIT3 = 1, DIMSUM_GEMM_EPI_GATED_GELU_F16 = 2, DIMSUM_GEMM_EPI_F32_BIAS = 3,
    DIMSUM_GEMM_EPI_F32_GATE_RESIDUAL = 4,
    DIMSUM_GEMM_EPI_F32_CONV = 6,
    DIMSUM_GEMM_EPI_F16_QKV = 5
} dimsum_gemm_epilogue_t;

typedef struct {
    uint32_t struct_size;
    int32_t rows_per_batch;
    void *timing_start_event, *timing_stop_event;
    int32_t tune_variant, tune_group_m, tune_reserved;
    int32_t c_image_pieces;
    const void *gate_bound_ptr;
    void *h_inv_scale_ptr;
    const void *residual_ptr, *gate_ptr;
    int64_t residual_ld, gate_ld;
    void *x12_ptr;
    int64_t x12_ld;
    int64_t a_alias_rows;
    int64_t b_alias_rows;
    int32_t a_alias_weight_order, qkv_q_cols;
    const void *conv_weight_ptr, *conv_bias_ptr;
    int32_t conv_rows, conv_width, conv_seq, conv_weight_ld;
    const void *a_block_inv_ptr;
    int64_t a_block_inv_ld;
    int64_t tn_pair_a_cols, tn_pair_b_cols;
    const void *k_scale_ptr;
    const void *c_scale_ptr;
    const void *k_inv_a_ptr;
    const void *k_inv_b_ptr;
} dimsum_gemm_ext_t;

typedef struct {
    uint32_t struct_size;
    int32_t m, n, k;
    int32_t operand_dtype;
    int32_t epilogue;
    float out_scale;
    int32_t reserved;
    int64_t lda, ldb, ldc;
    const void *a_ptr, *b_ptr, *bias_ptr;
    void *c_ptr;
    const void *a_inv_scale_ptr;
    const void *b_inv_scale_ptr;
    const dimsum_gemm_ext_t *ext;
} dimsum_gemm_params_t;

int dimsum_gemm_nt(const dimsum_gemm_params_t *p, void *stream);
int dimsum_gemm_nt_kernel_for(const dimsum_gemm_params_t *p);

int dimsum_gemm_tn(const dimsum_gemm_params_t *p, int32_t splits, int64_t c_split_stride, void *stream);

int dimsum_gemm_nn(const dimsum_gemm_params_t *p, int32_t splits, int64_t c_split_stride, void *stream);
int dimsum_row_factors(const void *a_inv, const void *b_inv, int64_t n, void *k_scale, void *c_scale, void *stream);

#ifdef __cplusplus
}
#endif
#endif
```

Before: 3475 latents/s.

## Fold the residual-stream add into the gated MLP down-projection GEMM epilogue

Adds a second residual operand to the gate+residual GEMM epilogue, so the down-projection writes residual2 + residual + gate*y straight to a second output. The model forward uses it in inference whenever the next block starts with a fused RMSNorm. That block's prenorm then normalizes the already-summed stream and skips its own residual add. This removes a separate elementwise add and one read/write pass over the f32 residual stream per block, at the cost of an extra residual load in the epilogue, a halved residual prefetch group size, and falling back from the persistent kernel variant when the fold is active.

```diff
diff --git a/dimsum_amd/_lib.py b/dimsum_amd/_lib.py
--- a/dimsum_amd/_lib.py
+++ b/dimsum_amd/_lib.py
@@ -136,7 +136,8 @@
                    ("a_alias_weight_order", i32), ("qkv_q_cols", i32), ("conv_weight_ptr", vp), ("conv_bias_ptr", vp),
                    ("conv_rows", i32), ("conv_width", i32), ("conv_seq", i32), ("conv_weight_ld", i32),
                    ("a_block_inv_ptr", vp), ("a_block_inv_ld", i64), ("tn_pair_a_cols", i64), ("tn_pair_b_cols", i64),
-                   ("k_scale_ptr", vp), ("c_scale_ptr", vp), ("k_inv_a_ptr", vp), ("k_inv_b_ptr", vp)])
+                   ("k_scale_ptr", vp), ("c_scale_ptr", vp), ("k_inv_a_ptr", vp), ("k_inv_b_ptr", vp),
+                   ("residual2_ptr", vp), ("out2_ptr", vp), ("residual2_ld", i64), ("out2_ld", i64)])
 
 
 class GemmParams(_Sized):
diff --git a/dimsum_amd/csrc/gemm_nt.hip b/dimsum_amd/csrc/gemm_nt.hip
--- a/dimsum_amd/csrc/gemm_nt.hip
+++ b/dimsum_amd/csrc/gemm_nt.hip
@@ -75,7 +75,9 @@
         if (frc != DIMSUM_OK) return frc;
     }
     const gemm_flat_t *p = &flat;
-    if (!p->a_ptr || !p->b_ptr || !p->c_ptr) return DIMSUM_ERR_NULL;
+    const bool res2 = p->residual2_ptr != nullptr;
+    if (res2 && p->epilogue != DIMSUM_GEMM_EPI_F32_GATE_RESIDUAL) return DIMSUM_ERR_UNSUPPORTED;
+    if (!p->a_ptr || !p->b_ptr || (!p->c_ptr && !res2)) return DIMSUM_ERR_NULL;
     if (p->operand_dtype != DIMSUM_F16 && p->operand_dtype != DIMSUM_BF16) return DIMSUM_ERR_DTYPE;
     if (p->m <= 0 || p->n <= 0 || p->k < 2 * kBK || p->m % kBM != 0 || p->k % kBK != 0 || p->n % 4 != 0) return DIMSUM_ERR_SHAPE;
     if (p->a_alias_rows != 0 && (p->a_alias_rows < 0 || p->a_alias_rows % kBK != 0 || p->k != 3 * p->a_alias_rows)) return DIMSUM_ERR_SHAPE;
@@ -117,7 +119,7 @@
     if (p->tune_variant == 512 && bf) return DIMSUM_ERR_UNSUPPORTED;
     if (p->epilogue == DIMSUM_GEMM_EPI_F32_GATE_RESIDUAL) {
         if (!p->residual_ptr) return DIMSUM_ERR_NULL;
-        if (p->ldc % 4 != 0 || p->ldc < p->n || !aligned_to<char>(p->c_ptr, 16) || p->residual_ld % 4 != 0 || p->residual_ld < p->n ||
+        if ((p->c_ptr && (p->ldc % 4 != 0 || p->ldc < p->n || !aligned_to<char>(p->c_ptr, 16))) || p->residual_ld % 4 != 0 || p->residual_ld < p->n ||
             !aligned_to<char>(p->residual_ptr, 16) || (p->bias_ptr && !aligned_to<char>(p->bias_ptr, 16)) ||
             (p->gate_ptr && (p->gate_ld % 4 != 0 || !aligned_to<char>(p->gate_ptr, 16))))
             return DIMSUM_ERR_STRIDE;
@@ -131,6 +133,18 @@
         a.N = p->n;
         a.tiles_n = (p->n + kBN - 1) / kBN;
         constexpr int kShipR = kVarFullLineStores | kVarNtStores;
+        if (res2) {
+            if (!bf && !m128 && p->tune_variant == 514 && p->n % kBN == 0 && persist_ok(a, p->tune_variant)) return DIMSUM_ERR_UNSUPPORTED;
+            if (!p->out2_ptr) return DIMSUM_ERR_NULL;
+            if (p->residual2_ld % 4 != 0 || p->residual2_ld < p->n || !aligned_to<char>(p->residual2_ptr, 16) || p->out2_ld % 4 != 0 || p->out2_ld < p->n ||
+                !aligned_to<char>(p->out2_ptr, 16) || (int64_t)257 * p->out2_ld * 4 >= ((int64_t)1 << 31))
+                return DIMSUM_ERR_STRIDE;
+            a.res2 = reinterpret_cast<const float *>(p->residual2_ptr);
+            a.out2 = reinterpret_cast<float *>(p->out2_ptr);
+            a.ldr2 = p->residual2_ld; a.ldo2 = p->out2_ld;
+            constexpr int kShipR2 = kShipR | kVarRes2;
+            return bf ? launch<kOpBf16, kEpiF32GateRes, kShipR2>(a, s, e0, e1, probe) : launch_f16<kEpiF32GateRes, kShipR2>(a, s, e0, e1, m128, probe);
+        }
         if (!bf && !m128 && p->tune_variant == 514 && p->n % kBN == 0 && persist_ok(a, p->tune_variant)) return launch_persist<kOpF16, kEpiF32GateRes, kShipR>(a, s, e0, e1, probe);
         return bf ? launch<kOpBf16, kEpiF32GateRes, kShipR>(a, s, e0, e1, probe) : launch_f16<kEpiF32GateRes, kShipR>(a, s, e0, e1, m128, probe);
     }
diff --git a/dimsum_amd/csrc/gemm_nt_kernel.hpp b/dimsum_amd/csrc/gemm_nt_kernel.hpp
--- a/dimsum_amd/csrc/gemm_nt_kernel.hpp
+++ b/dimsum_amd/csrc/gemm_nt_kernel.hpp
@@ -29,6 +29,9 @@
     float *inv_out;
     const float *res, *gate;
     int64_t ldr, ldg;
+    const float *res2;
+    float *out2;
+    int64_t ldr2, ldo2;
     int rows_per_batch;
     int64_t lda, ldb, ldc;
     int M, N, K;
@@ -55,7 +58,7 @@
     int q_cols;
     int c_pieces2;
 };
-enum { kVarLgkmAfterBarrier = 1, kVarNoEpilogue = 2, kVarNtStores = 4, kVarFullLineStores = 8, kVarNoSetprio = 16, kVarSc1Stores = 32, kVarSc0Stores = 64, kVarKeepX12 = 128, kVarTN = 256, kVarM128 = 512, kVarRebase = 1024, kVarPersist = 2048, kVarRowFac = 4096, kVarNN = 8192 };
+enum { kVarLgkmAfterBarrier = 1, kVarNoEpilogue = 2, kVarNtStores = 4, kVarFullLineStores = 8, kVarNoSetprio = 16, kVarSc1Stores = 32, kVarSc0Stores = 64, kVarKeepX12 = 128, kVarTN = 256, kVarM128 = 512, kVarRebase = 1024, kVarPersist = 2048, kVarRowFac = 4096, kVarNN = 8192, kVarRes2 = 16384 };
 
 __device__ __forceinline__ float dpp_row_ror8(float x) {
     const int v = __builtin_bit_cast(int, x);
@@ -626,6 +629,8 @@
     {
     const int lane = lane_e;
     const int ecol = wc * 32 + (lane >> 4) * 4;
+    constexpr bool kRes2 = (kVar & kVarRes2) != 0;
+    static_assert(!kRes2 || (kEpi == kEpiF32GateRes && (kVar & kVarFullLineStores) != 0), "the second residual operand serves the gate + residual epilogue");
     if constexpr (kVar & kVarNoEpilogue) {
 #pragma unroll
         for (int mi = 0; mi < 2; ++mi)
@@ -756,9 +761,12 @@
                         rs[mi][i][0] = pick(ms, sap[lrow], 1.0f); rs[mi][i][1] = pick(ms, sap[lrow + 8], 1.0f);
                     }
                 }
-            constexpr int kGS = kPersist ? DIMSUM_PERSIST_GS : 4, kNG = 16 / kGS;
-            f4 rr[2][kGS][2];
+            constexpr int kGS = (kPersist ? DIMSUM_PERSIST_GS : 4) / (kRes2 ? 2 : 1), kNG = 16 / kGS;
+            f4 rr[2][kGS][2], rr2[2][kRes2 ? kGS : 1][2];
             float rg[2][kGS][2];
+            const bool has_c = !kRes2 || p.C != nullptr;
+            __amdgpu_buffer_rsrc_t rsrc2 = rsrc;
+            if constexpr (kRes2) rsrc2 = __builtin_amdgcn_make_buffer_rsrc(p.out2 + (int64_t)m0 * p.ldo2 + n0, 0, 0x7fffffff, 0x00020000);
             auto load_res = [&](int g) {
                 if constexpr (kEpi == kEpiF32GateRes) {
                     const int t0 = g * kGS, ni = t0 >> 3, mi = (t0 >> 2) & 1;
@@ -775,6 +783,15 @@
                         const int i = (t0 + k) & 3;
                         rr[g & 1][k][0] = *reinterpret_cast<const f4 *>(rp + (int64_t)(i * 16) * p.ldr);
                         rr[g & 1][k][1] = *reinterpret_cast<const f4 *>(rp + (int64_t)(i * 16 + 8) * p.ldr);
+                    }
+                    if constexpr (kRes2) {
+                        const float *rp2 = p.res2 + (int64_t)(m0 + frow + mi * kMiRows) * p.ldr2 + (live[ni] ? n0 + ni * 128 + fcol : 0);
+#pragma unroll
+                        for (int k = 0; k < kGS; ++k) {
+                            const int i = (t0 + k) & 3;
+                            rr2[g & 1][k][0] = *reinterpret_cast<const f4 *>(rp2 + (int64_t)(i * 16) * p.ldr2);
+                            rr2[g & 1][k][1] = *reinterpret_cast<const f4 *>(rp2 + (int64_t)(i * 16 + 8) * p.ldr2);
+                        }
                     }
                 }
             };
@@ -807,7 +824,15 @@
                         s0 = s0 + bv[ni];
                         s1 = s1 + bv[ni];
                     }
-                    if (live[ni]) {
+                    if constexpr (kRes2) {
+                        const f4 t0 = rr2[g & 1][k][0] + s0, t1 = rr2[g & 1][k][1] + s1;
+                        const unsigned voff2 = (unsigned)((lrow * p.ldo2 + col) * 4);
+                        if (live[ni]) {
+                            store_f4<kAux>(rsrc2, voff2, t0);
+                            store_f4<kAux>(rsrc2, voff2 + (unsigned)(8 * p.ldo2 * 4), t1);
+                        }
+                    }
+                    if (has_c && live[ni]) {
                         store_f4<kAux>(rsrc, voff, s0);
                         store_f4<kAux>(rsrc, voff + (unsigned)(8 * p.ldc * 4), s1);
                     }
diff --git a/dimsum_amd/gemm.py b/dimsum_amd/gemm.py
--- a/dimsum_amd/gemm.py
+++ b/dimsum_amd/gemm.py
@@ -469,35 +469,50 @@
     return y if kw.get("bias") is None else y + kw["bias"]
 
 
-def _tail(y, bias, residual, gate, rows_per_batch):
+def _tail(y, bias, residual, gate, rows_per_batch, res2=None):
     if bias is not None:
         y = y + bias
     if residual is None:
         return y
     if gate is not None:
         y = (y.view(-1, rows_per_batch, y.shape[-1]) * gate.unsqueeze(1)).view(y.shape)
-    return residual + y
-
-
-def _nt_f16s(a, b, bias=None, residual=None, gate=None, rows_per_batch=None):
+    y = residual + y
+    return y if res2 is None else res2 + y
+
+
+def res_epilogue_enabled():
+    import os
+    return os.environ.get("DIMSUM_RES_EPILOGUE", "1") != "0"
+
+
+def _nt_res(native, a, b, res2, **kw):
+    if res2 is None:
+        return native.gemm_nt(a, b, **kw)
+    if native.gemm_nt_res2_supported(a, b):
+        return native.gemm_nt(a, b, res2=res2, **kw)
+    return res2 + native.gemm_nt(a, b, **kw)
+
+
+def _nt_f16s(a, b, bias=None, residual=None, gate=None, rows_per_batch=None, res2=None):
     from . import native
     if own_gemm_enabled() and native.gemm_nt_supported(a.data, b.data) and (gate is None or rows_per_batch % 256 == 0):
-        return native.gemm_nt(a.data, b.data, bias=bias, scales=(a.inv, b.inv), residual=residual, gate=gate, rows_per_batch=rows_per_batch)
-    return _tail(torch.mm(a.data, b.data.t(), out_dtype=torch.float32) * a.inv[:, None] * b.inv[None, :], bias, residual, gate, rows_per_batch)
-
-
-def linear_split3(x3, weight, bias=None, residual=None, gate=None, rows_per_batch=None):
-    from . import native
+        return _nt_res(native, a.data, b.data, res2, bias=bias, scales=(a.inv, b.inv), residual=residual, gate=gate, rows_per_batch=rows_per_batch)
+    return _tail(torch.mm(a.data, b.data.t(), out_dtype=torch.float32) * a.inv[:, None] * b.inv[None, :], bias, residual, gate, rows_per_batch, res2)
+
+
+def linear_split3(x3, weight, bias=None, residual=None, gate=None, rows_per_batch=None, res2=None):
+    from . import native
+    assert res2 is None or residual is not None, "linear_split3: res2 goes with residual"
     if isinstance(x3, native.F16Image):
-        return _nt_f16s(x3, weight_f16s(weight), bias, residual, gate, rows_per_batch)
+        return _nt_f16s(x3, weight_f16s(weight), bias, residual, gate, rows_per_batch, res2)
     w3i = weight_image(weight)
     if isinstance(x3, native.PairImage) and not (own_gemm_enabled() and native.gemm_nt_supported(x3, w3i) and (gate is None or rows_per_batch % 256 == 0)):
         x3 = x3.image3()
     if residual is None and bias is None:
         return _nt(x3, w3i)
     if own_gemm_enabled() and native.gemm_nt_supported(x3, w3i) and (gate is None or rows_per_batch % 256 == 0):
-        return native.gemm_nt(x3, w3i, bias=bias, residual=residual, gate=gate, rows_per_batch=rows_per_batch)
-    return _tail(torch.mm(x3, w3i.t(), out_dtype=torch.float32), bias, residual, gate, rows_per_batch)
+        return _nt_res(native, x3, w3i, res2, bias=bias, residual=residual, gate=gate, rows_per_batch=rows_per_batch)
+    return _tail(torch.mm(x3, w3i.t(), out_dtype=torch.float32), bias, residual, gate, rows_per_batch, res2)
 
 
 def matmul_wx_split3(weight, x3, conv=None):
diff --git a/dimsum_amd/mlp.py b/dimsum_amd/mlp.py
--- a/dimsum_amd/mlp.py
+++ b/dimsum_amd/mlp.py
@@ -143,14 +143,16 @@
         self.act_layer = act_layer()
         self._fused = isinstance(self.act_layer, nn.GELU) and self.act_layer.approximate == "tanh"
 
-    def forward_deferred(self, x, x3=None, residual=None, gate=None):
+    def forward_deferred(self, x, x3=None, residual=None, gate=None, res2=None):
+        assert res2 is None or (x3 is not None and residual is not None), "forward_deferred: res2 goes with x3 and residual"
         if x3 is not None:
             b12 = self.w12.bias
             h3 = gemm.gated_mlp_hidden_split3(x3, self.w12.weight, None if b12 is None else b12.float())
             if residual is not None:
                 H = self.w3.weight.shape[0]
                 b3 = None if self.w3.bias is None else self.w3.bias.float()
-                y = gemm.linear_split3(h3, self.w3.weight, bias=b3, residual=residual.reshape(-1, H), gate=gate, rows_per_batch=residual.shape[-2])
+                y = gemm.linear_split3(h3, self.w3.weight, bias=b3, residual=residual.reshape(-1, H), gate=gate, rows_per_batch=residual.shape[-2],
+                                       **({} if res2 is None else {"res2": res2.reshape(-1, H)}))
                 return y.view(residual.shape), None
             return gemm.linear_split3(h3, self.w3.weight).view(*x.shape[:-1], self.w3.weight.shape[0]), self.w3.bias
         if self._fused and x.dtype == torch.float32:
diff --git a/dimsum_amd/models_dim.py b/dimsum_amd/models_dim.py
--- a/dimsum_amd/models_dim.py
+++ b/dimsum_amd/models_dim.py
@@ -284,6 +284,11 @@
 class _BlockBase(nn.Module):
 
     def _prenorm(self, hidden_states, residual):
+        if hidden_states is None:
+            assert self.fused_add_norm and residual is not None
+            fn = rms_norm_fn if isinstance(self.norm, RMSNorm) else layer_norm_fn
+            return fn(residual, self.norm.weight, self.norm.bias, residual=None, prenorm=True,
+                      residual_in_fp32=self.residual_in_fp32, eps=self.norm.eps)
         if not self.fused_add_norm:
             residual = hidden_states if residual is None else residual + self.drop_path(hidden_states)
             hidden_states = (self.norm(residual) if isinstance(self.norm, nn.Identity)
@@ -453,7 +458,7 @@
         self.adaLN_modulation = nn.Sequential(nn.SiLU(), nn.Linear(dim, 3 * dim, bias=True))
         self.mlp = _make_mlp(dim, use_gated_mlp)
 
-    def forward(self, hidden_states, residual=None, c=None, inference_params=None):
+    def forward(self, hidden_states, residual=None, c=None, inference_params=None, fold_residual=False):
         hidden_states, residual = self._prenorm(hidden_states, residual)
         if hidden_states.is_cuda and torch.is_grad_enabled() and hidden_states.requires_grad:
             x1, x2, hidden_states = _ForkHalves.apply(hidden_states)
@@ -489,6 +494,8 @@
                                                   residual=None if in_epilogue else hidden_states.reshape(B * L, H), is_rms_norm=True, x_bias=pb,
                                                   mod_scale=scale, mod_shift=shift, rows_per_batch=L, **({"split3": s3} if s3 else {}))
             if s3 and hnew.is_contiguous():
+                if fold_residual and residual.dtype == torch.float32 and residual.is_contiguous():
+                    return None, self.mlp.forward_deferred(hidden_states, x3=y, residual=hnew.view(B, L, H), gate=gate, res2=residual)[0]
                 return self.mlp.forward_deferred(hidden_states, x3=y, residual=hnew.view(B, L, H), gate=gate)[0], residual
             m, mb = self.mlp.forward_deferred(hidden_states, x3=y) if s3 else self.mlp.forward_deferred(y.view(B, L, H))
             return token_ops.gate_residual(hnew.view(B, L, H), m, gate, mb), residual
@@ -540,7 +547,7 @@
         self.mlp = cls(in_features=hidden_size, hidden_features=int(hidden_size * mlp_ratio), act_layer=_approx_gelu, drop=0)
         self.adaLN_modulation = nn.Sequential(nn.SiLU(), nn.Linear(hidden_size, 6 * hidden_size, bias=True))
 
-    def forward(self, x, c=None, **kwargs):
+    def forward(self, x, c=None, res2=None, **kwargs):
         sa, ca, ga, sm, cm, gm = _modulation(self.adaLN_modulation, c).chunk(6, dim=1)
         s3 = gemm.split3_enabled(x, self.attn.qkv.weight, producer="norm")
         h = _ln_modulate(self.norm1, x, sa, ca, split3=s3)
@@ -559,6 +566,8 @@
             return _mlp_tail(self.mlp, x, self.norm2(x), sm, cm, gm)
         if hasattr(self.mlp, "forward_deferred"):
             if s3 and x.is_contiguous():
+                if res2 is not None and res2.dtype == torch.float32 and res2.is_contiguous() and res2.shape == x.shape:
+                    return None, self.mlp.forward_deferred(x, x3=h, residual=x, gate=gm, res2=res2)[0]
                 return self.mlp.forward_deferred(x, x3=h, residual=x, gate=gm)[0]
             m, mb = self.mlp.forward_deferred(x, x3=h) if s3 else self.mlp.forward_deferred(h)
             return token_ops.gate_residual(x, m, gm, mb)
@@ -717,16 +726,31 @@
         finally:
             gemm._tls.cond = None
 
+    def _takes_summed_stream(self, idx):
+        if idx >= len(self.blocks):
+            return False
+        nxt = self.blocks[idx]
+        return isinstance(nxt, _BlockBase) and nxt.fused_add_norm and isinstance(nxt.norm, RMSNorm)
+
     def _forward_blocks(self, x, c, inference_params):
         x = self.x_embedder(x) + self.pos_embed
         residual = None
+        fold = (not torch.is_grad_enabled() and not self.training and x.is_cuda and x.dtype == torch.float32 and self.fused_add_norm
+                and gemm.res_epilogue_enabled())
         for idx, block in enumerate(self.blocks):
-            x, residual = block(x, residual, c, inference_params=inference_params)
-            if self.use_attn_every_k_layers > 0 and (idx + 1) % self.use_attn_every_k_layers == 0:
-                if self.use_independent_attn:
-                    x = self.attn_block[(idx + 1) // self.use_attn_every_k_layers - 1](x, c)
+            attn_next = self.use_attn_every_k_layers > 0 and (idx + 1) % self.use_attn_every_k_layers == 0
+            if fold and not attn_next and isinstance(block, _CombinedBase) and self._takes_summed_stream(idx + 1):
+                x, residual = block(x, residual, c, inference_params=inference_params, fold_residual=True)
+            else:
+                x, residual = block(x, residual, c, inference_params=inference_params)
+            if attn_next:
+                attn = self.attn_block[(idx + 1) // self.use_attn_every_k_layers - 1] if self.use_independent_attn else self.attn_block
+                if fold and residual is not None and self._takes_summed_stream(idx + 1):
+                    x = attn(x, c, res2=residual)
+                    if isinstance(x, tuple):
+                        x, residual = x
                 else:
-                    x = self.attn_block(x, c)
+                    x = attn(x, c)
         if self.norm_f is not None:
             if not self.fused_add_norm:
                 residual = x if residual is None else residual + self.drop_path(x)
diff --git a/dimsum_amd/native.py b/dimsum_amd/native.py
--- a/dimsum_amd/native.py
+++ b/dimsum_amd/native.py
@@ -927,8 +927,40 @@
     return out[0] if splits == 1 else out.sum(0)
 
 
+_res2_probe_cache = {}
+
+
+def gemm_nt_res2_supported(a, b, tune=None):
+    pair = isinstance(a, PairImage)
+    if isinstance(a, (PairImage, F16Image)):
+        a = a.data
+    if isinstance(b, F16Image):
+        b = b.data
+    if not gemm_nt_supported(a, b, False, pair=pair):
+        return False
+    key = (a.dtype, a.shape[0], b.shape[0], b.shape[1], a.stride(0), b.stride(0), pair, None if tune is None else tuple(tune), a.device.index)
+    hit = _res2_probe_cache.get(key)
+    if hit is None:
+        M, N, K = a.shape[0], b.shape[0], b.shape[1]
+        P = _lib.GemmParams()
+        X = _lib.attach_ext(P, _lib.GemmExt)
+        P.m, P.n, P.k, P.operand_dtype, P.epilogue, P.out_scale = M, N, K, _DT[a.dtype], _lib.GEMM_EPI_F32_GATE_RESIDUAL, 1.0
+        P.lda, P.ldb, P.ldc = a.stride(0), b.stride(0), N
+        if pair:
+            X.a_alias_rows = K // 3
+        fake = _ptr(a)
+        P.a_ptr, P.b_ptr = _ptr(a), _ptr(b)
+        X.residual_ptr, X.residual_ld, X.residual2_ptr, X.residual2_ld, X.out2_ptr, X.out2_ld = fake, N, fake, N, fake, N
+        if tune is not None:
+            X.tune_variant, X.tune_group_m = tune[:2]
+        with torch.cuda.device(a.device):
+            hit = _res2_probe_cache[key] = int(_lib.load().dimsum_gemm_nt_kernel_for(P)) >= 0
+    return hit
+
+
 def gemm_nt(a, b, bias=None, epilogue="f32", out=None, out_scale=1.0, events=None, tune=None, scales=None, gate_bound=None, residual=None,
-            gate=None, rows_per_batch=None, keep_x12=False, pair_out=False, weight_order=False, q_cols=None, conv=None):
+            gate=None, rows_per_batch=None, keep_x12=False, pair_out=False, weight_order=False, q_cols=None, conv=None, res2=None, out2=None,
+            keep_out=False):
     pair_in = isinstance(a, PairImage)
     pair_b = isinstance(b, PairImage)
     if pair_in:
@@ -956,9 +988,9 @@
         _check(bias.dtype == torch.float32 and bias.is_contiguous() and bias.numel() == N, "gemm_nt: bias must be (N,) float32")
     if epilogue == "f32":
         P.epilogue = _lib.GEMM_EPI_F32 if bias is None else _lib.GEMM_EPI_F32_BIAS
-        if out is None:
+        if out is None and (res2 is None or keep_out):
             out = torch.empty((M, N), device=a.device, dtype=torch.float32)
-        _check(out.dtype == torch.float32 and out.shape == (M, N) and out.stride(1) == 1, "gemm_nt: out must be (M, N) float32 rows")
+        _check(out is None or (out.dtype == torch.float32 and out.shape == (M, N) and out.stride(1) == 1), "gemm_nt: out must be (M, N) float32 rows")
         if conv is not None:
             cw, cb, seq = conv
             _gpu(cw, cb)
@@ -978,6 +1010,13 @@
                 _check(rows_per_batch and rows_per_batch % 256 == 0 and M % rows_per_batch == 0 and gate.dtype == torch.float32
                        and gate.shape == (M // rows_per_batch, N) and gate.stride(1) == 1, "gemm_nt: gate must be (M / rows_per_batch, N) float32, rows_per_batch % 256 == 0")
                 X.gate_ptr, X.gate_ld, X.rows_per_batch = _ptr(gate), gate.stride(0), rows_per_batch
+        if res2 is not None:
+            _gpu(res2, out2)
+            if out2 is None:
+                out2 = torch.empty((M, N), device=a.device, dtype=torch.float32)
+            _check(residual is not None and all(t.dtype == torch.float32 and t.shape == (M, N) and t.stride(1) == 1 for t in (res2, out2)),
+                   "gemm_nt: res2 / out2 must be (M, N) float32 rows and go with residual")
+            X.residual2_ptr, X.residual2_ld, X.out2_ptr, X.out2_ld = _ptr(res2), res2.stride(0), _ptr(out2), out2.stride(0)
     elif epilogue == "gated_split3":
         P.epilogue = _lib.GEMM_EPI_GATED_GELU_SPLIT3
         pieces = 2 if pair_out else 3
@@ -1000,7 +1039,8 @@
         _check(out.dtype == torch.float16 and out.shape == (M, N // 2) and out.stride(1) == 1, "gemm_nt: out must be (M, F) float16 rows")
     else:
         raise ValueError(f"gemm_nt: unknown epilogue {epilogue!r}")
-    P.ldc = out.stride(0)
+    _check(res2 is None or epilogue == "f32", "gemm_nt: res2 goes with the gate + residual epilogue")
+    P.ldc = out.stride(0) if out is not None else N
     h_inv = None
     if scales is not None:
         sa, sb = scales
@@ -1034,6 +1074,8 @@
         if _gemm_kernel_log is not None:
             _gemm_kernel_log.append((epilogue if conv is None else "f32_conv", int(_lib.load().dimsum_gemm_nt_kernel_for(P))))
         _lib.check(_lib.load().dimsum_gemm_nt(P, _stream(a)), "gemm_nt")
+    if res2 is not None:
+        return (out, out2) if keep_out else out2
     if x12 is not None:
         if h_inv is not None:
             return F16Image(out, h_inv), x12
diff --git a/include/dimsum_hip.h b/include/dimsum_hip.h
--- a/include/dimsum_hip.h
+++ b/include/dimsum_hip.h
@@ -329,6 +329,9 @@
     const void *c_scale_ptr;
     const void *k_inv_a_ptr;
     const void *k_inv_b_ptr;
+    const void *residual2_ptr;
+    void *out2_ptr;
+    int64_t residual2_ld, out2_ld;
 } dimsum_gemm_ext_t;
 
 typedef struct {
```

Result: no change. 3505 latents/s (median of 6 runs) (+0.9%).
